# t-neumann/versalignLib

Hardware: AMD Instinct MI355X
Metric: GCUPS (giga DP cell updates/sec) SW affine-gap, 150x500 bp (higher is better)
Workload: dtype int16; 1 GPU; 1048576 pairs/GPU, 150 bp x 500 bp, SW affine-gap int16 score (open -5, extend -1), inputs resident in HBM; pairs_per_gpu=1048576, read_length=150, ref_length=500, kernel_geometry=16x10

## Files before the change

### versalignlib_amd/csrc/cell_constants.h

```cpp
#pragma once

namespace valign {

struct Scoring {
    int match = 2, mismatch = -1, gap_read = -3, gap_ref = -3;
    bool affine = false;
    int open_read = -3, ext_read = -3, open_ref = -3, ext_ref = -3;
};

constexpr int kAlgSW = 0;
constexpr int kAlgNW = 1;

constexpr int kGapLinear = 0, kGapSym = 1, kGapAffine = 2, kGapAffineSym = 3;
constexpr int kGapAffineSymF16 = 4, kGapAffineF16 = 5, kGapSymF16 = 6;
constexpr int kTiltMaxK = 12;

constexpr int kBandNwAbsent16 = -16384;
constexpr int kBandNwAbsent32 = -(1 << 29);

enum FillKernel {
    kFillLinear = 0,
    kFillLinearSym,
    kFillAffine,
    kFillSse,
    kFillTag,
    kFillTagKey,
    kFillAffineSym,
    kFillAffineTag,
    kFillAffineTagSym,
    kFillSseTag,
    kFillSseTagKey,
    kFillTagProfKey,
    kFillKernels
};

}
```

### versalignlib_amd/csrc/cell_rules.h

```cpp
#pragma once

#include <algorithm>
#include <cstdlib>
#include <stdexcept>
#include <string>

#include "cell_constants.h"

namespace valign {

struct RuleInputs {
    Scoring sc;
    int R = 0, F = 0;
    bool sse_policy = false;
    bool no_sym = false, no_tag = false, no_f16 = false, no_prof_key = false;
    bool no_max3 = false;
    bool no_tilt = false;
    bool no_row_tables = false;
};

inline long long nw_tilt_span(const Scoring &sc, int rows, int F) {
    const long long per_row = -(long long)(sc.affine ? sc.ext_ref : sc.gap_ref);
    const long long per_col = -(long long)(sc.affine ? sc.ext_read : sc.gap_read);
    return per_row * (rows + 1) + per_col * (F + 1);
}

inline bool half_float_exact(const Scoring &sc, int alg, int R, int F, int rows) {
    const long long top = (long long)std::min(R, F) * std::max({sc.match, sc.mismatch, 0});
    long long slack = std::max({std::abs(sc.match), std::abs(sc.mismatch), std::abs(sc.open_read),
                                std::abs(sc.ext_read), std::abs(sc.open_ref), std::abs(sc.ext_ref)});
    if (alg == kAlgSW) return top + 2 * slack <= 2048 && slack <= 1024;
    if (!sc.affine) slack = std::max<long long>(slack, std::max(std::abs(sc.gap_read), std::abs(sc.gap_ref)));
    const long long span = nw_tilt_span(sc, rows, F);
    const long long centre = (top + span) / 2;
    return span < 30000 && (top + span - centre) + 3 * slack <= 2048 && centre + 3 * slack <= 2048 && slack <= 512;
}

inline bool half_float_unit_exact(const Scoring &sc, int R, int F) {
    const long long top = (long long)std::min(R, F) * std::max({sc.match, sc.mismatch, 0});
    const long long slack = std::max({std::abs(sc.match), std::abs(sc.mismatch), std::abs(sc.gap_read), std::abs(sc.gap_ref)});
    return top + 2 * slack < 1024 && slack < 512;
}

inline bool int16_range_ok(const RuleInputs &in, int alg, bool score_path, bool long_mode, int tilt_rows) {
    const Scoring &sc = in.sc;
    long long hi = (long long)std::min(in.R, in.F) * std::max(sc.match, 0) + 1;
    if (score_path && alg == kAlgNW && !long_mode) hi += nw_tilt_span(sc, tilt_rows, in.F);
    const int worst_gap = std::min({sc.gap_read, sc.gap_ref, sc.open_read, sc.open_ref, sc.ext_read, sc.ext_ref, 0});
    long long lo = alg == kAlgSW ? (long long)std::min(sc.mismatch, 0) + worst_gap
                                 : (long long)(std::min(in.R, in.F) + 2) * std::min(worst_gap, std::min(sc.mismatch, 0));
    if ((!score_path || long_mode) && sc.affine && alg == kAlgNW)
        lo = (long long)std::min(sc.open_ref, 0) + (long long)in.R * std::min(sc.ext_ref, 0) + std::min({sc.open_read, sc.open_ref, 0}) +
             std::min(sc.mismatch, 0);
    return !(hi > 32000 || lo < -32000 || (sc.affine && alg == kAlgNW && lo < -15000));
}

inline bool border_bad(const RuleInputs &in, int alg) {
    return alg == kAlgNW && !in.sc.affine && (long long)(in.R + 1) * std::min(in.sc.gap_ref, 0) < -32000;
}

inline bool int32_refused(const RuleInputs &in) {
    const Scoring &sc = in.sc;
    const long long worst = std::max({std::abs((long long)sc.match), std::abs((long long)sc.mismatch),
                                      std::abs((long long)(sc.affine ? sc.open_read : sc.gap_read)), std::abs((long long)(sc.affine ? sc.open_ref : sc.gap_ref)),
                                      sc.affine ? std::abs((long long)sc.ext_read) : 0ll, sc.affine ? std::abs((long long)sc.ext_ref) : 0ll});
    return (long long)(in.R + in.F + 2) * worst >= (1ll << 28);
}

inline bool tagged_range_ok(const RuleInputs &in, int alg, int rows) {
    const Scoring &sc = in.sc;
    long long hi = (long long)std::min(in.R, in.F) * std::max(sc.match, 0) + 1;
    if (alg == kAlgNW && !in.sse_policy)
        hi += (long long)-sc.gap_ref * (rows + 1) + (long long)-sc.gap_read * (in.F + 1);
    const int worst = std::min({sc.gap_read, sc.gap_ref, sc.mismatch, 0});
    const long long lo = alg == kAlgSW ? worst : (long long)(in.R + in.F + 2) * worst;
    if (alg == kAlgSW && !in.sse_policy && sc.gap_ref >= 0) return false;
    return 4 * hi + 4 <= 32000 && 4 * lo - 4 >= -32000 && std::abs(sc.match) < 2000 && std::abs(sc.mismatch) < 2000;
}

inline bool affine_tagged_range_ok(const RuleInputs &in, int alg, int geo_rows, int K) {
    const Scoring &sc = in.sc;
    long long hi = (long long)std::min(in.R, in.F) * std::max(sc.match, 0) + 1;
    const int worst = std::min({sc.open_read, sc.open_ref, sc.ext_read, sc.ext_ref, sc.mismatch, 0});
    long long lo = alg == kAlgSW ? worst
                                 : 2ll * (std::min(sc.open_read, 0) + std::min(sc.open_ref, 0)) +
                                       (long long)(in.R + in.F + 2) * std::min({sc.ext_read, sc.ext_ref, 0}) + worst;
    if (alg == kAlgNW) {
        const long long rows = (long long)geo_rows + 1, cols = in.F + 1;
        hi += std::max(0, -sc.ext_ref) * rows + std::max(0, -sc.ext_read) * cols;
        lo += std::min(0, -sc.ext_ref) * rows + std::min(0, -sc.ext_read) * cols;
        if (std::abs((long long)sc.ext_ref) * rows > 3500 || std::abs((long long)sc.ext_read) * cols > 3500) return false;
    }
    if (alg == kAlgSW && (sc.open_read >= 0 || sc.open_ref >= 0)) return false;
    const int key_bits = K <= 16 ? 4 : 5;
    if (alg == kAlgSW && ((hi + 1) << key_bits) > 32000) return false;
    return 8 * hi + 8 <= 32000 && 8 * lo - 8 >= -28000 && std::abs(sc.match) < 1000 && std::abs(sc.mismatch) < 1000;
}

inline bool lane_key_ok(const RuleInputs &in, int K) {
    return (((long long)std::min(in.R, in.F) * std::max(in.sc.match, 0) + 1) << (K <= 16 ? 4 : 5)) <= 32000;
}
inline bool prof_key_ok(const RuleInputs &in, int K) {
    const Scoring &sc = in.sc;
    return !in.sse_policy && !in.no_prof_key && K <= 16 && (((long long)std::min(in.R, in.F) * std::max(sc.match, 0) + 2) << 6) <= 32000 &&
           64ll * std::max(std::abs(sc.gap_read), std::abs(sc.gap_ref)) < 32000 && 64ll * std::abs(sc.mismatch) < 16000;
}

inline int score_gap_form(const RuleInputs &in, int alg, int R, int F, int rows) {
    const Scoring &sc = in.sc;
    if (sc.affine) {
        const bool sym = sc.open_read == sc.open_ref && sc.ext_read == sc.ext_ref && !in.no_sym;
        if (!in.no_f16 && half_float_exact(sc, alg, R, F, rows)) return sym ? kGapAffineSymF16 : kGapAffineF16;
        return sym ? kGapAffineSym : kGapAffine;
    }
    const int gaps = (sc.gap_read == sc.gap_ref && !in.no_sym) ? kGapSym : kGapLinear;
    if ((gaps == kGapSym || alg == kAlgNW) && !in.no_f16 &&
        (alg == kAlgNW ? half_float_exact(sc, alg, R, F, rows) : half_float_unit_exact(sc, R, F)))
        return kGapSymF16;
    return gaps;
}
inline bool gap_form_f16(int gaps) { return gaps == kGapSymF16 || gaps == kGapAffineSymF16 || gaps == kGapAffineF16; }

constexpr int kMax3WindowLow = 0x0400, kMax3WindowHigh = 0x7BFF;
inline int sym_affine_bias(const Scoring &sc) {
    const int o = -sc.open_ref, x = -sc.ext_ref, m = std::max({0, -sc.mismatch, -sc.match});
    return kMax3WindowLow + o + x + m;
}
inline bool sym_affine_max3_ok(const RuleInputs &in, int R, int F) {
    const Scoring &sc = in.sc;
    if (in.no_max3 || !sc.affine || sc.open_read != sc.open_ref || sc.ext_read != sc.ext_ref) return false;
    if (sc.open_ref > 0 || sc.ext_ref > 0) return false;
    const long long B = sym_affine_bias(sc);
    const long long hi = (long long)std::min(R, F) * std::max({sc.match, sc.mismatch, 0}) + 1;
    return B - kMax3WindowLow <= 1024 && B + hi <= kMax3WindowHigh;
}
inline const char *ran_sym_affine_name(bool max3) { return max3 ? "max3" : "sources"; }

inline int sym_affine_tilt_bias(const Scoring &sc) {
    const int o = -sc.open_ref, x = -sc.ext_ref, m = std::max({0, -sc.mismatch, -sc.match});
    return kMax3WindowLow + std::max(o - x, m);
}
inline long long sym_affine_tilt_top_index(int R, int F, int rows, int K) {
    const int lead = rows > R ? (rows - R) / K : 0;
    return (long long)rows + F - lead;
}
inline bool sym_affine_tilt_ok(const RuleInputs &in, int R, int F, int rows, int K) {
    if (in.no_tilt || K > kTiltMaxK || !sym_affine_max3_ok(in, R, F)) return false;
    const Scoring &sc = in.sc;
    const long long B = sym_affine_tilt_bias(sc);
    const long long hi = (long long)std::min(R, F) * std::max({sc.match, sc.mismatch, 0}) + 1;
    return B + (long long)-sc.ext_ref * sym_affine_tilt_top_index(R, F, rows, K) + hi <= kMax3WindowHigh;
}
inline const char *ran_sym_affine_frame_name(bool tilted) { return tilted ? "tilted" : "plain"; }

inline int sym_affine_row_table_low(const Scoring &sc) { return std::min({sc.match, sc.mismatch, 0}) - 2 * sc.ext_ref; }
inline int sym_affine_row_table_high(const Scoring &sc) {
    return std::max({sc.match, sc.mismatch, 0}) - 2 * sc.ext_ref + (sc.ext_ref - sc.open_ref);
}
inline bool sym_affine_row_tables_ok(const RuleInputs &in, int R, int F, int rows, int K, int lds_profile, int lds_tables) {
    if (in.no_row_tables || !sym_affine_tilt_ok(in, R, F, rows, K)) return false;
    if (in.sc.ext_ref - in.sc.open_ref < 0 || F > 60000) return false;
    return sym_affine_row_table_low(in.sc) >= 0 && sym_affine_row_table_high(in.sc) <= 255 && lds_tables <= lds_profile;
}
inline const char *ran_sym_affine_scores_name(bool row_tables) { return row_tables ? "row_tables" : "lds_profile"; }

struct FillChoice {
    int kernel = 0;
    bool affine_tagged = false, tagged = false;
};
inline FillChoice fill_choice(const RuleInputs &in, int alg, int G, int K) {
    const Scoring &sc = in.sc;
    FillChoice c;
    const int rows = G * K;
    c.affine_tagged = sc.affine && !in.sse_policy && !in.no_tag && affine_tagged_range_ok(in, alg, rows, K);
    c.tagged = !sc.affine && !in.no_tag && tagged_range_ok(in, alg, rows);
    const bool lane_key = c.tagged && alg == kAlgSW && lane_key_ok(in, K);
    const bool prof_key = lane_key && prof_key_ok(in, K);
    const bool affine_sym = sc.affine && sc.open_read == sc.open_ref && sc.ext_read == sc.ext_ref && !in.no_sym;
    if (prof_key) c.kernel = kFillTagProfKey;
    else if (c.tagged) c.kernel = in.sse_policy ? (lane_key ? kFillSseTagKey : kFillSseTag) : (lane_key ? kFillTagKey : kFillTag);
    else if (in.sse_policy) c.kernel = kFillSse;
    else if (sc.affine) c.kernel = c.affine_tagged ? (affine_sym ? kFillAffineTagSym : kFillAffineTag) : (affine_sym ? kFillAffineSym : kFillAffine);
    else c.kernel = (sc.gap_read == sc.gap_ref && !in.no_sym) ? kFillLinearSym : kFillLinear;
    return c;
}

constexpr int placed_key_bits(int K) { return K <= 4 ? 2 : (K <= 8 ? 3 : 4); }
constexpr int kPlacedKeyMaxK = 16;
constexpr int kPlacedStripRows = 1024;

enum class PlacedRoute { Refused, Key, Rows, Strip, Chain, Wide };

constexpr int kBandPlacedKeyBits = 4;
inline bool band_placed_key_ok(const RuleInputs &in) {
    return (((long long)std::min(in.R, in.F) * std::max(in.sc.match, 0) + 1) << kBandPlacedKeyBits) <= 0x7FFFFFFFll;
}

struct PlacedFacts {
    int band_width = 0;
    int score_width = 0;
    bool forced = false;
    bool long_plan = false;
    bool band_placed = false;
    bool chain_usable = false;
    bool placed_wide = false;
    bool extend_wide = false;
};

struct PlacedChoice {
    PlacedRoute route = PlacedRoute::Refused;
    int key_bits = 0;
    const char *reason = "";
};

inline PlacedChoice placed_choice(const RuleInputs &in, int alg, const PlacedFacts &f, int G, int K) {
    PlacedChoice c;
    (void)G;
    if (alg != kAlgSW)
        c.reason = "placed scores exist for Smith-Waterman only (the NW variant's score and its alignment's end cell are different cells)";
    else if (f.band_width > 0 && !f.band_placed)
        c.reason = "placed scores are not built for band_width > 0";
    else if (in.sse_policy)
        c.reason = "placed scores are not built for traceback_policy = 1 (SSE/AVX tie-breaks)";
    else if (f.band_width > 0) {
        if (!f.chain_usable)
            c.reason = "band_placed: the block chain has no usable plan for this read_length, ref_length, band_width and scoring (band_chain_plan); "
                       "placed scores under a band run nowhere else";
        else if (int32_refused(in))
            c.reason = "band_placed: shape x scoring can leave the int32 range of the DP cells";
        else if (!band_placed_key_ok(in))
            c.reason = "band_placed: min(read_length, ref_length) x match leaves the range of the chain's end-cell key (value << 4 in int32)";
        else {
            c.route = PlacedRoute::Chain;
            c.key_bits = kBandPlacedKeyBits;
        }
        return c;
    } else if (f.score_width == 32)
        c.reason = "placed scores are not built for score_width = 32 (int32 cells)";
    else if (!int16_range_ok(in, kAlgSW, true, false, 0))
        c.reason = "placed scores run on int16 cells: shape x scoring can leave their range";
    if (c.reason[0] && alg == kAlgSW && f.band_width <= 0 && !in.sse_policy && f.placed_wide && f.score_width != 16) {
        c.reason = "";
        if (int32_refused(in))
            c.reason = "placed_wide: shape x scoring can leave the int32 range of the DP cells";
        else
            c.route = PlacedRoute::Wide;
        return c;
    }
    if (c.reason[0]) return c;
    if (f.long_plan || (!f.forced && in.R > kPlacedStripRows)) {
        c.route = PlacedRoute::Strip;
        return c;
    }
    const int bits = placed_key_bits(K);
    const long long top = (long long)std::min(in.R, in.F) * std::max(in.sc.match, 0);
    if (K <= kPlacedKeyMaxK && ((top + 1) << bits) <= 32000) {
        c.route = PlacedRoute::Key;
        c.key_bits = bits;
    } else {
        c.route = PlacedRoute::Rows;
    }
    return c;
}

inline const char *ran_placed_name(PlacedRoute r) {
    static const char *const names[] = {"none", "key", "rows", "strip", "chain", "wide"};
    return names[(int)r];
}

inline long long span_ref_length(const RuleInputs &in) {
    const Scoring &sc = in.sc;
    const long long R = in.R, F = in.F;
    const long long m = std::max({sc.match, sc.mismatch, 0});
    const long long c = sc.affine ? std::min(std::abs((long long)sc.open_read), std::abs((long long)sc.ext_read)) : std::abs((long long)sc.gap_read);
    if (c == 0) return F;
    const long long gap_cols = R * m >= 1 ? (R * m - 1) / c : 0;
    return std::min(F, R + gap_cols);
}

inline PlacedChoice span_choice(const RuleInputs &in, int alg, const PlacedFacts &f, int G = 0, int K = 0) {
    PlacedFacts unbanded = f;
    unbanded.band_width = 0;
    PlacedChoice c = placed_choice(in, alg, unbanded, G, K);
    if (c.route != PlacedRoute::Refused && f.band_width > 0) {
        c = PlacedChoice{};
        c.reason = "spanned scores are not built for band_width > 0";
    }
    return c;
}

inline PlacedChoice subopt_choice(const RuleInputs &in, int alg, const PlacedFacts &f, int G, int K, int mask = 0) {
    PlacedFacts plain = f;
    plain.band_width = 0;
    plain.placed_wide = false;
    PlacedChoice c = placed_choice(in, alg, plain, G, K);
    if (c.route == PlacedRoute::Refused) return c;
    const char *reason = "";
    if (mask < 0)
        reason = "suboptimal scores need mask >= 0";
    else if (f.band_width > 0)
        reason = "suboptimal scores are not built for band_width > 0";
    else if (c.route != PlacedRoute::Key && c.route != PlacedRoute::Rows)
        reason = "suboptimal scores run on the register sweep only: reads of more than 1024 rows and shapes without a register geometry are refused";
    if (reason[0]) {
        c = PlacedChoice{};
        c.reason = reason;
    }
    return c;
}

inline int subopt_block_waves(int wave_lds, int ring_bytes, int placed_waves, int block_limit) {
    for (int waves = placed_waves; waves >= 1; waves >>= 1)
        if ((long long)(wave_lds + ring_bytes) * waves <= block_limit) return waves;
    return 0;
}
constexpr const char *kSuboptNoRing = "suboptimal scores: one wave's reference tables leave no room for its column ring in the LDS (a shorter reference, or a geometry of more lanes per group, has it)";

inline long long extend_cell_top(const RuleInputs &in) {
    return (long long)std::min(in.R, in.F) * std::max({in.sc.match, in.sc.mismatch, 0});
}
inline long long extend_cell_bottom(const RuleInputs &in) {
    const Scoring &sc = in.sc;
    const long long per_row = sc.affine ? std::min({sc.open_ref, sc.ext_ref, 0}) : std::min(sc.gap_ref, 0);
    const long long per_col = sc.affine ? std::min({sc.open_read, sc.ext_read, 0}) : std::min(sc.gap_read, 0);
    const long long addend = sc.affine ? std::min({sc.match, sc.mismatch, sc.open_read, sc.ext_read, sc.open_ref, sc.ext_ref, 0})
                                       : std::min({sc.match, sc.mismatch, sc.gap_read, sc.gap_ref, 0});
    return per_row * in.R + per_col * in.F + addend;
}
inline bool extend_int16_ok(const RuleInputs &in) { return extend_cell_top(in) <= 32000 && extend_cell_bottom(in) >= -32000; }

constexpr long long kExtendWideCellBound = 1ll << 28;
constexpr int kExtendWideLoses = -(1 << 29);
inline bool extend_int32_ok(const RuleInputs &in) {
    const Scoring &sc = in.sc;
    const long long top_addend = std::max({sc.match, sc.mismatch, 0});
    const long long worst_ext = sc.affine ? std::min({sc.ext_read, sc.ext_ref, 0}) : std::min({sc.gap_read, sc.gap_ref, 0});
    const long long low_addend = sc.affine ? std::min({sc.match, sc.mismatch, sc.open_read, sc.ext_read, sc.open_ref, sc.ext_ref, 0})
                                           : std::min({sc.match, sc.mismatch, sc.gap_read, sc.gap_ref, 0});
    if (extend_cell_top(in) > kExtendWideCellBound || extend_cell_bottom(in) < -kExtendWideCellBound) return false;
    if (kExtendWideLoses + top_addend >= -kExtendWideCellBound) return false;
    return kExtendWideLoses + worst_ext * ((long long)in.R + in.F) + low_addend >= -(1ll << 31);
}

inline PlacedChoice extend_choice(const RuleInputs &in, int alg, const PlacedFacts &f, int G, int K) {
    PlacedChoice c;
    (void)G;
    (void)K;
    bool opens_wide = false;
    if (alg != kAlgSW)
        c.reason = "extension scores are defined for opt & 0xF == 0 only (the NW variant's free reference start is another matrix)";
    else if (in.sse_policy)
        c.reason = "extension scores are not built for traceback_policy = 1 (SSE/AVX tie-breaks)";
    else if (f.band_width > 0)
        c.reason = "extension scores are not built for band_width > 0";
    else if (f.score_width == 32) {
        c.reason = "extension scores are not built for score_width = 32 (int32 cells)";
        opens_wide = true;
    } else if (!extend_int16_ok(in)) {
        c.reason = "extension scores run on signed int16 cells: shape x scoring can leave their range";
        opens_wide = f.score_width == 0;
    } else if (f.long_plan || (!f.forced && in.R > kPlacedStripRows)) {
        c.reason = "extension scores run on the register sweep only: reads of more than 1024 rows and shapes without a register geometry are refused";
        opens_wide = true;
    } else
        c.route = PlacedRoute::Rows;
    if (opens_wide && f.extend_wide) {
        if (extend_int32_ok(in)) {
            c.reason = "";
            c.route = PlacedRoute::Wide;
        } else {
            c.reason = "extend_wide: shape x scoring can leave the range the int32 cells keep below their borders' sentinel";
        }
    }
    return c;
}

inline bool band_nw_connects(int R, int F, int band_width) {
    return R > 0 && 2ll * (band_width / 2) + 1 >= ((long long)F + R - 1) / R;
}
inline void band_nw_check(int R, int F, int band_width) {
    if (!band_nw_connects(R, F, band_width))
        throw std::runtime_error("band_nw: band_width " + std::to_string(band_width) + " is too narrow for read_length " + std::to_string(R) +
                                 ", ref_length " + std::to_string(F) + " (the windows of consecutive blocks do not connect: 2 * (band_width / 2) + 1 "
                                 "must be at least ceil(ref_length / read_length))");
}

inline bool band_nw_int16_ok(const RuleInputs &in) {
    const Scoring &sc = in.sc;
    const long long worst = sc.affine ? std::min({sc.open_read, sc.open_ref, sc.ext_read, sc.ext_ref, sc.mismatch, sc.match, 0})
                                      : std::min({sc.gap_read, sc.gap_ref, sc.mismatch, sc.match, 0});
    const long long top_add = std::max({sc.match, sc.mismatch, 0});
    const long long hi = (long long)std::min(in.R, in.F) * std::max(sc.match, 0) + 1;
    const long long lo = (long long)(in.R + in.F + 2) * worst + (sc.affine ? std::min({sc.open_read, sc.open_ref, 0}) : 0);
    return kBandNwAbsent16 + top_add < lo && kBandNwAbsent16 + worst >= -32768 && hi <= 16000;
}

enum class AlignRoute { Fused, Register, Strip, StripBand, StripWide, StripWideBand, StripCkpt };

struct RouteFacts {
    bool banded = false;
    bool wide_align = false;
    bool read_strips = false;
    bool fused_off = false;
    bool small_call = false;
    int fused_rows = 0;
    bool checkpoints = false;
    bool band_nw = false;
    int band_width = 0;
};

inline AlignRoute align_route(const RuleInputs &in, int alg, const RouteFacts &f) {
    if (f.banded && alg != kAlgSW && !f.band_nw) throw std::runtime_error("band_alignments applies to Smith-Waterman alignments only");
    if (f.banded && in.sse_policy)
        throw std::runtime_error("band_alignments needs traceback_policy = 0 (no banded SSE/AVX tie-breaks)");
    const bool nw_band = f.banded && alg == kAlgNW;
    if (nw_band) band_nw_check(in.R, in.F, f.band_width);
    if (border_bad(in, alg) || !int16_range_ok(in, alg, false, false, 0) || f.wide_align || (nw_band && !band_nw_int16_ok(in))) {
        if (int32_refused(in))
            throw std::runtime_error("shape x scoring can leave the int32 range of the DP cells (read_length " + std::to_string(in.R) +
                                     ", ref_length " + std::to_string(in.F) + ")");
        return f.banded ? AlignRoute::StripWideBand : AlignRoute::StripWide;
    }
    if (f.banded) return AlignRoute::StripBand;
    if (f.read_strips) return (f.checkpoints && !in.sse_policy) ? AlignRoute::StripCkpt : AlignRoute::Strip;
    if (in.sse_policy && in.sc.affine)
        throw std::runtime_error("traceback_policy = 1 (SSE/AVX tie-breaks) exists for the linear gap model only");
    if (f.small_call && !f.fused_off && !in.sc.affine && !in.sse_policy && !in.no_tag && tagged_range_ok(in, alg, f.fused_rows)) return AlignRoute::Fused;
    return AlignRoute::Register;
}

inline bool strip_chunks(AlignRoute r, const RouteFacts &f) {
    return r == AlignRoute::Strip || r == AlignRoute::StripCkpt || r == AlignRoute::StripBand || r == AlignRoute::StripWideBand || (r == AlignRoute::StripWide && f.read_strips);
}

inline const char *ran_fill_name(AlignRoute r, int fill_kernel = -1) {
    static const char *const names[kFillKernels] = {"linear", "linear_sym", "affine", "sse", "tag", "tag_key", "affine_sym",
                                                    "affine_tag", "affine_tag_sym", "sse_tag", "sse_tag_key", "tag_prof_key"};
    static const char *const routes[] = {"fused_tag", nullptr, "strip", "strip_band", "strip_wide", "strip_wide_band", "strip_ckpt"};
    if (r != AlignRoute::Register) return routes[(int)r];
    return fill_kernel >= 0 && fill_kernel < kFillKernels ? names[fill_kernel] : "none";
}

struct SpanCigarChoice {
    PlacedChoice forward;
    AlignRoute child = AlignRoute::Register;
    std::string reason;
    bool refused() const { return !reason.empty(); }
};
constexpr const char *kSpanCigarPrefix = "spanned CIGARs: ";
inline SpanCigarChoice span_cigar_choice(const RuleInputs &in, int alg, const PlacedFacts &f, const RuleInputs &child, const RouteFacts &child_facts,
                                         int G = 0, int K = 0) {
    SpanCigarChoice c;
    c.forward = span_choice(in, alg, f, G, K);
    if (c.forward.route == PlacedRoute::Refused) {
        c.reason = c.forward.reason;
        return c;
    }
    try {
        c.child = align_route(child, alg, child_facts);
    } catch (const std::runtime_error &e) {
        c.forward = PlacedChoice{};
        c.reason = std::string(kSpanCigarPrefix) + e.what();
    }
    return c;
}

}
```

### versalignlib_amd/csrc/dp_kernels.hip.h

```cpp
#pragma once

#include <hip/hip_runtime.h>
#include <stdint.h>

#include <type_traits>
#include <utility>

#include "base_classes.h"
#include "cell_constants.h"

namespace valign {

typedef short s16x2 __attribute__((ext_vector_type(2)));
typedef _Float16 f16x2 __attribute__((ext_vector_type(2)));
typedef unsigned short u16x2 __attribute__((ext_vector_type(2)));

constexpr int kWave = 64;
constexpr int kWaveLanes = 64;
constexpr int kCodePad = 72;
constexpr short kNegInf = -16384;

constexpr int kMaxScoreGroups = 16;
constexpr int kOneSweep = 0x7FFFFFFF;

struct ScoreArgs {
    const uint8_t *reads;
    const uint8_t *refs;
    int16_t *scores;
    long long n;
    int R, F;
    int prof_area;
    int refc_stride;
    int wave_lds;
    short match, mismatch;
    union {
        struct {
            short gap_read, gap_ref;
        };
        int sym_max3_bias;
    };
    short open_read, ext_read, open_ref, ext_ref;
    int n_groups;
    struct Group {
        unsigned block_end;
        int F;
        long long n;
        long long pair_ofs;
        long long read_ofs, ref_ofs;
    } groups[kMaxScoreGroups];
};

__device__ __forceinline__ s16x2 pk(short v) { return s16x2{v, v}; }
__device__ __forceinline__ s16x2 pk_max(s16x2 a, s16x2 b) { return __builtin_elementwise_max(a, b); }
__device__ __forceinline__ s16x2 pk_add_sat(s16x2 a, s16x2 b) { return __builtin_elementwise_add_sat(a, b); }
__device__ __forceinline__ s16x2 pk_sub_floor0(s16x2 a, s16x2 g) {
    return (s16x2)__builtin_elementwise_sub_sat((u16x2)a, (u16x2)g);
}
__device__ __forceinline__ unsigned as_u32(s16x2 v) { return __builtin_bit_cast(unsigned, v); }
__device__ __forceinline__ s16x2 as_pk(unsigned v) { return __builtin_bit_cast(s16x2, v); }

__device__ __forceinline__ unsigned from_prev_lane(unsigned v) {
    return (unsigned)__builtin_amdgcn_update_dpp(0, (int)v, 0x138 , 0xF, 0xF, false);
}

template <int G>
__device__ __forceinline__ unsigned group_prev_or_zero(unsigned v, unsigned lmask) {
    if (G == 16) return (unsigned)__builtin_amdgcn_update_dpp(0, (int)v, 0x111 , 0xF, 0xF, true);
    return from_prev_lane(v) & lmask;
}

template <int G>
__device__ __forceinline__ s16x2 group_prev_or(s16x2 v, s16x2 lead_border, unsigned lmask) {
    return as_pk(group_prev_or_zero<G>(as_u32(v), lmask) | as_u32(lead_border));
}
__device__ __forceinline__ s16x2 pk_max_h(s16x2 a, s16x2 b) {
    return __builtin_bit_cast(s16x2, __builtin_elementwise_maximum(__builtin_bit_cast(f16x2, a), __builtin_bit_cast(f16x2, b)));
}
__device__ __forceinline__ s16x2 pk_max3_h(s16x2 a, s16x2 b, s16x2 c) {
    return __builtin_bit_cast(s16x2, __builtin_elementwise_maximum(__builtin_elementwise_maximum(__builtin_bit_cast(f16x2, a), __builtin_bit_cast(f16x2, b)),
                                                                  __builtin_bit_cast(f16x2, c)));
}

template <int... Is, class Fn>
__device__ __forceinline__ void unrolled_steps(std::integer_sequence<int, Is...>, Fn &&fn) {
    (fn(std::integral_constant<int, Is>{}), ...);
}

constexpr int profile_conflicts(int G, int lane_dw, int width, int stride_dw) {
    const int banks = width == 1 ? 32 : 64;
    int extra = 0;
    const int ngroups = width == 4 ? 4 : 2;
    for (int grp = 0; grp < ngroups; ++grp) {
        int hits[64] = {};
        int worst = 0;
        for (int lane = 0; lane < kWaveLanes; ++lane) {
            int member = 0;
            if (width == 4) {
                const int m = lane & 31;
                const bool first = m < 4 || (m >= 12 && m < 16) || (m >= 20 && m < 28);
                member = (lane < 32 ? 0 : 2) + (first ? 0 : 1);
            } else {
                member = lane / 32;
            }
            if (member != grp) continue;
            const int l = lane % G, pair = 2 * (lane / G);
            const int dw = pair * stride_dw + l * lane_dw;
            for (int x = 0; x < width; ++x) {
                const int b = (dw + x) % banks;
                hits[b] += 1;
                worst = hits[b] > worst ? hits[b] : worst;
            }
        }
        extra += worst - 1;
    }
    return extra;
}

template <int G, int K>
struct Geo {
    static_assert(G == 4 || G == 8 || G == 16 || G == 32 || G == 64, "group size");
    static_assert(K % 2 == 0, "rows per lane must be even");
    static constexpr int kGroups = kWave / G;
    static constexpr int kPairs = 2 * kGroups;
    static constexpr int kRows = G * K;
    static constexpr int kLaneBytes = K * 2;
    static constexpr int kLoadDwords = (K * 2) % 16 == 0 ? 4 : ((K * 2) % 8 == 0 ? 2 : 1);
    static constexpr int slab_dwords() {
        const int rows_dw = kRows / 2;
        int best = rows_dw, best_cost = profile_conflicts(G, K / 2, kLoadDwords, rows_dw);
        for (int pad = kLoadDwords; pad < 64 && best_cost > 0; pad += kLoadDwords) {
            const int c = profile_conflicts(G, K / 2, kLoadDwords, rows_dw + pad);
            if (c < best_cost) {
                best_cost = c;
                best = rows_dw + pad;
            }
        }
        return best;
    }
    static constexpr int kPairStride = slab_dwords() * 4;
    static constexpr int kZeroSlab = 4 * kPairs;
    static constexpr int kProfBytes = (4 * kPairs + 1) * kPairStride;
    __host__ __device__ static constexpr int row_offset(int l, int q) { return l * kLaneBytes + q * 2; }
};

typedef __attribute__((address_space(3))) const unsigned lds_cu32;
typedef unsigned u32x2 __attribute__((ext_vector_type(2)));
typedef unsigned u32x4 __attribute__((ext_vector_type(4)));
typedef __attribute__((address_space(3))) const u32x2 lds_cu32x2;
typedef __attribute__((address_space(3))) const u32x4 lds_cu32x4;
typedef __attribute__((address_space(3))) const unsigned char lds_cu8;

__device__ __forceinline__ unsigned lds_offset(const void *p) {
    return (unsigned)(size_t)(__attribute__((address_space(3))) const void *)p;
}

__device__ __forceinline__ void stage_span(unsigned char *dst, const uint8_t *src, long long begin,
                                           long long end, int lane) {
    const unsigned long long a0 = (unsigned long long)(src + begin) & ~15ull;
    const unsigned long long lo = (unsigned long long)(src + begin);
    const unsigned long long hi = (unsigned long long)(src + end);
    for (unsigned long long a = a0 + 16ull * lane; a < hi; a += 16ull * kWave) {
        unsigned char *d = dst + (a - a0);
        if (a >= lo && a + 16 <= hi) {
            *reinterpret_cast<uint4 *>(d) = *reinterpret_cast<const uint4 *>(a);
        } else {
            for (int b = 0; b < 16; ++b)
                if (a + b >= lo && a + b < hi) d[b] = *reinterpret_cast<const uint8_t *>(a + b);
        }
    }
}

__device__ __forceinline__ unsigned lds_dword_at(const unsigned char *p) {
    const unsigned a = lds_offset(p), base = a & ~3u;
    const unsigned lo = *(lds_cu32 *)(base), hi = *(lds_cu32 *)(base + 4);
    return __builtin_amdgcn_alignbyte(hi, lo, a & 3u);
}

extern __shared__ __align__(16) unsigned char valign_smem[];

struct WaveTables {
    unsigned char *prof;
    unsigned char *refc;
    int *first_bad;
    long long pair0;
    int last;
    int cols_used;
};

template <int G, int K, bool FIND_BAD>
__device__ __forceinline__ bool wave_setup(const uint8_t *reads, const uint8_t *refs, long long n, int R, int F,
                                           int prof_area, int refc_stride, int wave_lds, short match,
                                           short mismatch, WaveTables &w, bool bad_is_non_acgt = false,
                                           unsigned block = blockIdx.x, short zero_score = 0,
                                           int strip_row0 = kOneSweep, short row_key_step = 0, short row0_score = 0) {
    using geo = Geo<G, K>;
    const int lane = threadIdx.x & (kWave - 1);
    const int wave = threadIdx.x / kWave;
    const int row0 = strip_row0 == kOneSweep ? R - geo::kRows : strip_row0;

    unsigned char *lds = valign_smem + (size_t)wave * wave_lds;
    unsigned char *prof = lds;
    unsigned char *refc = lds + prof_area;
    int *first_bad = reinterpret_cast<int *>(refc + geo::kGroups * refc_stride);

    const int waves = blockDim.x / kWave;
    const long long pair0 = ((long long)block * waves + wave) * geo::kPairs;
    const bool live = pair0 < n;
    long long pair_end = pair0 + geo::kPairs;
    if (pair_end > n) pair_end = n;
    const int last = (int)(pair_end - pair0) - 1;

    const bool whole = geo::kPairs * F + 32 <= prof_area;
    const int rd_off = ((geo::kPairs * F + 32 + 15) / 16) * 16;
    const bool rd_staged = whole && strip_row0 == kOneSweep && rd_off + geo::kPairs * R + 32 <= prof_area;

    unsigned char rd[2 * K];
    if (live && FIND_BAD && lane < geo::kPairs) {
        first_bad[2 * lane] = R;
        first_bad[2 * lane + 1] = F;
    }
    if (live && !rd_staged) {
#pragma unroll
        for (int i = 0; i < 2 * K; ++i) {
            const int idx = lane + kWave * i;
            const int p = idx / geo::kRows, rr = idx - p * geo::kRows;
            const int ps = p > last ? last : p;
            const int pos = row0 + rr;
            rd[i] = (pos >= 0 && pos < R) ? reads[(pair0 + ps) * R + pos] : (unsigned char)0;
        }
    }

    int cols_used = 0;
    if (live) {
        for (int idx = lane; idx < geo::kGroups * 2 * kCodePad; idx += kWave) {
            const int g = idx / (2 * kCodePad), x = idx - g * (2 * kCodePad);
            const int col = x < kCodePad ? x : F + x;
            unsigned char *dst = refc + g * refc_stride + 2 * col;
            dst[0] = dst[1] = (unsigned char)geo::kZeroSlab;
        }
    }
    if (whole) {
        if (live) stage_span(prof, refs, pair0 * F, pair_end * F, lane);
        if (live && rd_staged) stage_span(prof + rd_off, reads, pair0 * R, pair_end * R, lane);
        __syncthreads();
    }
    constexpr unsigned kZero4 = (unsigned)geo::kZeroSlab * 0x01010101u;
#pragma unroll
    for (int g = 0; g < geo::kGroups; ++g) {
        int pa = 2 * g, pb = 2 * g + 1;
        pa = pa > last ? last : pa;
        pb = pb > last ? last : pb;
        const long long ref_lo = whole ? pair0 * F : (pair0 + pa) * F;
        if (!whole) {
            if (live) stage_span(prof, refs, ref_lo, (pair0 + pb + 1) * F, lane);
            __syncthreads();
        }
        if (live) {
            const int ref_skew = (int)((unsigned long long)(refs + ref_lo) & 15ull);
            const unsigned char *raw_a = prof + ref_skew + (whole ? pa * F : 0), *raw_b = raw_a + (pb - pa) * F;
            unsigned char *codes_g = refc + g * refc_stride + 2 * kCodePad;
            const unsigned slab_a_lo = geo::kZeroSlab | (unsigned)(2 * g) << 8 | (unsigned)(geo::kPairs + 2 * g) << 16 |
                                       (unsigned)(2 * geo::kPairs + 2 * g) << 24;
            const unsigned slab_a_hi = (unsigned)(3 * geo::kPairs + 2 * g) | (kZero4 & 0xFFFFFF00u);
            const unsigned slab_b_lo = slab_a_lo + 0x01010100u, slab_b_hi = slab_a_hi + 1u;
            const int F4 = F & ~3;
            for (int j = 4 * lane; j < F4; j += 4 * kWave) {
                const unsigned ca = base_class4(lds_dword_at(raw_a + j)), cb = base_class4(lds_dword_at(raw_b + j));
                const unsigned sa = select_bytes8(slab_a_hi, slab_a_lo, ca), sb = select_bytes8(slab_b_hi, slab_b_lo, cb);
                uint2 codes;
                codes.x = __builtin_amdgcn_perm(sb, sa, 0x05010400u);
                codes.y = __builtin_amdgcn_perm(sb, sa, 0x07030602u);
                *reinterpret_cast<uint2 *>(codes_g + 2 * j) = codes;
                const unsigned used = (sa ^ kZero4) | (sb ^ kZero4);
                if (used) {
                    const int end = j + 4 - (__builtin_clz(used) >> 3);
                    cols_used = end > cols_used ? end : cols_used;
                }
                if (FIND_BAD) {
                    const unsigned bad_a = ~nonzero_bytes(bad_is_non_acgt ? sa ^ kZero4 : ca) & 0x80808080u;
                    const unsigned bad_b = ~nonzero_bytes(bad_is_non_acgt ? sb ^ kZero4 : cb) & 0x80808080u;
                    if (bad_a) atomicMin(&first_bad[2 * (2 * g) + 1], j + (__builtin_ctz(bad_a) >> 3));
                    if (bad_b) atomicMin(&first_bad[2 * (2 * g + 1) + 1], j + (__builtin_ctz(bad_b) >> 3));
                }
            }
            for (int j = F4 + lane; j < F; j += kWave) {
                const int ca = base_class(raw_a[j]);
                const int cb = base_class(raw_b[j]);
                const bool va = ca >= 1 && ca <= 4, vb = cb >= 1 && cb <= 4;
                const unsigned sa = va ? (ca - 1) * geo::kPairs + 2 * g : geo::kZeroSlab;
                const unsigned sb = vb ? (cb - 1) * geo::kPairs + 2 * g + 1 : geo::kZeroSlab;
                *reinterpret_cast<unsigned short *>(codes_g + 2 * j) = (unsigned short)(sa | (sb << 8));
                if (va || vb) cols_used = j + 1 > cols_used ? j + 1 : cols_used;
                if (FIND_BAD) {
                    if (ca == 0 || (bad_is_non_acgt && ca == 5)) atomicMin(&first_bad[2 * (2 * g) + 1], j);
                    if (cb == 0 || (bad_is_non_acgt && cb == 5)) atomicMin(&first_bad[2 * (2 * g + 1) + 1], j);
                }
            }
        }
        if (!whole) __syncthreads();
    }
    unsigned rd4[K / 2];
    constexpr int kItemPairs = 256 / geo::kRows, kItemRows = 256 % geo::kRows;
    const int item_p0 = (4 * lane) / geo::kRows, item_rr0 = (4 * lane) % geo::kRows, item_q0 = (4 * lane) % K;
    if (live && rd_staged) {
        const unsigned char *raw = prof + rd_off + (int)((unsigned long long)(reads + pair0 * R) & 15ull);
        int p = item_p0, rr = item_rr0;
#pragma unroll
        for (int it = 0; it < K / 2; ++it) {
            const int ps = p > last ? last : p;
            const int pos = row0 + rr;
            const int at = pos < -3 ? -3 : pos;
            unsigned w4 = lds_dword_at(raw + ps * R + at);
            if (pos < 0) w4 = pos < -3 ? 0u : w4 & (0xFFFFFFFFu << (8 * -pos));
            rd4[it] = base_class4(w4);
            p += kItemPairs; rr += kItemRows;
            if (rr >= geo::kRows) { rr -= geo::kRows; ++p; }
        }
    }
    if (whole) __syncthreads();

    if (live && rd_staged) {
        auto table = [&](int c, int shift, unsigned &lo, unsigned &hi) __attribute__((always_inline)) {
            unsigned b[8];
#pragma unroll
            for (int a = 0; a < 8; ++a)
                b[a] = ((unsigned)(unsigned short)(a >= 1 && a <= 4 ? (a == c + 1 ? match : mismatch) : zero_score) >> shift) & 0xFFu;
            lo = b[0] | b[1] << 8 | b[2] << 16 | b[3] << 24;
            hi = b[4] | b[5] << 8 | b[6] << 16 | b[7] << 24;
        };
        int p = item_p0, rr = item_rr0;
#pragma unroll
        for (int it = 0; it < K / 2; ++it) {
            const unsigned cls = rd4[it];
            const int pos = row0 + rr;
            if (FIND_BAD) {
                unsigned good = bad_is_non_acgt ? select_bytes8(0x00000001u, 0x01010100u, cls) : cls;
                if (pos < 0) good |= pos < -3 ? 0xFFFFFFFFu : ~(0xFFFFFFFFu << (8 * -pos));
                const unsigned bad = ~nonzero_bytes(good) & 0x80808080u;
                if (bad) atomicMin(&first_bad[2 * p], pos + (__builtin_ctz(bad) >> 3));
            }
            u16x2 key01 = u16x2{0, 0}, key23 = u16x2{0, 0};
            if (row_key_step != 0) {
                const int q0 = rr % K, q1 = (rr + 1) % K, q2 = (rr + 2) % K, q3 = (rr + 3) % K;
                key01 = u16x2{(unsigned short)(row_key_step * (15 - q0)), (unsigned short)(row_key_step * (15 - q1))};
                key23 = u16x2{(unsigned short)(row_key_step * (15 - q2)), (unsigned short)(row_key_step * (15 - q3))};
            }
            if (row0_score != 0) {
                int q0 = item_q0 + (256 * it) % K;
                q0 -= q0 >= K ? K : 0;
                auto row0 = [&](int i) __attribute__((always_inline)) {
                    const int q = q0 + i;
                    return (i == 0 ? q == 0 : q == K) || (K < 4 && q == 2 * K);
                };
                const unsigned short a = (unsigned short)row0_score, none = 0;
                key01 = key01 + u16x2{row0(0) ? a : none, row0(1) ? a : none};
                key23 = key23 + u16x2{row0(2) ? a : none, row0(3) ? a : none};
            }
            unsigned char *dst = prof + p * geo::kPairStride + 2 * rr;
#pragma unroll
            for (int c = 0; c < 4; ++c) {
                unsigned lo_lo, lo_hi, hi_lo, hi_hi;
                table(c, 0, lo_lo, lo_hi);
                table(c, 8, hi_lo, hi_hi);
                const unsigned lows = select_bytes8(lo_hi, lo_lo, cls), highs = select_bytes8(hi_hi, hi_lo, cls);
                const u16x2 s01 = __builtin_bit_cast(u16x2, __builtin_amdgcn_perm(highs, lows, 0x05010400u)) + key01;
                const u16x2 s23 = __builtin_bit_cast(u16x2, __builtin_amdgcn_perm(highs, lows, 0x07030602u)) + key23;
                unsigned *out = reinterpret_cast<unsigned *>(dst + c * geo::kPairs * geo::kPairStride);
                out[0] = __builtin_bit_cast(unsigned, s01);
                out[1] = __builtin_bit_cast(unsigned, s23);
            }
            p += kItemPairs; rr += kItemRows;
            if (rr >= geo::kRows) { rr -= geo::kRows; ++p; }
        }
    }
    if (live && !rd_staged) {
#pragma unroll
        for (int i = 0; i < 2 * K; ++i) {
            const int idx = lane + kWave * i;
            const int p = idx / geo::kRows, rr = idx - p * geo::kRows;
            const int pos = row0 + rr;
            const bool in_read = pos >= 0 && pos < R;
            const int a = in_read ? base_class(rd[i]) : 0;
            if (FIND_BAD && in_read && (a == 0 || (bad_is_non_acgt && a == 5)))
                atomicMin(&first_bad[2 * p], pos);
            const bool valid = a >= 1 && a <= 4;
            const int off = p * geo::kPairStride + geo::row_offset(rr / K, rr % K);
            const short row_key = (short)(row_key_step * (15 - rr % K) + (rr % K == 0 ? row0_score : 0));
#pragma unroll
            for (int c = 0; c < 4; ++c) {
                const short sc = (short)((valid ? (a == c + 1 ? match : mismatch) : zero_score) + row_key);
                *reinterpret_cast<short *>(prof + c * geo::kPairs * geo::kPairStride + off) = sc;
            }
        }
    }
    if (live) {
        for (int idx = lane; idx < geo::kPairStride / 4; idx += kWave) {
            const unsigned lo = (unsigned short)(zero_score + row_key_step * (15 - (2 * idx) % K) + ((2 * idx) % K == 0 ? row0_score : 0));
            const unsigned hi = (unsigned short)(zero_score + row_key_step * (15 - (2 * idx + 1) % K) + ((2 * idx + 1) % K == 0 ? row0_score : 0));
            reinterpret_cast<unsigned *>(prof + geo::kZeroSlab * geo::kPairStride)[idx] = lo | (hi << 16);
        }
    }
    __syncthreads();
#pragma unroll
    for (int d = kWave / 2; d >= 1; d >>= 1) {
        const int other = __shfl_xor(cols_used, d, kWave);
        cols_used = other > cols_used ? other : cols_used;
    }
    w.cols_used = __builtin_amdgcn_readfirstlane(cols_used);
    w.prof = prof;
    w.refc = refc + 2 * kCodePad;
    w.first_bad = first_bad;
    w.pair0 = pair0;
    w.last = last;
    return live;
}

constexpr int row_table_pad(int G) { return G + 4; }
constexpr unsigned kSelZero4 = 0x0c0c0c0cu;

template <int G, int K>
__device__ __forceinline__ bool wave_setup_tables(const uint8_t *reads, const uint8_t *refs, long long n, int R, int F,
                                                  int refs_area, int sel_stride, int wave_lds, short match, short mismatch,
                                                  short zero_score, short row0_score, unsigned block, WaveTables &w,
                                                  unsigned (&Ta)[K], unsigned (&Tb)[K], bool &repair) {
    using geo = Geo<G, K>;
    constexpr int kPad = row_table_pad(G);
    const int lane = threadIdx.x & (kWave - 1);
    const int wave = threadIdx.x / kWave;
    const int row0 = R - geo::kRows;

    unsigned char *raw = valign_smem + (size_t)wave * wave_lds;
    unsigned char *sel = raw + refs_area;

    const int waves = blockDim.x / kWave;
    const long long pair0 = ((long long)block * waves + wave) * geo::kPairs;
    const bool live = pair0 < n;
    long long pair_end = pair0 + geo::kPairs;
    if (pair_end > n) pair_end = n;
    const int last = (int)(pair_end - pair0) - 1;

    if (live) {
        stage_span(raw, refs, pair0 * F, pair_end * F, lane);
        stage_span(sel, reads, pair0 * R, pair_end * R, lane);
    }
    __syncthreads();

    if (live) {
        auto table = [&](int c, unsigned &lo, unsigned &hi) __attribute__((always_inline)) {
            unsigned b[8];
#pragma unroll
            for (int a = 0; a < 8; ++a) b[a] = (unsigned)(a >= 1 && a <= 4 ? (a == c + 1 ? match : mismatch) : zero_score) & 0xFFu;
            lo = b[0] | b[1] << 8 | b[2] << 16 | b[3] << 24;
            hi = b[4] | b[5] << 8 | b[6] << 16 | b[7] << 24;
        };
        unsigned t_lo[4], t_hi[4];
#pragma unroll
        for (int c = 0; c < 4; ++c) table(c, t_lo[c], t_hi[c]);
        const unsigned char *raw_rd = sel + (int)((unsigned long long)(reads + pair0 * R) & 15ull);
        const int grp = lane / G, l = lane % G;
#pragma unroll
        for (int half = 0; half < 2; ++half) {
            int p = 2 * grp + half;
            p = p > last ? last : p;
#pragma unroll
            for (int q0 = 0; q0 < K; q0 += 4) {
                const int pos = row0 + l * K + q0;
                const int at = pos < -3 ? -3 : pos;
                unsigned w4 = lds_dword_at(raw_rd + p * R + at);
                if (pos < 0) w4 = pos < -3 ? 0u : w4 & (0xFFFFFFFFu << (8 * -pos));
                const unsigned cls = base_class4(w4);
                unsigned col[4];
#pragma unroll
                for (int c = 0; c < 4; ++c) col[c] = select_bytes8(t_hi[c], t_lo[c], cls);
                const unsigned lo01 = __builtin_amdgcn_perm(col[1], col[0], 0x05010400u), hi01 = __builtin_amdgcn_perm(col[1], col[0], 0x07030602u);
                const unsigned lo23 = __builtin_amdgcn_perm(col[3], col[2], 0x05010400u), hi23 = __builtin_amdgcn_perm(col[3], col[2], 0x07030602u);
                unsigned (&T)[K] = half ? Tb : Ta;
                T[q0] = __builtin_amdgcn_perm(lo23, lo01, 0x05040100u);
                T[q0 + 1] = __builtin_amdgcn_perm(lo23, lo01, 0x07060302u);
                if (q0 + 2 < K) {
                    T[q0 + 2] = __builtin_amdgcn_perm(hi23, hi01, 0x05040100u);
                    T[q0 + 3] = __builtin_amdgcn_perm(hi23, hi01, 0x07060302u);
                }
            }
        }
        const unsigned r4 = ((unsigned)row0_score & 0xFFu) * 0x01010101u;
        Ta[0] += r4;
        Tb[0] += r4;
    }
    __syncthreads();

    int cols_used = 0;
    bool before_last = false;
    unsigned *stream = reinterpret_cast<unsigned *>(sel);
    const int stride_dw = sel_stride / 4;
    if (live) {
        for (int idx = lane; idx < geo::kGroups * 2 * kPad; idx += kWave) {
            const int g = idx / (2 * kPad), x = idx - g * (2 * kPad);
            stream[g * stride_dw + (x < kPad ? x : F + x)] = kSelZero4;
        }
        const int ref_skew = (int)((unsigned long long)(refs + pair0 * F) & 15ull);
        typedef unsigned short u16;
#pragma unroll
        for (int g = 0; g < geo::kGroups; ++g) {
            int pa = 2 * g, pb = 2 * g + 1;
            pa = pa > last ? last : pa;
            pb = pb > last ? last : pb;
            const unsigned char *raw_a = raw + ref_skew + pa * F, *raw_b = raw + ref_skew + pb * F;
            unsigned *out_g = stream + g * stride_dw + kPad;
            u16x2 ends_a = u16x2{0, 0}, ends_b = u16x2{0, 0};
            auto note = [](u16x2 &ends, unsigned acgt, int j) __attribute__((always_inline)) {
                const unsigned none = ~nonzero_bytes(acgt) & 0x80808080u;
                const u16 end = acgt ? (u16)(j + 4 - (__builtin_clz(acgt) >> 3)) : (u16)0;
                const u16 first_none = none ? (u16)(0xFFFF - (j + (__builtin_ctz(none) >> 3))) : (u16)0;
                ends = __builtin_elementwise_max(ends, u16x2{end, first_none});
            };
            const int F4 = F & ~3;
            for (int j = 4 * lane; j < F4; j += 4 * kWave) {
                const unsigned ca = base_class4(lds_dword_at(raw_a + j)), cb = base_class4(lds_dword_at(raw_b + j));
                const unsigned sa = select_bytes8(0x0c0c0c03u, 0x0201000cu, ca), sb = select_bytes8(0x0c0c0c07u, 0x0605040cu, cb);
                uint4 s;
                s.x = __builtin_amdgcn_perm(sb, sa, 0x0c040c00u) | 0x0c000c00u;
                s.y = __builtin_amdgcn_perm(sb, sa, 0x0c050c01u) | 0x0c000c00u;
                s.z = __builtin_amdgcn_perm(sb, sa, 0x0c060c02u) | 0x0c000c00u;
                s.w = __builtin_amdgcn_perm(sb, sa, 0x0c070c03u) | 0x0c000c00u;
                *reinterpret_cast<uint4 *>(out_g + j) = s;
                note(ends_a, sa ^ kSelZero4, j);
                note(ends_b, sb ^ kSelZero4, j);
            }
            for (int j = F4 + lane; j < F; j += kWave) {
                const int ca = base_class(raw_a[j]), cb = base_class(raw_b[j]);
                const bool va = ca >= 1 && ca <= 4, vb = cb >= 1 && cb <= 4;
                out_g[j] = (va ? (unsigned)(ca - 1) : 0x0cu) | (vb ? (unsigned)(cb + 3) : 0x0cu) << 16 | 0x0c000c00u;
                ends_a = __builtin_elementwise_max(ends_a, u16x2{va ? (u16)(j + 1) : (u16)0, va ? (u16)0 : (u16)(0xFFFF - j)});
                ends_b = __builtin_elementwise_max(ends_b, u16x2{vb ? (u16)(j + 1) : (u16)0, vb ? (u16)0 : (u16)(0xFFFF - j)});
            }
#pragma unroll
            for (int d = kWave / 2; d >= 1; d >>= 1) {
                ends_a = __builtin_elementwise_max(ends_a, __builtin_bit_cast(u16x2, __shfl_xor(__builtin_bit_cast(int, ends_a), d, kWave)));
                ends_b = __builtin_elementwise_max(ends_b, __builtin_bit_cast(u16x2, __shfl_xor(__builtin_bit_cast(int, ends_b), d, kWave)));
            }
            before_last |= 0xFFFF - (int)ends_a.y < (int)ends_a.x || 0xFFFF - (int)ends_b.y < (int)ends_b.x;
            cols_used = (int)ends_a.x > cols_used ? (int)ends_a.x : cols_used;
            cols_used = (int)ends_b.x > cols_used ? (int)ends_b.x : cols_used;
        }
    }
    __syncthreads();
    repair = __builtin_amdgcn_readfirstlane((int)before_last) != 0;
    w.cols_used = __builtin_amdgcn_readfirstlane(cols_used);
    w.prof = raw;
    w.refc = reinterpret_cast<unsigned char *>(stream + kPad);
    w.first_bad = nullptr;
    w.pair0 = pair0;
    w.last = last;
    return live;
}

template <int K>
__device__ __forceinline__ void lds_load_lane(unsigned addr, unsigned (&v)[K / 2]) {
    constexpr int N = K / 2;
    if constexpr ((K * 2) % 16 == 0) {
#pragma unroll
        for (int i = 0; i < N / 4; ++i) {
            const u32x4 x = *(lds_cu32x4 *)(addr + 16 * i);
            v[4 * i] = x.x; v[4 * i + 1] = x.y; v[4 * i + 2] = x.z; v[4 * i + 3] = x.w;
        }
    } else if constexpr ((K * 2) % 8 == 0) {
#pragma unroll
        for (int i = 0; i < N / 2; ++i) {
            const u32x2 x = *(lds_cu32x2 *)(addr + 8 * i);
            v[2 * i] = x.x; v[2 * i + 1] = x.y;
        }
    } else {
#pragma unroll
        for (int i = 0; i < N; ++i) v[i] = *(lds_cu32 *)(addr + 4 * i);
    }
}

template <int K>
__device__ __forceinline__ void merge_profile(const unsigned (&va)[K / 2], const unsigned (&vb)[K / 2], s16x2 (&S)[K]) {
#pragma unroll
    for (int c = 0; c < K / 2; ++c) {
        S[2 * c + 0] = as_pk(__builtin_amdgcn_perm(vb[c], va[c], 0x05040100u));
        S[2 * c + 1] = as_pk(__builtin_amdgcn_perm(vb[c], va[c], 0x07060302u));
    }
}

template <int G, int K>
__device__ __forceinline__ void fetch_profile(unsigned addr_a, unsigned addr_b, s16x2 (&S)[K]) {
    unsigned va[K / 2], vb[K / 2];
    lds_load_lane<K>(addr_a, va);
    lds_load_lane<K>(addr_b, vb);
    merge_profile<K>(va, vb, S);
}



constexpr int kTrackAll = 0, kTrackNone = 1, kTrackPair = 2;

__host__ __device__ inline int nw_frame_centre(int R, int F, int rows, int match, int mismatch, int tilt_row, int tilt_col) {
    const int best = match > mismatch ? match : mismatch;
    const int top = (R < F ? R : F) * (best > 0 ? best : 0);
    return (top + tilt_row * (rows + 1) + tilt_col * (F + 1)) / 2;
}

template <int G, int K, int ALG, int GAPS>
__global__ void __launch_bounds__(256)
score_kernel(const ScoreArgs args) {
    using geo = Geo<G, K>;
    constexpr bool F16 = GAPS == kGapAffineSymF16 || GAPS == kGapAffineF16;
    constexpr bool F16SYM = GAPS == kGapAffineSymF16;
    constexpr bool AFFINE = GAPS == kGapAffine || GAPS == kGapAffineSym || F16;
    constexpr bool SYM = GAPS == kGapSym;
    constexpr bool LINF16 = GAPS == kGapSymF16;
    constexpr bool AFFSYM = GAPS == kGapAffineSym;
    constexpr bool SOURCES = AFFSYM && ALG == kAlgSW;
    const int lane = threadIdx.x & (kWave - 1);
    const int grp = lane / G;
    const int l = lane % G;

    const uint8_t *reads = args.reads, *refs = args.refs;
    int16_t *scores = args.scores;
    long long n_pairs = args.n;
    int F_batch = args.F;
    unsigned block = blockIdx.x;
    if (args.n_groups > 0) {
        int g = 0;
        while (g + 1 < args.n_groups && block >= args.groups[g].block_end) ++g;
        block -= g ? args.groups[g - 1].block_end : 0u;
        reads += args.groups[g].read_ofs;
        refs += args.groups[g].ref_ofs;
        scores += args.groups[g].pair_ofs;
        n_pairs = args.groups[g].n;
        F_batch = args.groups[g].F;
    }

    WaveTables w;
    constexpr bool LINF16_SW = LINF16 && ALG == kAlgSW, LINF16_NW = LINF16 && ALG == kAlgNW;
    constexpr bool TILT = ALG == kAlgNW;
    constexpr bool HALF = F16 || LINF16;
    const int tilt_row = TILT ? -(int)(AFFINE ? args.ext_ref : args.gap_ref) : 0;
    const int tilt_col = TILT ? -(int)(AFFINE ? args.ext_read : args.gap_read) : 0;
    int fold = tilt_row + tilt_col;
    short s_row0 = 0;
    if constexpr (SOURCES && K <= kTiltMaxK) {
        if (args.sym_max3_bias > 0 && (args.sym_max3_bias >> 16) != 0) {
            fold = -2 * (int)args.ext_ref;
            s_row0 = (short)((int)args.ext_ref - (int)args.open_ref);
        }
    }
    const int centre = (HALF && TILT) ? nw_frame_centre(args.R, F_batch, G * K, args.match, args.mismatch, tilt_row, tilt_col) : 0;
    const int rcentre = (HALF && TILT) ? nw_frame_centre(args.R, F_batch, G * K, args.match, args.mismatch, 0, 0) : 0;
    const float unit = LINF16_SW ? 1.0f / 1024.0f : 1.0f;
    auto cell = [](int v) __attribute__((always_inline)) {
        return HALF ? pk(__builtin_bit_cast(short, (_Float16)v)) : pk((short)v);
    };
    auto cell_add = [](s16x2 a, s16x2 b) __attribute__((always_inline)) {
        return HALF ? __builtin_bit_cast(s16x2, __builtin_bit_cast(f16x2, a) + __builtin_bit_cast(f16x2, b)) : a + b;
    };
    auto cell_sub = [](s16x2 a, s16x2 b) __attribute__((always_inline)) {
        return HALF ? __builtin_bit_cast(s16x2, __builtin_bit_cast(f16x2, a) - __builtin_bit_cast(f16x2, b)) : a - b;
    };
    const short s_match = HALF ? __builtin_bit_cast(short, (_Float16)(((int)args.match + fold) * unit)) : (short)(args.match + fold);
    const short s_mismatch = HALF ? __builtin_bit_cast(short, (_Float16)(((int)args.mismatch + fold) * unit)) : (short)(args.mismatch + fold);
    const short s_zero = HALF ? __builtin_bit_cast(short, (_Float16)fold) : (short)fold;
    bool tables = false, repair = false;
    unsigned Ta[K], Tb[K];
    if constexpr (SOURCES && K <= kTiltMaxK) {
        tables = args.sym_max3_bias > 0 && (args.sym_max3_bias >> 16 & 3) == 3;
        bool live = false;
        if (tables)
            live = wave_setup_tables<G, K>(reads, refs, n_pairs, args.R, F_batch, args.prof_area, args.refc_stride, args.wave_lds,
                                           s_match, s_mismatch, s_zero, s_row0, block, w, Ta, Tb, repair);
        if (!tables)
            live = wave_setup<G, K, false>(reads, refs, n_pairs, args.R, F_batch, args.prof_area, args.refc_stride,
                                           args.wave_lds, s_match, s_mismatch, w, false, block, s_zero, kOneSweep, 0, s_row0);
        if (!live) return;
    } else if (!wave_setup<G, K, false>(reads, refs, n_pairs, args.R, F_batch, args.prof_area, args.refc_stride,
                                        args.wave_lds, s_match, s_mismatch, w, false, block, s_zero, kOneSweep, 0, s_row0))
        return;
    const long long pair0 = w.pair0;
    const int F = (ALG == kAlgSW) ? w.cols_used : F_batch;

    const unsigned lmask = l == 0 ? 0u : 0xFFFFFFFFu;
    const unsigned lane_base = lds_offset(w.prof) + l * geo::kLaneBytes;
    const int lead = (ALG == kAlgSW && G * K > args.R) ? (G * K - args.R) / K : 0;
    unsigned code_addr = lds_offset(w.refc) + grp * args.refc_stride - 2 * (l - lead);

    s16x2 g_read, g_ref, o_read, e_read, o_ref, e_ref;
    if (ALG == kAlgSW) {
        g_read = pk((short)-args.gap_read);   g_ref = pk((short)-args.gap_ref);
        o_read = pk((short)-args.open_read);  e_read = pk((short)-args.ext_read);
        o_ref = pk((short)-args.open_ref);    e_ref = pk((short)-args.ext_ref);
    } else {
        g_read = g_ref = e_read = e_ref = pk(0);
        o_read = pk((short)(args.open_read - args.ext_read));
        o_ref = pk((short)(args.open_ref - args.ext_ref));
    }
    const s16x2 border_f = pk(ALG == kAlgNW ? (F16 ? (short)0xFC00 : kNegInf) : (short)0);
    const _Float16 open_h = (_Float16)(int)(TILT ? args.open_ref - args.ext_ref : args.open_ref), ext_h = (_Float16)(int)args.ext_ref;
    const _Float16 open_rd = (_Float16)(int)(TILT ? args.open_read - args.ext_read : args.open_read), ext_rd = (_Float16)(int)args.ext_read;
    const f16x2 o_half = f16x2{open_h, open_h}, e_half = f16x2{ext_h, ext_h}, zero_half = f16x2{(_Float16)0, (_Float16)0};
    const f16x2 o_read_half = f16x2{open_rd, open_rd}, e_read_half = f16x2{ext_rd, ext_rd};

    s16x2 Hl[K], El[K], HOl[K];
#pragma unroll
    for (int q = 0; q < K; ++q) {
        Hl[q] = cell(tilt_row * (l * K + q) - centre);
        El[q] = border_f;
        HOl[q] = (ALG == kAlgSW) ? pk(0) : (F16 ? cell_add(Hl[q], pk(__builtin_bit_cast(short, open_h))) : Hl[q] + o_ref);
    }
    s16x2 up0 = pk(0), h_last = Hl[K - 1], f_last = border_f, best = pk(0);
    s16x2 fup_keep = border_f;
    s16x2 row_best = cell(-rcentre);
    int j = -l;
    s16x2 top_row = pk(0), top_step = pk(0), row_tilt = pk(0);
    const s16x2 col_step = cell(tilt_col);
    if (TILT) {
        if (l == 0) {
            top_row = cell(-tilt_row + tilt_col - centre);
            top_step = col_step;
            up0 = cell(-tilt_row - centre);
        }
        row_tilt = cell(tilt_row * (G * K - 1) + tilt_col * (1 - l) - centre + rcentre);
    }

    constexpr bool PIPE = true;
    unsigned pa[K / 2], pb[K / 2];
    s16x2 S0[K], S1[K];
    unsigned ca_next = 0, cb_next = 0;
    if (PIPE && !tables) {
        const unsigned ca = *(lds_cu8 *)(code_addr), cb = *(lds_cu8 *)(code_addr + 1);
        lds_load_lane<K>(lane_base + ca * geo::kPairStride, pa);
        lds_load_lane<K>(lane_base + cb * geo::kPairStride, pb);
        ca_next = *(lds_cu8 *)(code_addr + 2);
        cb_next = *(lds_cu8 *)(code_addr + 3);
    }

    lds_cu8 *code_ptr = (lds_cu8 *)code_addr;

    auto step = [&](auto masked_tag, auto track_tag, s16x2 (&S)[K], s16x2 (&Snext)[K]) __attribute__((always_inline)) {
        constexpr bool MASKED = decltype(masked_tag)::value;
        constexpr int TRACK = decltype(track_tag)::value;
        const s16x2 diag0 = up0;
        if (G == 16) {
            up0 = as_pk((unsigned)__builtin_amdgcn_update_dpp(0, (int)as_u32(h_last), 0x111, 0xF, 0xF, true));
        } else {
            up0 = as_pk(from_prev_lane(as_u32(h_last)) & lmask);
        }
        if (TILT) up0 = as_pk(as_u32(up0) | as_u32(top_row));
        s16x2 fup0 = border_f;
        if (AFFINE && !SOURCES) {
            if (G == 16 && ALG == kAlgSW) {
                fup0 = as_pk((unsigned)__builtin_amdgcn_update_dpp(0, (int)as_u32(f_last), 0x111, 0xF, 0xF, true));
            } else if (G != 16) {
                const unsigned fv = from_prev_lane(as_u32(f_last));
                fup0 = (ALG == kAlgNW) ? as_pk(l == 0 ? as_u32(border_f) : fv) : as_pk(fv & lmask);
            }
            if (G == 16 && ALG == kAlgNW) {
                fup_keep = as_pk((unsigned)__builtin_amdgcn_update_dpp((int)as_u32(fup_keep), (int)as_u32(f_last), 0x111, 0xF, 0xF, false));
                fup0 = fup_keep;
            }
        }
        s16x2 gup0 = pk(0);
        if (LINF16_SW) gup0 = as_pk(group_prev_or_zero<G>(as_u32(f_last), lmask));
        if (PIPE) {
            merge_profile<K>(pa, pb, S);
            lds_load_lane<K>(lane_base + ca_next * geo::kPairStride, pa);
            lds_load_lane<K>(lane_base + cb_next * geo::kPairStride, pb);
            if constexpr (SOURCES) {
                ca_next = code_ptr[4];
                cb_next = code_ptr[5];
            } else {
                ca_next = *(lds_cu8 *)(code_addr + 4);
                cb_next = *(lds_cu8 *)(code_addr + 5);
            }
        }
        if (!MASKED || (unsigned)j < (unsigned)F) {
            if (!PIPE) {
                const unsigned ca = *(lds_cu8 *)(code_addr), cb = *(lds_cu8 *)(code_addr + 1);
                fetch_profile<G, K>(lane_base + ca * geo::kPairStride, lane_base + cb * geo::kPairStride, S);
            }
            if (LINF16_SW) {
                auto hf = [](s16x2 v) __attribute__((always_inline)) { return __builtin_bit_cast(f16x2, v); };
                auto bits = [](f16x2 v) __attribute__((always_inline)) { return __builtin_bit_cast(s16x2, v); };
                const _Float16 gs = (_Float16)((int)args.gap_ref * (1.0f / 1024.0f));
                const f16x2 g_unit = f16x2{gs, gs}, zero2 = f16x2{(_Float16)0, (_Float16)0}, one2 = f16x2{(_Float16)1, (_Float16)1};
                f16x2 up_c = hf(gup0);
                f16x2 h = zero2;
                f16x2 d_cur = hf(diag0) + hf(S[0]), d_prev = zero2;
                f16x2 bestf = hf(best);
#pragma unroll
                for (int q = 0; q < K; ++q) {
                    f16x2 d_next = d_cur;
                    if (q + 1 < K) d_next = hf(Hl[q]) + hf(S[q + 1]);
                    h = __builtin_elementwise_maximum(__builtin_elementwise_maximum(d_cur, hf(El[q])), up_c);
                    Hl[q] = bits(h);
                    up_c = __builtin_elementwise_min(__builtin_elementwise_max(h + g_unit, zero2), one2);
                    El[q] = bits(up_c);
                    if (q & 1) bestf = __builtin_elementwise_maximum(__builtin_elementwise_maximum(bestf, d_prev), d_cur);
                    else if (q == K - 1) bestf = __builtin_elementwise_maximum(bestf, d_cur);
                    d_prev = d_cur;
                    d_cur = d_next;
                }
                best = bits(bestf);
                h_last = bits(h);
                f_last = bits(up_c);
            } else if (LINF16) {
                auto hf = [](s16x2 v) __attribute__((always_inline)) { return __builtin_bit_cast(f16x2, v); };
                f16x2 h = hf(up0);
                f16x2 d_cur = hf(diag0) + hf(S[0]);
#pragma unroll
                for (int q = 0; q < K; ++q) {
                    f16x2 d_next = d_cur;
                    if (q + 1 < K) d_next = hf(Hl[q]) + hf(S[q + 1]);
                    h = __builtin_elementwise_maximum(__builtin_elementwise_maximum(d_cur, hf(Hl[q])), h);
                    Hl[q] = __builtin_bit_cast(s16x2, h);
                    d_cur = d_next;
                }
                h_last = __builtin_bit_cast(s16x2, h);
            } else if (F16) {
                auto hf = [](s16x2 v) __attribute__((always_inline)) { return __builtin_bit_cast(f16x2, v); };
                auto bits = [](f16x2 v) __attribute__((always_inline)) { return __builtin_bit_cast(s16x2, v); };
                f16x2 d_cur, e_cur, d_prev = zero_half;
                auto pass1 = [&](int q, f16x2 &d, f16x2 &e) __attribute__((always_inline)) {
                    d = hf(q == 0 ? diag0 : Hl[q - 1]) + hf(S[q]);
                    const f16x2 e_open = F16SYM ? hf(HOl[q]) : hf(Hl[q]) + o_read_half;
                    e = __builtin_elementwise_maximum(TILT ? hf(El[q]) : hf(El[q]) + e_read_half, e_open);
                    if (ALG == kAlgSW) e = __builtin_elementwise_maximum(e, zero_half);
                    El[q] = bits(e);
                };
                f16x2 f = hf(fup0);
                f16x2 ho = hf(up0) + o_half;
                f16x2 h = zero_half;
                f16x2 bestf = hf(best);
                pass1(0, d_cur, e_cur);
#pragma unroll
                for (int q = 0; q < K; ++q) {
                    f = __builtin_elementwise_maximum(TILT ? f : f + e_half, ho);
                    f16x2 d_next = zero_half, e_next = zero_half;
                    if (q + 1 < K) pass1(q + 1, d_next, e_next);
                    h = __builtin_elementwise_maximum(__builtin_elementwise_maximum(d_cur, e_cur), f);
                    Hl[q] = bits(h);
                    ho = h + o_half;
                    if (F16SYM) HOl[q] = bits(ho);
                    if (ALG == kAlgSW) {
                        if (q & 1) bestf = __builtin_elementwise_maximum(__builtin_elementwise_maximum(bestf, d_prev), d_cur);
                        else if (q == K - 1) bestf = __builtin_elementwise_maximum(bestf, d_cur);
                    }
                    d_prev = d_cur;
                    d_cur = d_next;
                    e_cur = e_next;
                }
                best = bits(bestf);
                h_last = bits(h);
                f_last = bits(f);
            } else if (SOURCES) {
                s16x2 d_cur = diag0 + S[0];
                s16x2 xf = as_pk(group_prev_or_zero<G>(as_u32(f_last), lmask)), h = pk(0);
#pragma unroll
                for (int q = 0; q < K; ++q) {
                    const s16x2 g = pk_max(El[q], xf);
                    s16x2 d_next = pk(0);
                    if (q + 1 < K) d_next = Hl[q] + S[q + 1];
                    const s16x2 y = pk_sub_floor0(g, o_ref);
                    const s16x2 a = pk_sub_floor0(El[q], e_ref);
                    if (TRACK == kTrackAll) best = pk_max(best, d_cur);
                    if (TRACK == kTrackPair) best = pk_max(best, g);
                    h = pk_max(d_cur, y);
                    const s16x2 b = pk_sub_floor0(xf, e_ref);
                    Hl[q] = h;
                    El[q] = pk_max(a, h);
                    xf = pk_max(b, h);
                    d_cur = d_next;
                }
                if (TRACK == kTrackPair) best = pk_max(best, h);
                h_last = h;
                f_last = xf;
            } else if (SYM) {
                s16x2 h = up0;
                s16x2 d_cur = diag0 + S[0];
#pragma unroll
                for (int q = 0; q < K; ++q) {
                    const s16x2 x = pk_max(Hl[q], h);
                    s16x2 d_next = pk(0);
                    if (q + 1 < K) d_next = Hl[q] + S[q + 1];
                    const s16x2 y = (ALG == kAlgSW) ? pk_sub_floor0(x, g_ref) : x;
                    if (ALG == kAlgSW && TRACK == kTrackAll) best = pk_max(best, d_cur);
                    if (ALG == kAlgSW && TRACK == kTrackPair) best = pk_max(best, x);
                    h = pk_max(d_cur, y);
                    Hl[q] = h;
                    d_cur = d_next;
                }
                if (ALG == kAlgSW && TRACK == kTrackPair) best = pk_max(best, h);
                h_last = h;
            } else {
                auto pass1 = [&](int q) __attribute__((always_inline)) -> s16x2 {
                    const s16x2 d = (q == 0 ? diag0 : Hl[q - 1]) + S[q];
                    s16x2 e;
                    if (AFFSYM) {
                        e = pk_max((ALG == kAlgSW) ? pk_sub_floor0(El[q], e_read) : El[q], HOl[q]);
                        El[q] = e;
                    } else if (AFFINE) {
                        e = (ALG == kAlgSW)
                                ? pk_max(pk_sub_floor0(El[q], e_read), pk_sub_floor0(Hl[q], o_read))
                                : pk_max(El[q], pk_add_sat(Hl[q], o_read));
                        El[q] = e;
                    } else {
                        e = (ALG == kAlgSW) ? pk_sub_floor0(Hl[q], g_read) : Hl[q];
                    }
                    if (ALG == kAlgSW) best = pk_max(best, d);
                    return pk_max(d, e);
                };
                s16x2 h = up0, f = fup0;
                s16x2 ho = pk(0);
                if (AFFSYM) ho = (ALG == kAlgSW) ? pk_sub_floor0(up0, o_ref) : pk_add_sat(up0, o_ref);
                s16x2 m_cur = pass1(0);
#pragma unroll
                for (int q = 0; q < K; ++q) {
                    if (AFFSYM) {
                        f = pk_max((ALG == kAlgSW) ? pk_sub_floor0(f, e_ref) : f, ho);
                    } else if (AFFINE) {
                        f = (ALG == kAlgSW) ? pk_max(pk_sub_floor0(f, e_ref), pk_sub_floor0(h, o_ref))
                                            : pk_max(f, pk_add_sat(h, o_ref));
                    } else {
                        f = (ALG == kAlgSW) ? pk_sub_floor0(h, g_ref) : h;
                    }
                    s16x2 m_next = pk(0);
                    if (q + 1 < K) m_next = pass1(q + 1);
                    h = pk_max(m_cur, f);
                    Hl[q] = h;
                    if (AFFSYM) {
                        ho = (ALG == kAlgSW) ? pk_sub_floor0(h, o_ref) : pk_add_sat(h, o_ref);
                        HOl[q] = ho;
                    }
                    m_cur = m_next;
                }
                h_last = h;
                f_last = f;
            }
            if (ALG == kAlgNW) {
                const s16x2 last = cell_sub(h_last, row_tilt);
                if (HALF) row_best = __builtin_bit_cast(s16x2, __builtin_elementwise_maximum(__builtin_bit_cast(f16x2, row_best),
                                                                                      __builtin_bit_cast(f16x2, last)));
                else row_best = pk_max(row_best, last);
            }
        }
        if (TILT) {
            top_row = cell_add(top_row, top_step);
            row_tilt = cell_add(row_tilt, col_step);
        }
        ++j;
        if constexpr (SOURCES) code_ptr += 2;
        else code_addr += 2;
    };

    using all_t = std::integral_constant<int, kTrackAll>;
    using first_t = std::integral_constant<int, ((SYM && ALG == kAlgSW) || SOURCES) ? kTrackNone : kTrackAll>;
    using second_t = std::integral_constant<int, ((SYM && ALG == kAlgSW) || SOURCES) ? kTrackPair : kTrackAll>;
    if constexpr (ALG == kAlgSW) {
        static_assert(G - 1 + 1 + 2 <= kCodePad, "the unmasked sweep and its prefetch stay inside the code pad");
        const int steps = F + G - 1 - lead;
        int t = 0;
        bool biased = false;
        if constexpr (SOURCES) {
            biased = args.sym_max3_bias > 0;
            const bool tilted = K <= kTiltMaxK && biased && (args.sym_max3_bias >> 16) != 0;
            if constexpr (K <= kTiltMaxK) if (tilted) {
                const int B = args.sym_max3_bias & 0xFFFF, xi = -(int)args.ext_ref;
                const int oxi = -(int)args.open_ref - xi;
                const s16x2 ox_c = pk((short)oxi), kx_c = pk((short)(K * xi));
                const int u0 = l * (K - 1);
                s16x2 lead_border = as_pk(as_u32(pk((short)(B + xi - oxi))) & ~lmask);
                const s16x2 lead_step = as_pk(as_u32(pk((short)xi)) & ~lmask);
                const int s0 = K - steps % K;
                s16x2 fl[K], acc[K], dprev[K];
#pragma unroll
                for (int q = 0; q < K; ++q) {
                    Hl[q] = El[q] = pk((short)(B + xi * (u0 + q + 1)));
                    HOl[q] = Hl[q] - ox_c;
                    int c = q - s0;
                    c += c < 0 ? K : 0;
                    fl[q] = acc[q] = pk((short)(B + xi * (u0 + c + 2)));
                    dprev[q] = Hl[q];
                }
                up0 = pk((short)(B + xi * u0 - oxi));
                f_last = HOl[K - 1];
                constexpr int kLdsProfile = 0, kRowTables = 1, kRowTablesRepair = 2;
                lds_cu32 *sel_ptr = (lds_cu32 *)(lds_offset(w.refc) + grp * args.refc_stride - 4 * (l - lead));
                unsigned sel_cur = 0, sel_next = 0;
                if (tables) {
                    sel_cur = sel_ptr[0];
                    sel_next = sel_ptr[1];
                }
                const unsigned zero_q = as_u32(pk(s_zero)), zero_0 = as_u32(pk((short)(s_zero + s_row0)));
                auto tilted_step = [&](auto slot_tag, auto form_tag) __attribute__((always_inline)) {
                    constexpr int SLOT0 = decltype(slot_tag)::value;
                    constexpr int FORM = decltype(form_tag)::value;
                    s16x2 S[K], d[K];
                    const s16x2 diag0 = up0;
                    up0 = group_prev_or<G>(HOl[K - 1], lead_border, lmask);
                    lead_border = lead_border + lead_step;
                    if constexpr (FORM == kLdsProfile) {
                        merge_profile<K>(pa, pb, S);
                        lds_load_lane<K>(lane_base + ca_next * geo::kPairStride, pa);
                        lds_load_lane<K>(lane_base + cb_next * geo::kPairStride, pb);
                        ca_next = ((volatile lds_cu8 *)code_ptr)[4];
                        cb_next = ((volatile lds_cu8 *)code_ptr)[5];
                    } else {
#pragma unroll
                        for (int q = 0; q < K; ++q) S[q] = as_pk(__builtin_amdgcn_perm(Tb[q], Ta[q], sel_cur));
                        if constexpr (FORM == kRowTablesRepair) {
                            const unsigned none = ((sel_cur >> 3) & 0x00010001u) * 0xFFFFu;
                            const unsigned fix_0 = zero_0 & none, fix_q = zero_q & none;
#pragma unroll
                            for (int q = 0; q < K; ++q) S[q] = as_pk(as_u32(S[q]) | (q == 0 ? fix_0 : fix_q));
                        }
                        sel_cur = sel_next;
                        sel_next = ((volatile lds_cu32 *)sel_ptr)[2];
                        sel_ptr += 1;
                    }
                    s16x2 e_cur;
                    auto pass1 = [&](int q, s16x2 &e) __attribute__((always_inline)) {
                        d[q] = (q == 0 ? diag0 : Hl[q - 1]) + S[q];
                        e = pk_max3_h(El[q], HOl[q], fl[(q + SLOT0) % K]);
                        El[q] = e;
                    };
                    s16x2 ho = up0;
                    pass1(0, e_cur);
                    s16x2 f = as_pk(group_prev_or_zero<G>(as_u32(f_last), lmask)), h = pk(0);
#pragma unroll
                    for (int q = 0; q < K; ++q) {
                        f = pk_max_h(f, ho);
                        s16x2 e_next = pk(0);
                        if (q + 1 < K) pass1(q + 1, e_next);
                        h = pk_max3_h(d[q], e_cur, f);
                        Hl[q] = h;
                        ho = h - ox_c;
                        HOl[q] = ho;
                        if (!(q & 1)) {
                            s16x2 &a = acc[(q + SLOT0) % K];
                            a = pk_max3_h(a, d[q], dprev[q + 1]);
                        }
                        e_cur = e_next;
                    }
#pragma unroll
                    for (int q = 1; q < K; q += 2) dprev[q] = d[q];
                    f_last = f;
                    acc[SLOT0 % K] = acc[SLOT0 % K] + kx_c;
                    fl[SLOT0 % K] = fl[SLOT0 % K] + kx_c;
                    if constexpr (FORM == kLdsProfile) code_ptr += 2;
                };
                auto tilted_sweep = [&](auto form_tag) __attribute__((always_inline)) {
                    unrolled_steps(std::make_integer_sequence<int, K>{}, [&](auto slot_tag) __attribute__((always_inline)) {
                        if constexpr (decltype(slot_tag)::value > 0) {
                            if (decltype(slot_tag)::value >= s0) tilted_step(slot_tag, form_tag);
                        }
                    });
                    for (int trips = steps / K; trips > 0; --trips)
                        unrolled_steps(std::make_integer_sequence<int, K>{}, [&](auto slot_tag) __attribute__((always_inline)) { tilted_step(slot_tag, form_tag); });
                };
                int form = __builtin_amdgcn_readfirstlane(tables ? (repair ? kRowTablesRepair : kRowTables) : kLdsProfile);
                if (form == kLdsProfile) tilted_sweep(std::integral_constant<int, kLdsProfile>{});
                asm volatile("" : "+s"(form));
                if (form == kRowTables) tilted_sweep(std::integral_constant<int, kRowTables>{});
                asm volatile("" : "+s"(form));
                if (form == kRowTablesRepair) tilted_sweep(std::integral_constant<int, kRowTablesRepair>{});
                best = pk(0);
#pragma unroll
                for (int q = 0; q < K; q += 2) acc[q] = pk_max_h(acc[q], dprev[q + 1]);
#pragma unroll
                for (int q = 0; q < K; ++q) best = pk_max(best, acc[q] - fl[q]);
            }
            if (biased && !tilted) {
                const s16x2 bias_c = pk((short)args.sym_max3_bias);
                const s16x2 lead_bias = as_pk(as_u32(bias_c) & ~lmask);
                auto biased_step = [&](s16x2 (&S)[K]) __attribute__((always_inline)) {
                    const s16x2 diag0 = up0;
                    up0 = group_prev_or<G>(h_last, lead_bias, lmask);
                    merge_profile<K>(pa, pb, S);
                    lds_load_lane<K>(lane_base + ca_next * geo::kPairStride, pa);
                    lds_load_lane<K>(lane_base + cb_next * geo::kPairStride, pb);
                    ca_next = code_ptr[4];
                    cb_next = code_ptr[5];
                    s16x2 d_cur, e_cur, d_prev = bias_c;
                    auto pass1 = [&](int q, s16x2 &d, s16x2 &e) __attribute__((always_inline)) {
                        d = (q == 0 ? diag0 : Hl[q - 1]) + S[q];
                        e = pk_max3_h(El[q] - e_read, HOl[q], bias_c);
                        El[q] = e;
                    };
                    s16x2 ho = up0 - o_ref;
                    pass1(0, d_cur, e_cur);
                    s16x2 f = group_prev_or<G>(f_last, lead_bias, lmask), h = bias_c;
#pragma unroll
                    for (int q = 0; q < K; ++q) {
                        f = pk_max_h(f - e_ref, ho);
                        s16x2 d_next = bias_c, e_next = bias_c;
                        if (q + 1 < K) pass1(q + 1, d_next, e_next);
                        h = pk_max3_h(d_cur, e_cur, f);
                        Hl[q] = h;
                        ho = h - o_ref;
                        HOl[q] = ho;
                        if (q & 1) best = pk_max3_h(best, d_prev, d_cur);
                        else if (q == K - 1) best = pk_max_h(best, d_cur);
                        d_prev = d_cur;
                        d_cur = d_next;
                        e_cur = e_next;
                    }
                    h_last = h;
                    f_last = f;
                    code_ptr += 2;
                };
#pragma unroll
                for (int q = 0; q < K; ++q) {
                    Hl[q] = El[q] = bias_c;
                    HOl[q] = bias_c - o_ref;
                }
                up0 = h_last = f_last = best = bias_c;
                for (; t + 1 < steps; t += 2) {
                    biased_step(S0);
                    biased_step(S1);
                }
                if (t < steps) biased_step(S0);
                best = best - bias_c;
            }
        }
        if (!biased) {
            for (; t + 1 < steps; t += 2) {
                step(std::false_type{}, first_t{}, S0, S1);
                step(std::false_type{}, second_t{}, S1, S0);
            }
            if (t < steps) step(std::false_type{}, all_t{}, S0, S1);
        }
    } else {
        const int steps = F + G - 1;
        const int fill_end = G - 1 < steps ? G - 1 : steps;
        const int steady_end = F > fill_end ? F : fill_end;
        int t = 0;
        auto single = [&](auto masked_tag) __attribute__((always_inline)) { step(masked_tag, all_t{}, S0, S1); };
        for (; t < fill_end; ++t) single(std::true_type{});
        {
            for (; t + 1 < steady_end; t += 2) {
                step(std::false_type{}, first_t{}, S0, S1);
                step(std::false_type{}, second_t{}, S1, S0);
            }
        }
        for (; t < steady_end; ++t) single(std::false_type{});
        for (; t < steps; ++t) single(std::true_type{});
    }

    s16x2 res;
    if (LINF16_SW) {
        const f16x2 b = __builtin_bit_cast(f16x2, best);
        res = s16x2{(short)(int)((float)b.x * 1024.0f), (short)(int)((float)b.y * 1024.0f)};
    } else if (HALF) {
        f16x2 b = __builtin_bit_cast(f16x2, best);
        if (ALG == kAlgNW) {
            b = __builtin_bit_cast(f16x2, l == G - 1 ? row_best : cell(-rcentre));
#pragma unroll
            for (int q = 0; q < K; ++q)
                b = __builtin_elementwise_maximum(b, __builtin_bit_cast(f16x2, cell_sub(Hl[q], cell(tilt_row * (l * K + q) + tilt_col * F - centre + rcentre))));
            res = s16x2{(short)((int)b.x + rcentre), (short)((int)b.y + rcentre)};
        } else {
            res = s16x2{(short)(int)b.x, (short)(int)b.y};
        }
    } else if (ALG == kAlgSW) {
        res = best;
    } else {
        s16x2 col = l == G - 1 ? row_best : pk(0);
#pragma unroll
        for (int q = 0; q < K; ++q) col = pk_max(col, Hl[q] - cell(tilt_row * (l * K + q) + tilt_col * F));
        res = pk_max(col, pk(0));
    }
#pragma unroll
    for (int d = G / 2; d >= 1; d >>= 1)
        res = pk_max(res, as_pk((unsigned)__shfl_xor((int)as_u32(res), d, kWave)));
    if (l == 0) {
        const long long pa = pair0 + 2 * grp;
        if (pa + 1 < n_pairs && ((unsigned long long)scores & 3ull) == 0) {
            *reinterpret_cast<unsigned *>(scores + pa) = as_u32(res);
        } else {
            if (pa < n_pairs) scores[pa] = res.x;
            if (pa + 1 < n_pairs) scores[pa + 1] = res.y;
        }
    }
}

struct WaveLds {
    int prof_area, refc_stride, total;
};

template <int G, int K>
inline WaveLds wave_lds(int R, int F) {
    using geo = Geo<G, K>;
    WaveLds w;
    const int raw_refs = ((2 * F + 16 + 15) / 16) * 16;
    w.prof_area = geo::kProfBytes > raw_refs ? geo::kProfBytes : raw_refs;
    w.prof_area = ((w.prof_area + 15) / 16) * 16;
    w.refc_stride = ((2 * (F + 2 * kCodePad) + 15) / 16) * 16;
    w.total = w.prof_area + geo::kGroups * w.refc_stride + ((geo::kPairs * 8 + 15) / 16) * 16;
    return w;
}

inline WaveLds row_table_lds(int G, int R, int F) {
    const int groups = kWave / G, pairs = 2 * groups;
    WaveLds w;
    w.prof_area = ((pairs * F + 32 + 15) / 16) * 16;
    int stride_dw = F + 2 * row_table_pad(G);
    stride_dw += ((G - stride_dw) % 64 + 64) % 64;
    w.refc_stride = 4 * stride_dw;
    const int streams = groups * w.refc_stride, raw_reads = ((pairs * R + 32 + 15) / 16) * 16;
    w.total = w.prof_area + (streams > raw_reads ? streams : raw_reads);
    return w;
}

}
```

### versalignlib_amd/csrc/engine.hip.h

```cpp
#pragma once

#include <hip/hip_runtime.h>
#include <stdint.h>
#include <stdio.h>
#include <stdlib.h>
#include <string.h>

#include <algorithm>
#include <atomic>
#include <chrono>
#include <condition_variable>
#include <functional>
#include <map>
#include <memory>
#include <mutex>
#include <stdexcept>
#include <string>
#include <thread>
#include <utility>
#include <vector>

#include "align_parts.h"
#include "cell_rules.h"
#include "hip_handles.h"
#include "host_pipeline.h"
#include "kernel_instances.hip.h"
#include "band_kernels.hip.h"
#include "cigar_kernels.hip.h"
#include "long_kernels.hip.h"
#include "long_plan.h"
#include "pack_kernels.hip.h"
#include "ragged_kernels.hip.h"
#include "span_kernels.hip.h"
#include "span_cigar_kernels.hip.h"
#include "subopt_kernels.hip.h"
#include "strip_kernels.hip.h"
#include "strip_plan.h"

namespace valign {

#define VALIGN_DECLARE_FULL(G, K) VALIGN_FAST_KERNELS(extern template, G, K) VALIGN_FALLBACK_KERNELS(extern template, G, K)
#define VALIGN_DECLARE_FAST(G, K) VALIGN_FAST_KERNELS(extern template, G, K)
VALIGN_ALL_PARTS(VALIGN_DECLARE_FULL, VALIGN_DECLARE_FAST)
#undef VALIGN_DECLARE_FULL
#undef VALIGN_DECLARE_FAST

struct Geometry {
    int G, K;
    bool full;
    WaveLds (*lds)(int R, int F);
    const void *kernel[2][7];
    const void *fill[2][kFillKernels];
    const void *(*placed)(int track, int gaps);
    const void *(*subopt)(int track, int gaps);
    const void *(*extend)(int gaps);
};

template <int G, int K>
constexpr void set_fast_kernels(Geometry &g) {
    g.kernel[0][0] = (const void *)&score_kernel<G, K, kAlgSW, kGapLinear>;
    g.kernel[0][1] = (const void *)&score_kernel<G, K, kAlgSW, kGapSym>;
    g.kernel[0][2] = (const void *)&score_kernel<G, K, kAlgSW, kGapAffine>;
    g.kernel[0][3] = (const void *)&score_kernel<G, K, kAlgSW, kGapAffineSym>;
    g.kernel[0][4] = (const void *)&score_kernel<G, K, kAlgSW, kGapAffineSymF16>;
    g.kernel[0][5] = (const void *)&score_kernel<G, K, kAlgSW, kGapAffineF16>;
    g.kernel[0][6] = (const void *)&score_kernel<G, K, kAlgSW, kGapSymF16>;
    g.kernel[1][0] = (const void *)&score_kernel<G, K, kAlgNW, kGapLinear>;
    g.kernel[1][1] = (const void *)&score_kernel<G, K, kAlgNW, kGapSym>;
    g.kernel[1][2] = (const void *)&score_kernel<G, K, kAlgNW, kGapAffine>;
    g.kernel[1][3] = (const void *)&score_kernel<G, K, kAlgNW, kGapAffineSym>;
    g.kernel[1][4] = (const void *)&score_kernel<G, K, kAlgNW, kGapAffineSymF16>;
    g.kernel[1][5] = (const void *)&score_kernel<G, K, kAlgNW, kGapAffineF16>;
    g.kernel[1][6] = (const void *)&score_kernel<G, K, kAlgNW, kGapSymF16>;
    g.fill[0][kFillTagKey] = (const void *)&align_fill_tag_kernel<G, K, kAlgSW, true, false>;
    g.fill[0][kFillTagProfKey] = (const void *)&align_fill_tag_kernel<G, K, kAlgSW, true, false, false, true>;
    g.fill[0][kFillAffineTagSym] = (const void *)&align_fill_affine_tag_kernel<G, K, kAlgSW, true>;
    g.fill[1][kFillTag] = (const void *)&align_fill_tag_kernel<G, K, kAlgNW, false, false>;
    g.fill[1][kFillAffineTagSym] = (const void *)&align_fill_affine_tag_kernel<G, K, kAlgNW, true>;
}

template <int G, int K>
constexpr Geometry fast_geometry() {
    Geometry g{G, K, false, &wave_lds<G, K>, {}, {}, &placed_kernel<G, K, false>, &subopt_kernel<G, K, false>, &extend_kernel<G, K, false>};
    set_fast_kernels<G, K>(g);
    return g;
}

template <int G, int K>
constexpr Geometry full_geometry() {
    Geometry g{G, K, true, &wave_lds<G, K>, {}, {}, &placed_kernel<G, K, true>, &subopt_kernel<G, K, true>, &extend_kernel<G, K, true>};
    set_fast_kernels<G, K>(g);
    g.fill[0][kFillLinear] = (const void *)&align_fill_kernel<G, K, kAlgSW, false>;
    g.fill[0][kFillLinearSym] = (const void *)&align_fill_kernel<G, K, kAlgSW, true>;
    g.fill[0][kFillAffine] = (const void *)&align_fill_affine_kernel<G, K, kAlgSW, false>;
    g.fill[0][kFillAffineSym] = (const void *)&align_fill_affine_kernel<G, K, kAlgSW, true>;
    g.fill[0][kFillSse] = (const void *)&align_fill_sse_kernel<G, K, kAlgSW>;
    g.fill[0][kFillTag] = (const void *)&align_fill_tag_kernel<G, K, kAlgSW, false, false>;
    g.fill[0][kFillSseTag] = (const void *)&align_fill_tag_kernel<G, K, kAlgSW, false, true>;
    g.fill[1][kFillLinear] = (const void *)&align_fill_kernel<G, K, kAlgNW, false>;
    g.fill[1][kFillLinearSym] = (const void *)&align_fill_kernel<G, K, kAlgNW, true>;
    g.fill[1][kFillAffine] = (const void *)&align_fill_affine_kernel<G, K, kAlgNW, false>;
    g.fill[1][kFillAffineSym] = (const void *)&align_fill_affine_kernel<G, K, kAlgNW, true>;
    g.fill[1][kFillSse] = (const void *)&align_fill_sse_kernel<G, K, kAlgNW>;
    g.fill[0][kFillSseTagKey] = (const void *)&align_fill_tag_kernel<G, K, kAlgSW, true, true>;
    g.fill[0][kFillAffineTag] = (const void *)&align_fill_affine_tag_kernel<G, K, kAlgSW, false>;
    g.fill[1][kFillSseTag] = (const void *)&align_fill_tag_kernel<G, K, kAlgNW, false, true>;
    g.fill[1][kFillAffineTag] = (const void *)&align_fill_affine_tag_kernel<G, K, kAlgNW, false>;
    return g;
}

static const Geometry kGeometries[] = {
    fast_geometry<8, 4>(),   fast_geometry<8, 6>(),   full_geometry<8, 8>(),   fast_geometry<16, 4>(),
    fast_geometry<8, 10>(),  fast_geometry<8, 12>(),  fast_geometry<16, 8>(),  full_geometry<16, 10>(),
    fast_geometry<16, 12>(), fast_geometry<32, 8>(),  full_geometry<32, 10>(), fast_geometry<32, 12>(),
    full_geometry<64, 8>(),  fast_geometry<64, 12>(), full_geometry<64, 16>(), fast_geometry<64, 24>(),
    full_geometry<64, 32>(),
};
constexpr int kNumGeometries = sizeof(kGeometries) / sizeof(kGeometries[0]);
#define VALIGN_COUNT(G, K) +1
static_assert(kNumGeometries == 0 VALIGN_ALL_PARTS(VALIGN_COUNT, VALIGN_COUNT), "kernel_instances.hip.h lists other geometries than this table");
#undef VALIGN_COUNT

constexpr int kMaxBlockLds = 160 * 1024;
constexpr int kSlots = 4;
constexpr int kDefaultBlockLds = 64 * 1024;

struct LaunchPlan {
    bool long_mode = false;
    const Geometry *geo = nullptr;
    WaveLds lds{};
    int waves_per_block = 4;
    int pairs_per_wave = 0;
};

class DebugSwitches {
public:
    DebugSwitches() {
        const char *env = getenv("VALIGN_HIP_DEBUG");
        if (!env) return;
        static const char *const known[] = {"no_sym", "no_tag", "no_f16", "no_max3", "no_tilt", "no_row_tables", "no_fused", "no_prof_key", "no_overlap", "no_band_chain",
                                            "force_long", "wide_align", "strip_k", "no_single_strip", "no_direct_out", "ragged_min", "chunk_bytes",
                                            "align_chunk_bytes", "direct_bytes", "scratch_cap_mb", "whole_rows", "short_strips", "cigar_rows_mb", "cigar_lanes",
                                            "span_scratch_bytes", "subopt_scratch_bytes", "span_cigar_mb"};
        std::string s(env);
        for (size_t at = 0; at <= s.size();) {
            const size_t end = std::min(s.find(',', at), s.size());
            const std::string item = s.substr(at, end - at);
            at = end + 1;
            if (item.empty()) continue;
            const size_t eq = item.find('=');
            const std::string name = item.substr(0, eq);
            bool ok = false;
            for (const char *k : known) ok = ok || name == k;
            if (!ok) throw std::runtime_error("VALIGN_HIP_DEBUG: unknown switch '" + name + "'");
            kv_[name] = eq == std::string::npos ? 1 : atoll(item.c_str() + eq + 1);
        }
    }
    bool on(const char *name) const { return kv_.count(name) != 0; }
    long long value(const char *name, long long fallback) const {
        auto it = kv_.find(name);
        return it == kv_.end() ? fallback : it->second;
    }

private:
    std::map<std::string, long long> kv_;
};

}

#include "host_runtime.hip.h"

namespace valign {

class Engine {
public:
    struct LengthGroup {
        int R = 0, F = 0;
        long long pairs = 0, pair_ofs = 0;
        size_t read_ofs = 0, ref_ofs = 0;
    };
    struct HostStats {
        int launches = 0;
        double cells_swept = 0, cells_padded = 0;
        double gather_ms = 0, wait_ms = 0, drain_ms = 0;
        double classify_ms = 0;
        double launch_ms = 0;
        int packed = 0;
        int direct_out = 0;
        int direct = 0;
        double d2h_row_bytes = 0, full_row_bytes = 0;
    };

    Engine(int device, int R, int F, const Scoring &sc, int force_g, int force_k);

    ~Engine();

    void set_band_width(int diagonals) {
        if (diagonals < 0) throw std::runtime_error("band_width must be >= 0");
        band_width_ = diagonals;
        plan_ = (diagonals > 0 && !base_plan_.long_mode) ? long_plan() : base_plan_;
        band_plan_ = band_chain_plan(R_, F_, band_width_, sc_.affine);
    }
    int band_width() const { return band_width_; }
    void set_band_alignments(int on) {
        if (on != 0 && on != 1) throw std::runtime_error("band_alignments must be 0 or 1");
        band_alignments_ = on == 1;
    }
    int band_alignments() const { return band_alignments_ ? 1 : 0; }
    void set_band_nw(int on) {
        if (on != 0 && on != 1) throw std::runtime_error("band_nw must be 0 or 1");
        band_nw_ = on == 1;
    }
    int band_nw() const { return band_nw_ ? 1 : 0; }
    void set_band_placed(int on) {
        if (on != 0 && on != 1) throw std::runtime_error("band_placed must be 0 or 1");
        band_placed_ = on == 1;
    }
    int band_placed() const { return band_placed_ ? 1 : 0; }
    void set_placed_wide(int on) {
        if (on != 0 && on != 1) throw std::runtime_error("placed_wide must be 0 or 1");
        placed_wide_ = on == 1;
    }
    int placed_wide() const { return placed_wide_ ? 1 : 0; }
    void set_extend_wide(int on) {
        if (on != 0 && on != 1) throw std::runtime_error("extend_wide must be 0 or 1");
        extend_wide_ = on == 1;
    }
    int extend_wide() const { return extend_wide_ ? 1 : 0; }
    void set_trace_checkpoints(int on) {
        if (on != 0 && on != 1) throw std::runtime_error("trace_checkpoints must be 0 or 1");
        trace_checkpoints_ = on == 1;
    }
    int trace_checkpoints() const { return trace_checkpoints_ ? 1 : 0; }
    void band_block_shape(int &block_rows, int &col_align) const;
    void set_score_width(int bits) {
        if (bits != 0 && bits != 16 && bits != 32) throw std::runtime_error("score_width must be 0, 16 or 32");
        score_width_ = bits;
    }
    void set_traceback_policy(int policy) {
        if (policy != 0 && policy != 1) throw std::runtime_error("traceback_policy must be 0 (default) or 1 (sse)");
        sse_policy_ = policy == 1;
    }
    void set_ragged_batching(int mode) {
        if (mode < 0 || mode > 2) throw std::runtime_error("ragged_batching must be 0, 1 or 2");
        ragged_ = mode;
    }
    void set_host_packing(int mode) {
        if (mode != 0 && mode != 1) throw std::runtime_error("host_packing must be 0 or 1");
        pack_ = mode == 1;
    }
    void set_half_float_cells(int mode) {
        if (mode != 0 && mode != 1) throw std::runtime_error("half_float_cells must be 0 or 1");
        no_f16_ = mode == 0 || dbg_.on("no_f16");
    }
    void set_pointer_scratch_cap_mb(long long mb) {
        if (mb < 0) throw std::runtime_error("pointer_scratch_cap_mb must be >= 0");
        if (mb > 0) scratch_cap_mb_ = mb;
    }
    int device() const { return device_; }
    int read_length() const { return R_; }
    int ref_length() const { return F_; }
    const LaunchPlan &plan() const { return plan_; }
    hipStream_t own_stream() const { return streams_[0].get(); }

    void score_device(int opt, long long n, const uint8_t *d_reads, const uint8_t *d_refs,
                      int16_t *d_scores, hipStream_t stream, bool length_sorted = true);

    void launch_score(const LaunchPlan &plan, int alg, int R, int F, long long n, const uint8_t *d_reads,
                      const uint8_t *d_refs, int16_t *d_scores, hipStream_t stream,
                      const LengthGroup *groups = nullptr, int n_groups = 0);


    void launch_unpack(const uint8_t *d_packed, uint8_t *d_out, long long n, int len, hipStream_t stream);

    LongFacts long_facts(int alg) const {
        return LongFacts{band_width_, band_nw_, score_wide_cells(alg), dbg_.on("short_strips"), dbg_.on("no_single_strip"), no_band_chain_, band_plan_.usable};
    }
    LongScoreMode long_mode(int alg, bool refuse) const { return long_score_mode(rule_inputs(), alg, long_facts(alg), refuse); }

    void score_long_device(int alg, long long n, const uint8_t *d_reads, const uint8_t *d_refs, int16_t *d_scores, hipStream_t stream);
    void sync_band_tables(hipStream_t stream);
    void score_band_device(const LongScoreMode &mode, long long n, const uint8_t *d_reads, const uint8_t *d_refs, int16_t *d_scores, PlacedRec *d_placed,
                           hipStream_t stream);

    const char *score_cell_format(int alg, long long n = 0) const;
    std::string ran_score_cells() const;
    const char *ran_align_fill() const { return ran_align_fill_; }
    static std::string ran_geometry(const Geometry *g) { return g ? std::to_string(g->G) + "x" + std::to_string(g->K) : "none"; }
    std::string ran_kernels() const;

    RuleInputs rule_inputs() const {
        RuleInputs in = RuleInputs{sc_, R_, F_, sse_policy_, no_sym_, no_tag_, no_f16_, no_prof_key_, no_max3_, no_tilt_};
        in.no_row_tables = no_row_tables_;
        return in;
    }
    bool score_int16_ok(int alg) const;
    bool score_wide_cells(int alg) const { return score_width_ == 32 || (score_width_ == 0 && !score_int16_ok(alg)); }

    void score_host(int opt, int n, const char *const *reads, const char *const *refs, short *scores,
                    int threads, int16_t *d_dest = nullptr);



    struct WalkChain {
        int region;
        long long chunk_pairs;
        int *min_start;
        uint8_t *packed;
    };
    hipEvent_t trace_done(int region) const { return trace_done_[region].get(); }
    const LaunchPlan &align_plan_for(int alg, FillChoice &choice);
    const LaunchPlan &align_base_plan() const {
        if (plan_.long_mode && align_resident_.geo && !align_resident_.long_mode && R_ <= 1024 && align_resident_.lds.total <= 140 * 1024) {
            const int wpb = align_resident_.waves_per_block;
            const int waves_per_cu = (kMaxBlockLds / std::max(1, align_resident_.lds.total * wpb)) * wpb;
            if (waves_per_cu >= 2 || !sc_.affine) return align_resident_;
        }
        return plan_;
    }

    bool align_device(int opt, long long n, const uint8_t *d_reads, const uint8_t *d_refs, uint8_t *d_rows,
                      short *d_idx, hipStream_t stream, const WalkChain *chain = nullptr);

    void ensure_trace_stream();

    RouteFacts route_facts(bool small_call) const;

    bool align_fused(int alg, long long n, const uint8_t *d_reads, const uint8_t *d_refs, uint8_t *d_rows, short *d_idx,
                     hipStream_t stream);

    void align_strips_device(const StripMode &mode, long long n, const uint8_t *d_reads, const uint8_t *d_refs, uint8_t *d_rows, short *d_idx,
                             hipStream_t stream);
    bool align_banded() const { return band_alignments_ && band_width_ > 0; }

    using FlatSink = valign::FlatSink;

    template <typename Sink>
    void align_host(int opt, int n, const char *const *reads, const char *const *refs, Sink alignments,
                    int threads);

    void align_cigar_device(int opt, long long n, const uint8_t *d_reads, const uint8_t *d_refs, int extended, CigarRec *d_recs,
                            unsigned *d_ops, int ops_stride, hipStream_t stream);
    bool align_cigar_host(int opt, int n, const char *const *reads, const char *const *refs, int extended, CigarRec *recs,
                          unsigned *ops, long long ops_cap, long long *offsets, long long *ops_needed, int threads);

    void score_placed_device(int opt, long long n, const uint8_t *d_reads, const uint8_t *d_refs, PlacedRec *d_placed, hipStream_t stream);
    void score_placed_host(int opt, int n, const char *const *reads, const char *const *refs, PlacedRec *placed, int threads);
    PlacedFacts placed_facts() const;
    const LaunchPlan &placed_plan_for(int alg, PlacedChoice &choice, int &gaps);
    const char *ran_placed() const { return ran_placed_; }

    void score_span_device(int opt, long long n, const uint8_t *d_reads, const uint8_t *d_refs, SpanRec *d_spans, hipStream_t stream);
    void score_span_host(int opt, int n, const char *const *reads, const char *const *refs, SpanRec *spans, int threads);
    const char *ran_span() const { return ran_span_.c_str(); }

    void align_span_device(int opt, long long n, const uint8_t *d_reads, const uint8_t *d_refs, int extended, CigarRec *d_recs, unsigned *d_ops,
                           int ops_stride, hipStream_t stream);
    bool align_span_host(int opt, int n, const char *const *reads, const char *const *refs, int extended, CigarRec *recs, unsigned *ops,
                         long long ops_cap, long long *offsets, long long *ops_needed, int threads);
    const char *ran_span_cigar() const { return ran_span_cigar_.c_str(); }

    void score_subopt_device(int opt, long long n, const uint8_t *d_reads, const uint8_t *d_refs, int mask, SuboptRec *d_subopt, hipStream_t stream);
    void score_subopt_host(int opt, int n, const char *const *reads, const char *const *refs, int mask, SuboptRec *subopt, int threads);
    const char *ran_subopt() const { return ran_subopt_; }

    void score_extend_device(int opt, long long n, const uint8_t *d_reads, const uint8_t *d_refs, ExtendRec *d_extend, hipStream_t stream);
    void score_extend_host(int opt, int n, const char *const *reads, const char *const *refs, ExtendRec *extend, int threads);
    const char *ran_extend() const { return ran_extend_; }

    std::string host_phases() const;

    std::string describe(int opt, long long n) const;

private:
    void validate_scoring();

    template <class A>
    void put_scoring(A &a) const {
        a.match = (short)sc_.match;
        a.mismatch = (short)sc_.mismatch;
        a.gap_read = (short)sc_.gap_read;
        a.gap_ref = (short)sc_.gap_ref;
        a.open_read = (short)sc_.open_read;
        a.ext_read = (short)sc_.ext_read;
        a.open_ref = (short)sc_.open_ref;
        a.ext_ref = (short)sc_.ext_ref;
    }

    template <class A>
    void put_sweep(A &a, const uint8_t *d_reads, const uint8_t *d_refs, long long n, int blocks8) const {
        a.reads = d_reads;
        a.refs = d_refs;
        a.n = n;
        a.R = R_;
        a.F = F_;
        a.blocks8 = blocks8;
        put_scoring(a);
    }
    template <class A>
    void put_lds(A &a, const WaveLds &lds) const {
        a.prof_area = lds.prof_area;
        a.refc_stride = lds.refc_stride;
        a.wave_lds = lds.total;
    }
    template <class A>
    void put_sweep(A &a, const uint8_t *d_reads, const uint8_t *d_refs, long long n, int blocks8, const WaveLds &lds) const {
        put_sweep(a, d_reads, d_refs, n, blocks8);
        put_lds(a, lds);
    }
    StripArgs strip_args(const uint8_t *d_reads, const uint8_t *d_refs, long long n, const StripPlan &plan, const WaveLds &lds, int s, unsigned *scratch,
                         size_t top, size_t bottom, size_t f_rows, EndCell *ends, const int *first_bad) const {
        StripArgs a{};
        put_sweep(a, d_reads, d_refs, n, plan.blocks8, lds);
        a.ends = ends;
        a.first_bad = first_bad;
        a.top = scratch + top;
        a.bottom = scratch + bottom;
        a.top_f = a.top + f_rows;
        a.bottom_f = a.bottom + f_rows;
        a.strip = s;
        a.strips = plan.strips;
        a.row_dwords = plan.row_dwords;
        a.band = plan.band;
        return a;
    }
    struct PlacedSweep {
        using ChunkStep = std::function<void(const StripArgs &a, long long begin, hipStream_t stream)>;
        const void *fn;
        WaveLds lds;
        StripPlan plan;
        bool first_bad;
        const char *rows_label, *what;
        ChunkStep close;
        size_t pair_bytes = sizeof(EndCell);
        std::function<void(StripArgs &a, long long pairs)> bind;
        ChunkStep open;
    };
    PlacedSweep placed_strip_sweep(PlacedRec *d_placed) const;
    PlacedSweep placed_wide_sweep(PlacedRec *d_placed) const;
    PlacedSweep::ChunkStep placed_records_step(PlacedRec *d_placed, bool wide) const;
    PlacedSweep extend_wide_sweep(ExtendRec *d_extend) const;
    void score_placed_strips(const PlacedSweep &sweep, long long n, const uint8_t *d_reads, const uint8_t *d_refs, hipStream_t stream);
    static void raise_block_lds(const void *fn, int bytes) {
        if (bytes > kDefaultBlockLds)
            hip_check(hipFuncSetAttribute(fn, hipFuncAttributeMaxDynamicSharedMemorySize, bytes), "hipFuncSetAttribute(MaxDynamicSharedMemorySize)");
    }
    TraceArgs trace_args(int alg, const uint8_t *d_reads, const uint8_t *d_refs, long long n, const unsigned *ptr, const EndCell *ends, uint8_t *rows,
                         short *idx, int G, int K, int pad_rows, int blocks8) const;

    LaunchPlan choose_plan(int R, int F, int force_g, int force_k, bool latency = false, bool full_only = false) const;

    static LaunchPlan long_plan();


    long long whole_rounds(long long pairs) const;

    bool direct_call(long long n, size_t per_pair) const;

    void prime_copy_engines(hipStream_t copy_in, hipStream_t copy_out, long long staged_pairs);

    void flat_destination(FlatSink sink, long long n, uint8_t *&rows, short *&idx) const {
        if (HostRegistry::instance().covers(sink.rows, (size_t)n * 2 * sink.AL) &&
            HostRegistry::instance().covers(sink.idx, sizeof(short) * 4 * (size_t)n)) {
            rows = sink.rows;
            idx = sink.idx;
        }
    }
    template <typename AlignmentT>
    void flat_destination(AlignmentT *, long long, uint8_t *&, short *&) const {}

    static uint8_t *dev_view(void *pinned) {
        void *d = nullptr;
        hip_check(hipHostGetDevicePointer(&d, pinned, 0), "hipHostGetDevicePointer");
        return (uint8_t *)d;
    }

    void reset_pipeline();

    void ensure_trace_scratch(long long pairs, size_t bytes_per_pp, long long ppw, hipStream_t stream);

    void ensure_align_staging(long long pairs);

    struct CigarSink {
        CigarRec *recs;
        unsigned *ops;
        int ops_stride, extended;
        const PlacedRec *fwd = nullptr;
        int fwd_ref_length = 0;
    };
    void launch_cigar(hipStream_t stream, const uint8_t *rows, const short *idx, const EndCell *ends, long long begin, long long cnt);
    void launch_cigar_args(hipStream_t stream, CigarArgs &a);
    void ensure_cigar_scratch(int slots, long long pairs, hipStream_t stream);
    void launch_cigar_scan(const CigarRec *recs, long long *offsets, long long n, hipStream_t stream);

    template <typename Sink>
    void scatter(Sink sink, long long cnt, const uint8_t *rows, const short *idx, int threads, size_t first_col = 0) {
        packer_.scatter(sink, cnt, rows, idx, threads, first_col);
    }

    void ensure_staging(long long pairs);

    long long host_chunk_pairs(bool shared_scratch, long long n) const;
    void stage_chunk(int slot, hipStream_t stream, const char *const *reads, const char *const *refs, long long cnt, int threads);
    void wait_slot(int slot, const std::function<void(int)> &drain);
    struct RecordKind {
        size_t bytes;
        const char *label, *d2h;
    };
    using ChunkLaunch = std::function<void(int slot, long long cnt, const uint8_t *d_reads, const uint8_t *d_refs, uint8_t *d_records, hipStream_t stream)>;
    void record_pipeline(long long n, const char *const *reads, const char *const *refs, void *out, const RecordKind &kind, long long chunk, bool one_stream,
                         int threads, const ChunkLaunch &launch);
    void ensure_record_staging(long long pairs, const RecordKind &kind);

    struct SpanCtx {
        long long cap = 0;
        DeviceBuffer<uint8_t> rev_reads, rev_refs;
        DeviceBuffer<PlacedRec> fwd, rev;
        size_t bytes() const { return rev_reads.bytes() + rev_refs.bytes() + fwd.bytes() + rev.bytes(); }
    };
    Engine &span_prepare(int alg, bool &strips);
    long long span_chunk_pairs(long long n) const;
    void ensure_span_scratch(int c, long long pairs, hipStream_t stream);
    void span_chunk(int c, int opt, long long n, const uint8_t *d_reads, const uint8_t *d_refs, SpanRec *d_spans, hipStream_t stream);
    void launch_span_reverse(long long n, const uint8_t *d_reads, const uint8_t *d_refs, const PlacedRec *fwd, uint8_t *rev_reads, uint8_t *rev_refs,
                             int Fr, hipStream_t stream);

    struct SpanCigarCtx {
        long long cap = 0;
        DeviceBuffer<uint8_t> rev_reads, rev_refs, rows;
        DeviceBuffer<PlacedRec> fwd;
        DeviceBuffer<short> idx;
        DeviceBuffer<CigarRec> recs;
        DeviceBuffer<long long> offsets;
        DeviceBuffer<uint8_t> out;
        PinnedBuffer<uint8_t> h_out;
        PinnedBuffer<long long> h_total;
        size_t bytes() const { return rev_reads.bytes() + rev_refs.bytes() + rows.bytes() + fwd.bytes() + idx.bytes(); }
    };
    Engine &span_cigar_prepare(int alg);
    long long span_cigar_chunk_pairs(long long n) const;
    void ensure_span_cigar_scratch(int c, long long pairs, bool host, hipStream_t stream);
    void span_cigar_chunk(int c, int opt, long long n, const uint8_t *d_reads, const uint8_t *d_refs, const CigarSink &sink, hipStream_t stream);
    void launch_span_cigar(hipStream_t stream, const uint8_t *rows, const short *idx, long long begin, long long cnt);
    void launch_span_cigar_args(hipStream_t stream, SpanCigarArgs &a);

    struct SuboptCtx {
        DeviceBuffer<unsigned> colmax;
        DeviceBuffer<PlacedRec> placed;
        size_t bytes() const { return colmax.bytes() + placed.bytes(); }
    };
    LaunchPlan subopt_plan_for(int alg, int mask, PlacedChoice &choice, int &gaps);
    long long subopt_chunk_pairs(const LaunchPlan &plan, long long n) const;
    void ensure_subopt_scratch(int c, const LaunchPlan &plan, long long pairs, hipStream_t stream);
    void subopt_chunk(int c, const LaunchPlan &plan, int track, int gaps, long long n, const uint8_t *d_reads, const uint8_t *d_refs, int mask,
                      SuboptRec *d_subopt, hipStream_t stream);

    const LaunchPlan &extend_plan_for(int alg, int &gaps, PlacedRoute &route);


    static double ms_between(std::chrono::steady_clock::time_point a, std::chrono::steady_clock::time_point b) {
        return std::chrono::duration<double, std::milli>(b - a).count();
    }

    bool ragged_applies(int alg) const;

    double sampled_cell_fraction(const char *const *reads, const char *const *refs, long long n) const;

    void build_length_classes();

    const LaunchPlan &class_plan(int R, int F);

    static int trimmed_length(const unsigned char *s, int len);

    template <typename Fn>
    void for_ranges(int threads, long long cnt, long long serial_below, Fn fn) {
        packer_.for_ranges(threads, cnt, serial_below, fn);
    }

    struct RaggedCtx {
        long long cap = 0;
        EventHandle counted;
        DeviceBuffer<uint8_t> reads, refs;
        DeviceBuffer<int16_t> scores;
        DeviceBuffer<uint16_t> bin;
        DeviceBuffer<int> pos;
        DeviceBuffer<RaggedPlace> place;
        DeviceBuffer<unsigned> counters;
        DeviceBuffer<uint8_t> tables;
        PinnedBuffer<unsigned> h_counts;
        PinnedBuffer<uint8_t> h_tables;
        const uint8_t *src_reads = nullptr, *src_refs = nullptr;
    };
    static constexpr size_t kRaggedTableBytes = sizeof(uint16_t) * kRaggedMaxBins + sizeof(RaggedGroupDev) * kRaggedMaxGroups;

    int ragged_bins() const { return (int)(read_caps_.size() * ref_caps_.size()); }
    bool ragged_fits(long long n) const {
        return ragged_bins() <= kRaggedMaxBins && read_caps_.size() * (size_t)kMaxScoreGroups <= (size_t)kRaggedMaxGroups &&
               n < 0x7FFFFFFFll;
    }

    void ensure_ragged(int c, long long n);

    void ragged_begin(int c, long long n, const uint8_t *d_reads, const uint8_t *d_refs, hipStream_t stream);

    std::vector<LengthGroup> fold_groups(std::vector<long long> &total, std::vector<int> &group_of_bin) const;

    bool ragged_finish(int c, int alg, long long n, int16_t *d_scores, hipStream_t stream, bool always);

    void gather(const char *const *reads, const char *const *refs, long long cnt, uint8_t *dst_reads,
                uint8_t *dst_refs, int threads) {
        packer_.gather(reads, refs, cnt, dst_reads, dst_refs, threads);
    }

    int device_, R_, F_;
    Scoring sc_;
    bool sse_policy_ = false;
    int band_width_ = 0;
    bool band_alignments_ = false;
    bool band_nw_ = false;
    bool band_placed_ = false;
    bool placed_wide_ = false;
    bool extend_wide_ = false;
    bool trace_checkpoints_ = false;
    int score_width_ = 0;
    int ragged_ = 0, force_g_ = 0, force_k_ = 0;
    size_t score_chunk_bytes_ = 48u << 20;
    size_t align_chunk_bytes_ = 128u << 20;
    size_t direct_bytes_ = 768u << 10;
    long long ragged_min_ = 2048;
    std::vector<int> read_caps_, ref_caps_;
    std::vector<unsigned char> read_class_;
    std::vector<unsigned short> ref_class_;
    std::map<std::pair<int, int>, LaunchPlan> class_plans_;
    hipStream_t ragged_dev_stream_ = nullptr;
    HostPacker packer_{R_, F_};
    HostStats host_stats_;
    DebugSwitches dbg_;
    bool no_sym_ = dbg_.on("no_sym");
    bool no_tag_ = dbg_.on("no_tag");
    bool no_f16_ = dbg_.on("no_f16");
    bool no_max3_ = dbg_.on("no_max3");
    bool no_tilt_ = dbg_.on("no_tilt");
    bool no_row_tables_ = dbg_.on("no_row_tables");
    bool no_fused_ = dbg_.on("no_fused");
    bool no_prof_key_ = dbg_.on("no_prof_key");
    bool copy_engines_primed_ = false;
    std::unique_ptr<CopyIssuer> copy_issuer_;
    bool wide_align_ = dbg_.on("wide_align");
    bool whole_rows_ = dbg_.on("whole_rows");
    bool no_direct_out_ = dbg_.on("no_direct_out");
    bool no_overlap_ = dbg_.on("no_overlap");
    int strip_k_ = (int)dbg_.value("strip_k", 0);
    long long scratch_cap_mb_ = dbg_.value("scratch_cap_mb", 0);
    bool chain_regions_busy_[2] = {false, false};
    std::string arch_;
    LaunchPlan plan_, latency_plan_;
    LaunchPlan base_plan_;
    LaunchPlan align_resident_;
    LaunchPlan fallback_plan_;
    long long slot_begin_[kSlots] = {}, slot_pending_[kSlots] = {};
    long long staged_pairs_ = 0, align_staged_pairs_ = 0;
    size_t record_staged_bytes_ = 0;
    bool pack_ = true;
    BandPlan band_plan_;
    int band_tables_width_ = -1;
    int band_blocks_per_cu_ = 0, band_lds_ = 0;
    int long_strip_rows_ = 0;
    static constexpr unsigned kRanF16 = 1, kRanInt16 = 2, kRanInt32 = 4;
    unsigned ran_score_cells_ = 0;
    const char *ran_align_fill_ = "none";
    const Geometry *ran_score_geo_ = nullptr, *ran_align_geo_ = nullptr;
    const Geometry *ran_placed_geo_ = nullptr, *ran_subopt_geo_ = nullptr, *ran_extend_geo_ = nullptr;
    const char *ran_score_sym_affine_ = nullptr;
    const char *ran_score_sym_affine_frame_ = "plain";
    const char *ran_score_sym_affine_scores_ = "lds_profile";
    const char *ran_placed_ = "none";
    std::string ran_span_ = "none";
    size_t span_scratch_bytes_ = (size_t)dbg_.value("span_scratch_bytes", 256ll << 20);
    std::string ran_span_cigar_ = "none";
    size_t span_cigar_bytes_ = (size_t)std::max(0ll, dbg_.value("span_cigar_mb", 768)) << 20;
    const char *ran_subopt_ = "none";
    int subopt_ring_cols_ = 0;
    size_t subopt_scratch_bytes_ = (size_t)dbg_.value("subopt_scratch_bytes", 256ll << 20);
    const char *ran_extend_ = "none";
    const char *ran_result_format_ = "rows";
    long long cigar_d2h_bytes_ = 0;
    const CigarSink *cigar_ = nullptr;
    long long cigar_pairs_[2] = {0, 0};
    long long align_ptr_bytes_per_pair_ = 0;
    long long align_ckpt_bytes_per_pair_ = 0;
    int cu_count_ = 0;
    bool no_band_chain_ = dbg_.on("no_band_chain");
    int start_col_[kSlots] = {};

    StreamHandle streams_[kSlots];
    EventHandle slot_done_[kSlots];
    EventHandle in_done_[kSlots], kernels_done_[kSlots];
    StreamHandle trace_stream_;
    EventHandle fill_done_[2], trace_done_[2], entry_ev_;
    EventHandle ragged_dev_done_;
    PinnedBuffer<uint8_t> h_reads_[kSlots], h_refs_[kSlots];
    PinnedBuffer<short> h_scores_[kSlots];
    DeviceBuffer<uint8_t> d_reads_[kSlots], d_refs_[kSlots];
    DeviceBuffer<int16_t> d_scores_[kSlots];
    DeviceBuffer<uint8_t> d_pack_reads_[kSlots], d_pack_refs_[kSlots];
    DeviceBuffer<unsigned> d_ptr_;
    DeviceBuffer<EndCell> d_ends_;
    DeviceBuffer<int> d_first_bad_;
    PinnedBuffer<uint8_t> h_rows_[kSlots];
    PinnedBuffer<short> h_idx_[kSlots];
    DeviceBuffer<uint8_t> d_rows_[kSlots];
    DeviceBuffer<short> d_idx_[kSlots];
    DeviceBuffer<uint8_t> d_packed_rows_[kSlots];
    DeviceBuffer<uint8_t> d_cig_rows_[2];
    DeviceBuffer<short> d_cig_idx_[2];
    DeviceBuffer<CigarRec> d_cig_recs_[2];
    DeviceBuffer<long long> d_cig_offsets_[2];
    DeviceBuffer<uint8_t> d_cig_out_[2];
    PinnedBuffer<uint8_t> h_cig_out_[2];
    PinnedBuffer<long long> h_cig_total_;
    DeviceBuffer<int> d_min_start_;
    PinnedBuffer<int> h_min_start_;
    PinnedBuffer<uint8_t> h_records_[kSlots];
    DeviceBuffer<uint8_t> d_records_[kSlots];
    DeviceBuffer<unsigned> d_placed_rows_;
    DeviceBuffer<EndCell> d_placed_ends_;
    DeviceBuffer<int> d_placed_bad_;
    SpanCtx span_[kSlots + 1];
    std::unique_ptr<Engine> span_child_;
    SpanCigarCtx span_cigar_[2];
    SuboptCtx subopt_[kSlots + 1];
    DeviceBuffer<unsigned> d_brow_;
    DeviceBuffer<BandBlock> d_band_blocks_;
    DeviceBuffer<int> d_band_fill_;
    RaggedCtx rag_[kSlots + 1];
    DeviceBuffer<uint8_t> d_read_class_;
    DeviceBuffer<uint16_t> d_ref_class_;
};

}
```

### versalignlib_amd/csrc/engine_core.hip

```cpp
#include "engine.hip.h"

namespace valign {

Engine::Engine(int device, int R, int F, const Scoring &sc, int force_g, int force_k)
    : device_(device), R_(R), F_(F), sc_(sc) {
    if (R < 0 || F < 0) throw std::runtime_error("negative sequence length");
    if ((long long)R + F > 32767)
        throw std::runtime_error("read_length + ref_length exceeds the ABI's 16-bit coordinates");
    validate_scoring();
    int count = 0;
    hip_check(hipGetDeviceCount(&count), "hipGetDeviceCount");
    if (device < 0 || device >= count)
        throw std::runtime_error("HIP device " + std::to_string(device) + " not present (" +
                                 std::to_string(count) + " visible): libHIPKernel.so has no CPU path");
    hip_check(hipSetDevice(device_), "hipSetDevice");
    hipDeviceProp_t prop;
    hip_check(hipGetDeviceProperties(&prop, device_), "hipGetDeviceProperties");
    arch_ = prop.gcnArchName;
    cu_count_ = prop.multiProcessorCount;
    if (arch_.find("gfx950") == std::string::npos)
        throw std::runtime_error("device is " + arch_ + "; this library carries gfx950 code only");
    force_g_ = force_g;
    force_k_ = force_k;
    plan_ = choose_plan(R_, F_, force_g, force_k);
    align_resident_ = plan_;
    if (!force_g && !force_k && !plan_.long_mode && plan_.geo && plan_.geo->G * plan_.geo->K > 1536) plan_ = long_plan();
    if (!force_g && !force_k && !plan_.long_mode && plan_.geo) {
        const int waves_per_cu = std::min(32, (kMaxBlockLds / std::max(1, plan_.lds.total * plan_.waves_per_block)) * plan_.waves_per_block);
        const int strip_rows = kLongG * kLongK;
        const bool pads_alike = R_ <= 1024 && ((R_ + strip_rows - 1) / strip_rows) * strip_rows * 100 <= plan_.geo->G * plan_.geo->K * 115;
        if (waves_per_cu <= 1 || (waves_per_cu <= 2 && (!sc_.affine || pads_alike)) || (waves_per_cu <= 4 && pads_alike)) plan_ = long_plan();
    }
    base_plan_ = plan_;
    latency_plan_ = (force_g || force_k || plan_.long_mode) ? plan_ : choose_plan(R_, F_, 0, 0, true);
    build_length_classes();
    for (int s = 0; s < kSlots; ++s) streams_[s] = make_stream();
    for (int s = 0; s < kSlots; ++s) {
        slot_done_[s] = make_event(hipEventDisableTiming);
        in_done_[s] = make_event(hipEventDisableTiming);
        kernels_done_[s] = make_event(hipEventDisableTiming | hipEventBlockingSync);
    }
}

Engine::~Engine() {
    copy_issuer_.reset();
    (void)hipSetDevice(device_);
    if (trace_stream_) (void)hipStreamSynchronize(trace_stream_.get());
}

const char *Engine::score_cell_format(int alg, long long n) const {
    if (alg > 1) return "none";
    if (plan_.long_mode || band_width_ > 0 || score_wide_cells(alg)) return long_cells_name(long_mode(alg, false).cells);
    const LaunchPlan &plan = (n > 0 && n <= (long long)latency_plan_.pairs_per_wave * 1024 && band_width_ == 0) ? latency_plan_ : plan_;
    return gap_form_f16(score_gap_form(rule_inputs(), alg, R_, F_, plan.geo->G * plan.geo->K)) ? "f16" : "int16";
}

std::string Engine::ran_score_cells() const {
    if (!ran_score_cells_) return "none";
    std::string s;
    for (const auto &f : {std::make_pair(kRanF16, "f16"), std::make_pair(kRanInt16, "int16"), std::make_pair(kRanInt32, "int32")})
        if (ran_score_cells_ & f.first) s += (s.empty() ? "" : "+") + std::string(f.second);
    return s;
}

std::string Engine::ran_kernels() const {
    return "{\"ran_score_cells\": \"" + ran_score_cells() + "\", \"ran_align_fill\": \"" + ran_align_fill_ + "\"}";
}

bool Engine::score_int16_ok(int alg) const {
    int rows = 0;
    if (!plan_.long_mode && plan_.geo) rows = plan_.geo->G * plan_.geo->K;
    if (latency_plan_.geo && !latency_plan_.long_mode) rows = std::max(rows, latency_plan_.geo->G * latency_plan_.geo->K);
    return int16_range_ok(rule_inputs(), alg, true, plan_.long_mode, rows);
}

std::string Engine::host_phases() const {
    char buf[320];
    snprintf(buf, sizeof buf, "{\"host_gather_ms\": %.3f, \"host_wait_ms\": %.3f, \"host_drain_ms\": %.3f, \"host_classify_ms\": %.3f, \"host_launch_ms\": %.3f, \"d2h_row_mb\": %.1f, \"full_row_mb\": %.1f}",
             host_stats_.gather_ms, host_stats_.wait_ms, host_stats_.drain_ms, host_stats_.classify_ms, host_stats_.launch_ms,
             host_stats_.d2h_row_bytes / 1e6, host_stats_.full_row_bytes / 1e6);
    return buf;
}

std::string Engine::describe(int opt, long long n) const {
    const long long ppb = (long long)plan_.pairs_per_wave * plan_.waves_per_block;
    int band_rows = 0, band_align = 0;
    band_block_shape(band_rows, band_align);
    char buf[4096];
    snprintf(buf, sizeof buf,
             "{\"arch\": \"%s\", \"device\": %d, \"alg\": %d, \"affine\": %d, \"group_lanes\": %d, "
             "\"rows_per_lane\": %d, \"padded_rows\": %d, \"pairs_per_wave\": %d, \"waves_per_block\": %d, "
             "\"lds_per_wave\": %d, \"lds_per_block\": %d, \"steps\": %d, \"blocks\": %lld, \"long_mode\": %d, "
             "\"band_width\": %d, \"ragged_batching\": %d, \"ragged_launches\": %d, \"ragged_cell_fraction\": %.4f, "
             "\"score_cells\": \"%s\", \"direct_call\": %d, \"packed_classes\": %d, \"direct_out\": %d, \"band_block_rows\": %d, \"band_col_align\": %d, \"band_waves_per_cu\": %d, \"band_lds_per_wave\": %d, \"band_cells_per_pair\": %lld, \"long_strip_rows\": %d, \"d2h_row_mb\": %.1f, \"full_row_mb\": %.1f, \"host_gather_ms\": %.3f, \"host_classify_ms\": %.3f, \"host_wait_ms\": %.3f, \"host_drain_ms\": %.3f, \"ran_score_cells\": \"%s\", \"ran_align_fill\": \"%s\", "
             "\"band_alignments\": %d, \"band_nw\": %d, \"band_placed\": %d, \"align_ptr_bytes_per_pair\": %lld, \"trace_checkpoints\": %d, "
             "\"align_ckpt_bytes_per_pair\": %lld, \"align_scratch_bytes\": %lld, \"ran_result_format\": \"%s\", "
             "\"cigar_d2h_bytes\": %lld, \"cigar_rows_scratch_bytes\": %lld, \"ran_placed\": \"%s\", \"placed_wide\": %d, \"placed_scratch_bytes\": %lld, "
             "\"ran_span\": \"%s\", \"span_ref_length\": %lld, \"span_scratch_bytes\": %lld, "
             "\"ran_span_cigar\": \"%s\", \"span_cigar_scratch_bytes\": %lld, "
             "\"ran_subopt\": \"%s\", \"subopt_scratch_bytes\": %lld, \"subopt_ring_cols\": %d, \"ran_extend\": \"%s\", \"extend_wide\": %d, "
             "\"ran_score_geometry\": \"%s\", \"ran_align_geometry\": \"%s\", "
             "\"ran_placed_geometry\": \"%s\", \"ran_subopt_geometry\": \"%s\", \"ran_extend_geometry\": \"%s\"}",
             arch_.c_str(), device_, opt & 0xF, sc_.affine ? 1 : 0, plan_.geo->G, plan_.geo->K,
             plan_.geo->G * plan_.geo->K, plan_.pairs_per_wave, plan_.waves_per_block, plan_.lds.total,
             plan_.lds.total * plan_.waves_per_block, F_ + plan_.geo->G - 1, n > 0 ? (n + ppb - 1) / ppb : 0,
             plan_.long_mode ? 1 : 0, band_width_, ragged_, host_stats_.launches,
             host_stats_.cells_padded > 0 ? host_stats_.cells_swept / host_stats_.cells_padded : 1.0,
             score_cell_format(opt & 0xF, n), host_stats_.direct, host_stats_.packed, host_stats_.direct_out,
             ((opt & 0xF) == kAlgSW || band_nw_) ? band_rows : VALIGN_HIP_BAND_BLOCK_ROWS, ((opt & 0xF) == kAlgSW || band_nw_) ? band_align : VALIGN_HIP_BAND_COL_ALIGN,
             band_blocks_per_cu_, band_lds_, (band_tables_width_ == band_width_ && band_plan_.usable) ? band_plan_.cells : 0ll, long_strip_rows_, host_stats_.d2h_row_bytes / 1e6, host_stats_.full_row_bytes / 1e6, host_stats_.gather_ms, host_stats_.classify_ms, host_stats_.wait_ms,
             host_stats_.drain_ms, ran_score_cells().c_str(), ran_align_fill_, band_alignments(), band_nw(), band_placed(), align_ptr_bytes_per_pair_, trace_checkpoints(),
             align_ckpt_bytes_per_pair_, (long long)d_ptr_.bytes(), ran_result_format_, cigar_d2h_bytes_,
             (long long)(d_cig_rows_[0].bytes() + d_cig_rows_[1].bytes()), ran_placed_, placed_wide(), (long long)(d_placed_rows_.bytes() + d_placed_ends_.bytes()),
             ran_span_.c_str(), span_ref_length(rule_inputs()), (long long)span_[kSlots].bytes(),
             ran_span_cigar_.c_str(), (long long)(span_cigar_[0].bytes() + span_cigar_[1].bytes()),
             ran_subopt_, (long long)subopt_[kSlots].bytes(), subopt_ring_cols_, ran_extend_, extend_wide(),
             ran_geometry(ran_score_geo_).c_str(), ran_geometry(ran_align_geo_).c_str(),
             ran_geometry(ran_placed_geo_).c_str(), ran_geometry(ran_subopt_geo_).c_str(), ran_geometry(ran_extend_geo_).c_str());
    std::string out(buf);
    if (ran_score_sym_affine_)
        out.insert(out.size() - 1, std::string(", \"ran_score_sym_affine\": \"") + ran_score_sym_affine_ + "\", \"ran_score_sym_affine_frame\": \"" +
                                       ran_score_sym_affine_frame_ + "\", \"ran_score_sym_affine_scores\": \"" + ran_score_sym_affine_scores_ + "\"");
    return out;
}

void Engine::band_block_shape(int &block_rows, int &col_align) const {
    const bool chain = long_mode(kAlgSW, false).chain;
    block_rows = chain ? kBandK : VALIGN_HIP_BAND_BLOCK_ROWS;
    col_align = chain ? VALIGN_HIP_BAND_CHAIN_COL_ALIGN : VALIGN_HIP_BAND_COL_ALIGN;
}

void Engine::validate_scoring() {
    auto fits = [](int v) { return v >= -32768 && v <= 32767; };
    if (!fits(sc_.match) || !fits(sc_.mismatch) || !fits(sc_.gap_read) || !fits(sc_.gap_ref) ||
        !fits(sc_.open_read) || !fits(sc_.ext_read) || !fits(sc_.open_ref) || !fits(sc_.ext_ref))
        throw std::runtime_error("scoring parameter outside int16");
    const bool gaps_ok = sc_.affine ? (sc_.open_read <= 0 && sc_.ext_read <= 0 && sc_.open_ref <= 0 && sc_.ext_ref <= 0)
                                    : (sc_.gap_read <= 0 && sc_.gap_ref <= 0);
    if (!gaps_ok) throw std::runtime_error("positive gap scores are not supported by the HIP kernels");
    if (sc_.affine && (sc_.ext_read < sc_.open_read || sc_.ext_ref < sc_.open_ref))
        throw std::runtime_error("affine gap scores need extend >= open in each direction (an extension dearer "
                                 "than the opening is not an affine model)");
}

LaunchPlan Engine::choose_plan(int R, int F, int force_g, int force_k, bool latency, bool full_only) const {
    LaunchPlan best;
    double best_cost = 0;
    for (int i = 0; i < kNumGeometries; ++i) {
        const Geometry &g = kGeometries[i];
        if (g.G * g.K < R) continue;
        if (full_only && !g.full) continue;
        if (force_g && (g.G != force_g || (force_k && g.K != force_k))) continue;
        if (!force_g && force_k && g.K != force_k) continue;
        LaunchPlan p;
        p.geo = &g;
        p.lds = g.lds(R, F);
        p.pairs_per_wave = 2 * (kWave / g.G);
        int best_waves = 0;
        if (p.lds.total * 8 <= kMaxBlockLds) {
            p.waves_per_block = 4;
            best_waves = std::min(32, (kMaxBlockLds / (p.lds.total * 4)) * 4);
        } else {
            for (int wpb = 4; wpb >= 1; wpb >>= 1) {
                if (p.lds.total * wpb > kMaxBlockLds) continue;
                const int resident = std::min(32, (kMaxBlockLds / (p.lds.total * wpb)) * wpb);
                if (resident > best_waves && (best_waves == 0 || 2 * resident >= 3 * best_waves)) {
                    best_waves = resident;
                    p.waves_per_block = wpb;
                }
            }
        }
        if (best_waves == 0) continue;
        double per_step = g.K * (sc_.affine ? 9.3 : 5.6) + 7.0;
        if (g.K > 10) per_step *= 1.0 + 0.06 * (g.K - 10);
        double cost = (double)(F + g.G - 1) * per_step * g.G / 2.0;
        if (best_waves < 8) cost *= 1.0 + 0.08 * (8 - best_waves);
        if (latency) cost = (double)(F + g.G - 1) * (g.K * (sc_.affine ? 9.3 : 5.6) + 7.0);
        if (!best.geo || cost < best_cost) {
            best = p;
            best_cost = cost;
        }
    }
    if (!best.geo || (dbg_.on("force_long") && !force_g)) {
        if (force_g || force_k)
            throw std::runtime_error("the forced kernel geometry does not fit read_length=" + std::to_string(R) +
                                     ", ref_length=" + std::to_string(F));
        return long_plan();
    }
    return best;
}

LaunchPlan Engine::long_plan() {
    LaunchPlan p;
    p.long_mode = true;
    p.pairs_per_wave = 2 * (kWave / kLongG);
    p.waves_per_block = 1;
    p.lds.total = LongLds<kLongG, kLongK>::kTotal;
    for (int i = 0; i < kNumGeometries; ++i)
        if (kGeometries[i].G == kLongG && kGeometries[i].K == kLongK) p.geo = &kGeometries[i];
    return p;
}

long long Engine::whole_rounds(long long pairs) const {
    if (plan_.long_mode || !plan_.geo || cu_count_ <= 0) return pairs;
    const long long waves_per_cu = std::min<long long>(32, (kMaxBlockLds / std::max(1, plan_.lds.total * plan_.waves_per_block)) * plan_.waves_per_block);
    const long long round_pairs = std::max<long long>(1, waves_per_cu) * cu_count_ * plan_.pairs_per_wave;
    return pairs >= round_pairs ? pairs / round_pairs * round_pairs : pairs;
}

bool Engine::direct_call(long long n, size_t per_pair) const {
    return direct_bytes_ > 0 && (size_t)n * per_pair <= direct_bytes_ && n <= staged_pairs_;
}

void Engine::reset_pipeline() {
    bool stale = false;
    for (int s = 0; s < kSlots; ++s) stale = stale || slot_pending_[s] != 0;
    if (!stale) return;
    if (copy_issuer_) {
        try {
            copy_issuer_->wait_idle();
        } catch (...) {
        }
    }
    if (trace_stream_) (void)hipStreamSynchronize(trace_stream_.get());
    for (int s = 0; s < kSlots; ++s) {
        (void)hipStreamSynchronize(streams_[s].get());
        slot_pending_[s] = 0;
        slot_begin_[s] = 0;
    }
}

void Engine::ensure_staging(long long pairs) {
    if (pairs <= staged_pairs_) return;
    staged_pairs_ = 0;
    for (int s = 0; s < kSlots; ++s) {
        h_reads_[s].reset();
        h_refs_[s].reset();
        h_scores_[s].reset();
        d_reads_[s].reset();
        d_refs_[s].reset();
        d_scores_[s].reset();
        d_pack_reads_[s].reset();
        d_pack_refs_[s].reset();
    }
    for (int s = 0; s < kSlots; ++s) {
        h_reads_[s].reserve(std::max<size_t>((size_t)pairs * R_, 16));
        h_refs_[s].reserve(std::max<size_t>((size_t)pairs * F_, 16));
        h_scores_[s].reserve(sizeof(short) * (size_t)pairs);
        d_reads_[s].reserve(std::max<size_t>((size_t)pairs * R_, 16));
        d_refs_[s].reserve(std::max<size_t>((size_t)pairs * F_, 16));
        d_scores_[s].reserve(sizeof(short) * (size_t)pairs);
        d_pack_reads_[s].reserve(std::max<size_t>((size_t)pairs * packed_length(R_), 16));
        d_pack_refs_[s].reserve(std::max<size_t>((size_t)pairs * packed_length(F_), 16));
    }
    staged_pairs_ = pairs;
}

void Engine::build_length_classes() {
    std::vector<int> caps;
    for (int i = 0; i < kNumGeometries; ++i) {
        const int rows = kGeometries[i].G * kGeometries[i].K;
        if (rows < R_) caps.push_back(rows);
    }
    caps.push_back(R_);
    std::sort(caps.begin(), caps.end());
    caps.erase(std::unique(caps.begin(), caps.end()), caps.end());
    read_caps_ = caps;
    ref_caps_.clear();
    const int width = 64 * std::max(1, (F_ + 64 * kMaxScoreGroups - 1) / (64 * kMaxScoreGroups));
    for (int c = width; c < F_; c += width) ref_caps_.push_back(c);
    ref_caps_.push_back(F_);
    read_class_.assign((size_t)R_ + 1, 0);
    for (int len = 0, c = 0; len <= R_; ++len) {
        while (read_caps_[c] < len) ++c;
        read_class_[len] = (unsigned char)c;
    }
    ref_class_.assign((size_t)F_ + 1, 0);
    for (int len = 0, c = 0; len <= F_; ++len) {
        while (ref_caps_[c] < len) ++c;
        ref_class_[len] = (unsigned short)c;
    }
    ragged_min_ = std::max(1ll, dbg_.value("ragged_min", ragged_min_));
    score_chunk_bytes_ = (size_t)std::max(4096ll, dbg_.value("chunk_bytes", (long long)score_chunk_bytes_));
    align_chunk_bytes_ = (size_t)std::max(4096ll, dbg_.value("align_chunk_bytes", (long long)align_chunk_bytes_));
    direct_bytes_ = (size_t)std::max(0ll, dbg_.value("direct_bytes", (long long)direct_bytes_));
}

const LaunchPlan &Engine::class_plan(int R, int F) {
    const std::pair<int, int> key(R, F);
    auto it = class_plans_.find(key);
    if (it == class_plans_.end()) it = class_plans_.emplace(key, choose_plan(R, F, 0, 0)).first;
    return it->second;
}

int Engine::trimmed_length(const unsigned char *s, int len) {
    static const struct Table {
        bool acgt[256] = {};
        Table() { for (const char *p = "ACGTacgt"; *p; ++p) acgt[(unsigned char)*p] = true; }
    } table;
    while (len >= 8) {
        uint64_t tail;
        memcpy(&tail, s + len - 8, 8);
        if (tail != 0) break;
        len -= 8;
    }
    while (len > 0 && !table.acgt[s[len - 1]]) --len;
    return len;
}

}
```

### versalignlib_amd/csrc/engine_score.hip

```cpp
#define VALIGN_TU_SCORE 1
#include "engine.hip.h"

namespace valign {

void Engine::score_device(int opt, long long n, const uint8_t *d_reads, const uint8_t *d_refs,
                  int16_t *d_scores, hipStream_t stream, bool length_sorted) {
    const int alg = opt & 0xF;
    if (alg > 1 || n <= 0) return;
    hip_check(hipSetDevice(device_), "hipSetDevice");
    if (length_sorted) {
        host_stats_ = HostStats{};
        ran_score_cells_ = 0;
        ran_score_geo_ = nullptr;
        ran_score_sym_affine_ = nullptr;
    }
    if (score_width_ == 16 && !score_int16_ok(alg))
        throw std::runtime_error("shape x scoring can leave the int16 range of the DP cells (read_length " +
                                 std::to_string(R_) + ", ref_length " + std::to_string(F_) + ")");
    const bool wide = score_wide_cells(alg);
    if (plan_.long_mode || wide) {
        score_long_device(alg, n, d_reads, d_refs, d_scores, stream);
        return;
    }
    if (length_sorted && ragged_applies(alg) && ragged_fits(n) && n >= 2 * ragged_min_) {
        if (ragged_dev_done_ && ragged_dev_stream_ != stream)
            hip_check(hipEventSynchronize(ragged_dev_done_.get()), "hipEventSynchronize(previous length-sorted call)");
        if (!ragged_dev_done_) ragged_dev_done_ = make_event(hipEventDisableTiming);
        ragged_dev_stream_ = stream;
        ragged_begin(kSlots, n, d_reads, d_refs, stream);
        const bool swept = ragged_finish(kSlots, alg, n, d_scores, stream, ragged_ == 2);
        hip_check(hipEventRecord(ragged_dev_done_.get(), stream), "hipEventRecord");
        if (swept) return;
    }
    const bool few = n <= (long long)latency_plan_.pairs_per_wave * 1024 && band_width_ == 0;
    launch_score(few ? latency_plan_ : plan_, alg, R_, F_, n, d_reads, d_refs, d_scores, stream);
}

void Engine::launch_score(const LaunchPlan &plan, int alg, int R, int F, long long n, const uint8_t *d_reads,
                  const uint8_t *d_refs, int16_t *d_scores, hipStream_t stream,
                  const LengthGroup *groups, int n_groups) {
    ScoreArgs a;
    a.reads = d_reads;
    a.refs = d_refs;
    a.scores = d_scores;
    a.n = n;
    a.R = R;
    a.F = F;
    a.n_groups = n_groups;
    const long long pairs_per_block = (long long)plan.pairs_per_wave * plan.waves_per_block;
    long long blocks = (n + pairs_per_block - 1) / pairs_per_block;
    if (n_groups > 0) {
        if (n_groups > kMaxScoreGroups) throw std::runtime_error("too many length groups for one launch");
        blocks = 0;
        for (int g = 0; g < n_groups; ++g) {
            blocks += (groups[g].pairs + pairs_per_block - 1) / pairs_per_block;
            if (blocks > 0x7FFFFFFFll) throw std::runtime_error("batch too large for one launch");
            a.groups[g].block_end = (unsigned)blocks;
            a.groups[g].F = groups[g].F;
            a.groups[g].n = groups[g].pairs;
            a.groups[g].pair_ofs = groups[g].pair_ofs;
            a.groups[g].read_ofs = (long long)groups[g].read_ofs;
            a.groups[g].ref_ofs = (long long)groups[g].ref_ofs;
        }
    }
    a.prof_area = plan.lds.prof_area;
    a.refc_stride = plan.lds.refc_stride;
    a.wave_lds = plan.lds.total;
    put_scoring(a);
    const int gaps = score_gap_form(rule_inputs(), alg, R, F, plan.geo->G * plan.geo->K);
    const void *fn = plan.geo->kernel[alg][gaps];
    ran_score_cells_ |= gap_form_f16(gaps) ? kRanF16 : kRanInt16;
    ran_score_geo_ = plan.geo;
    if (alg == kAlgSW && gaps == kGapAffineSym) {
        const bool max3 = sym_affine_max3_ok(rule_inputs(), R_, F_);
        a.sym_max3_bias = max3 ? sym_affine_bias(sc_) : 0;
        const bool tilted = sym_affine_tilt_ok(rule_inputs(), R_, F_, plan.geo->G * plan.geo->K, plan.geo->K);
        if (tilted) a.sym_max3_bias = sym_affine_tilt_bias(sc_) | 1 << 16;
        const WaveLds tables_lds = row_table_lds(plan.geo->G, R, F);
        const bool row_tables = tilted && sym_affine_row_tables_ok(rule_inputs(), R_, F_, plan.geo->G * plan.geo->K, plan.geo->K, plan.lds.total, tables_lds.total);
        if (row_tables) {
            a.sym_max3_bias |= 1 << 17;
            a.prof_area = tables_lds.prof_area;
            a.refc_stride = tables_lds.refc_stride;
            a.wave_lds = tables_lds.total;
        }
        ran_score_sym_affine_ = ran_sym_affine_name(max3);
        ran_score_sym_affine_frame_ = ran_sym_affine_frame_name(tilted);
        ran_score_sym_affine_scores_ = ran_sym_affine_scores_name(row_tables);
    }
    const int block_lds = a.wave_lds * plan.waves_per_block;
    if (block_lds > kDefaultBlockLds)
        hip_check(hipFuncSetAttribute(fn, hipFuncAttributeMaxDynamicSharedMemorySize, block_lds),
                  "hipFuncSetAttribute(MaxDynamicSharedMemorySize)");
    if (blocks > 0x7FFFFFFFll) throw std::runtime_error("batch too large for one launch");
    if (blocks == 0) return;
    void *kargs[] = {&a};
    hip_check(hipLaunchKernel(fn, dim3((unsigned)blocks), dim3(plan.waves_per_block * kWave), kargs,
                              (size_t)block_lds, stream),
              "hipLaunchKernel(score_kernel)");
}

void Engine::launch_unpack(const uint8_t *d_packed, uint8_t *d_out, long long n, int len, hipStream_t stream) {
    if (n <= 0 || len <= 0) return;
    UnpackArgs a{d_packed, d_out, n, len};
    void *kargs[] = {&a};
    const bool even = (len & 1) == 0;
    const long long items = even ? (n * (long long)(len / 2) + 7) / 8 : n * (long long)((len + 1) / 2);
    const long long blocks = (items + 255) / 256;
    if (blocks > 0x7FFFFFFFll) throw std::runtime_error("batch too large for one launch");
    hip_check(hipLaunchKernel(even ? (const void *)&unpack_even_kernel : (const void *)&unpack_odd_kernel, dim3((unsigned)blocks),
                              dim3(256), kargs, 0, stream),
              "hipLaunchKernel(unpack_kernel)");
}

long long Engine::host_chunk_pairs(bool shared_scratch, long long n) const {
    const size_t per_pair = (size_t)R_ + F_;
    const size_t chunk_bytes = shared_scratch && !dbg_.on("chunk_bytes") ? std::max<size_t>(score_chunk_bytes_, 192u << 20) : score_chunk_bytes_;
    long long chunk = per_pair ? (long long)(chunk_bytes / per_pair) : n;
    chunk = whole_rounds(chunk);
    chunk = std::max<long long>(chunk, 1024);
    return std::min<long long>(chunk, n);
}

void Engine::stage_chunk(int slot, hipStream_t st, const char *const *reads, const char *const *refs, long long cnt, int threads) {
    const auto t0 = std::chrono::steady_clock::now();
    uint8_t *h_reads = h_reads_[slot].get(), *h_refs = h_refs_[slot].get(), *d_reads = d_reads_[slot].get(), *d_refs = d_refs_[slot].get();
    if (pack_) {
        const size_t PR = packed_length(R_), PF = packed_length(F_);
        packer_.gather_packed(reads, refs, cnt, h_reads, h_refs, threads);
        host_stats_.gather_ms += ms_between(t0, std::chrono::steady_clock::now());
        hip_check(hipMemcpyAsync(d_pack_reads_[slot].get(), h_reads, (size_t)cnt * PR, hipMemcpyHostToDevice, st), "H2D reads (classes)");
        hip_check(hipMemcpyAsync(d_pack_refs_[slot].get(), h_refs, (size_t)cnt * PF, hipMemcpyHostToDevice, st), "H2D refs (classes)");
        launch_unpack(d_pack_reads_[slot].get(), d_reads, cnt, R_, st);
        launch_unpack(d_pack_refs_[slot].get(), d_refs, cnt, F_, st);
        host_stats_.packed = 1;
    } else {
        gather(reads, refs, cnt, h_reads, h_refs, threads);
        host_stats_.gather_ms += ms_between(t0, std::chrono::steady_clock::now());
        hip_check(hipMemcpyAsync(d_reads, h_reads, (size_t)cnt * R_, hipMemcpyHostToDevice, st), "H2D reads");
        hip_check(hipMemcpyAsync(d_refs, h_refs, (size_t)cnt * F_, hipMemcpyHostToDevice, st), "H2D refs");
    }
}

void Engine::wait_slot(int slot, const std::function<void(int)> &drain) {
    const auto t0 = std::chrono::steady_clock::now();
    hip_check(hipEventSynchronize(slot_done_[slot].get()), "hipEventSynchronize");
    const auto t1 = std::chrono::steady_clock::now();
    drain(slot);
    host_stats_.wait_ms += ms_between(t0, t1);
    host_stats_.drain_ms += ms_between(t1, std::chrono::steady_clock::now());
}

void Engine::ensure_record_staging(long long pairs, const RecordKind &kind) {
    const size_t bytes = kind.bytes * (size_t)pairs;
    if (bytes <= record_staged_bytes_) return;
    record_staged_bytes_ = 0;
    for (int s = 0; s < kSlots; ++s) {
        h_records_[s].reset();
        d_records_[s].reset();
    }
    for (int s = 0; s < kSlots; ++s) {
        h_records_[s].reserve(bytes);
        d_records_[s].reserve(bytes, kind.label);
    }
    record_staged_bytes_ = bytes;
}

void Engine::record_pipeline(long long n, const char *const *reads, const char *const *refs, void *out, const RecordKind &kind, long long chunk,
                             bool one_stream, int threads, const ChunkLaunch &launch) {
    const size_t per_pair = (size_t)R_ + F_;
    reset_pipeline();
    ensure_staging(chunk);
    ensure_record_staging(chunk, kind);
    threads = std::min(std::max(threads, 1), 64);
    host_stats_ = HostStats{};
    if (direct_call(n, per_pair)) {
        auto t0 = std::chrono::steady_clock::now();
        gather(reads, refs, n, h_reads_[0].get(), h_refs_[0].get(), threads);
        auto t1 = std::chrono::steady_clock::now();
        launch(0, n, dev_view(h_reads_[0].get()), dev_view(h_refs_[0].get()), dev_view(h_records_[0].get()), streams_[0].get());
        hip_check(hipStreamSynchronize(streams_[0].get()), "hipStreamSynchronize");
        auto t2 = std::chrono::steady_clock::now();
        memcpy(out, h_records_[0].get(), kind.bytes * (size_t)n);
        host_stats_.gather_ms = ms_between(t0, t1);
        host_stats_.wait_ms = ms_between(t1, t2);
        host_stats_.drain_ms = ms_between(t2, std::chrono::steady_clock::now());
        host_stats_.direct = 1;
        return;
    }
    const std::function<void(int)> drain = [&](int s) {
        if (slot_pending_[s] <= 0) return;
        memcpy((uint8_t *)out + kind.bytes * (size_t)slot_begin_[s], h_records_[s].get(), kind.bytes * (size_t)slot_pending_[s]);
        slot_pending_[s] = 0;
    };
    int slot = 0;
    for (long long begin = 0; begin < n; begin += chunk, slot = (slot + 1) % kSlots) {
        const long long cnt = std::min<long long>(chunk, n - begin);
        wait_slot(slot, drain);
        hipStream_t st = streams_[one_stream ? 0 : slot].get();
        stage_chunk(slot, st, reads + begin, refs + begin, cnt, threads);
        launch(slot, cnt, d_reads_[slot].get(), d_refs_[slot].get(), d_records_[slot].get(), st);
        hip_check(hipMemcpyAsync(h_records_[slot].get(), d_records_[slot].get(), kind.bytes * (size_t)cnt, hipMemcpyDeviceToHost, st), kind.d2h);
        hip_check(hipEventRecord(slot_done_[slot].get(), st), "hipEventRecord");
        slot_begin_[slot] = begin;
        slot_pending_[slot] = cnt;
    }
    for (int k = 0; k < kSlots; ++k) wait_slot((slot + k) % kSlots, drain);
}

void Engine::score_host(int opt, int n, const char *const *reads, const char *const *refs, short *scores,
                int threads, int16_t *d_dest) {
    const int alg = opt & 0xF;
    if (alg > 1 || n <= 0) return;
    hip_check(hipSetDevice(device_), "hipSetDevice");
    ran_score_cells_ = 0;
    ran_score_geo_ = nullptr;
    ran_score_sym_affine_ = nullptr;
    const size_t per_pair = (size_t)R_ + F_;
    const bool shared_scratch = (plan_.long_mode || score_wide_cells(alg)) && long_mode(alg, false).brow;
    const bool strips_in_turn = plan_.long_mode && shared_scratch;
    const long long chunk = host_chunk_pairs(strips_in_turn, n);
    reset_pipeline();
    ensure_staging(chunk);
    if (threads < 1) threads = 1;
    threads = std::min(threads, 64);
    if (direct_call(n, per_pair) && (!ragged_applies(alg) || d_dest)) {
        host_stats_ = HostStats{};
        auto t0 = std::chrono::steady_clock::now();
        gather(reads, refs, n, h_reads_[0].get(), h_refs_[0].get(), threads);
        auto t1 = std::chrono::steady_clock::now();
        score_device(opt, n, dev_view(h_reads_[0].get()), dev_view(h_refs_[0].get()), d_dest ? d_dest : (int16_t *)dev_view(h_scores_[0].get()),
                     streams_[0].get());
        hip_check(hipStreamSynchronize(streams_[0].get()), "hipStreamSynchronize");
        auto t2 = std::chrono::steady_clock::now();
        if (!d_dest) memcpy(scores, h_scores_[0].get(), sizeof(short) * (size_t)n);
        host_stats_.gather_ms = ms_between(t0, t1);
        host_stats_.wait_ms = ms_between(t1, t2);
        host_stats_.drain_ms = ms_between(t2, std::chrono::steady_clock::now());
        host_stats_.direct = 1;
        return;
    }
    const bool ragged = !d_dest && ragged_applies(alg) && ragged_fits(chunk) &&
                        (ragged_ == 2 || sampled_cell_fraction(reads, refs, n) < 0.67);
    host_stats_ = HostStats{};
    const std::function<void(int)> drain = [&](int s) {
        if (slot_pending_[s] <= 0) return;
        if (d_dest) {
            slot_pending_[s] = 0;
            return;
        }
        memcpy(scores + slot_begin_[s], h_scores_[s].get(), sizeof(short) * (size_t)slot_pending_[s]);
        slot_pending_[s] = 0;
    };
    auto finish_chunk = [&](int s, long long pairs) {
        hipStream_t cs = streams_[shared_scratch ? 0 : s].get();
        if (ragged) (void)ragged_finish(s, alg, pairs, d_scores_[s].get(), cs, true);
        if (!d_dest)
            hip_check(hipMemcpyAsync(h_scores_[s].get(), d_scores_[s].get(), sizeof(short) * (size_t)pairs, hipMemcpyDeviceToHost, cs), "D2H scores");
        hip_check(hipEventRecord(slot_done_[s].get(), cs), "hipEventRecord");
    };
    struct OpenChunk {
        int slot;
        long long pairs;
    };
    std::vector<OpenChunk> open;
    constexpr size_t kOpenChunks = 2;
    int slot = 0;
    long long chunk_no = 0, cnt = 0;
    for (long long begin = 0; begin < n; begin += cnt, slot = (slot + 1) % kSlots, ++chunk_no) {
        const long long ramp = (n > 2 * chunk) ? (chunk_no == 0 ? whole_rounds(chunk / 4) : (chunk_no == 1 ? whole_rounds(chunk / 2) : chunk)) : chunk;
        cnt = std::min<long long>(std::max<long long>(ramp, 1024), n - begin);
        wait_slot(slot, drain);
        hipStream_t st = streams_[shared_scratch ? 0 : slot].get();
        stage_chunk(slot, st, reads + begin, refs + begin, cnt, threads);
        const uint8_t *d_reads = d_reads_[slot].get(), *d_refs = d_refs_[slot].get();
        if (!ragged) {
            score_device(opt, cnt, d_reads, d_refs, d_dest ? d_dest + begin : d_scores_[slot].get(), st, false);
            finish_chunk(slot, cnt);
        } else {
            ragged_begin(slot, cnt, d_reads, d_refs, st);
            open.push_back(OpenChunk{slot, cnt});
            if (open.size() > kOpenChunks) {
                finish_chunk(open.front().slot, open.front().pairs);
                open.erase(open.begin());
            }
        }
        slot_begin_[slot] = begin;
        slot_pending_[slot] = cnt;
    }
    for (const OpenChunk &c : open) finish_chunk(c.slot, c.pairs);
    for (int k = 0; k < kSlots; ++k) wait_slot((slot + k) % kSlots, drain);
}

bool Engine::ragged_applies(int alg) const {
    return ragged_ && alg <= kAlgNW && !plan_.long_mode && !force_g_ && !force_k_ && score_width_ != 32 &&
           R_ > 0 && F_ > 0 && score_int16_ok(alg);
}

double Engine::sampled_cell_fraction(const char *const *reads, const char *const *refs, long long n) const {
    const long long samples = std::min<long long>(n, 256);
    double swept = 0;
    for (long long k = 0; k < samples; ++k) {
        const long long i = k * n / samples;
        const int r = read_caps_[read_class_[trimmed_length((const unsigned char *)reads[i], R_)]];
        const int f = ref_caps_[ref_class_[trimmed_length((const unsigned char *)refs[i], F_)]];
        swept += (double)r * f;
    }
    return swept / ((double)samples * R_ * F_);
}

void Engine::ensure_ragged(int c, long long n) {
    RaggedCtx &x = rag_[c];
    if (!d_ref_class_.get()) {
        d_read_class_.reserve(read_class_.size(), "read classes");
        d_ref_class_.reserve(sizeof(uint16_t) * ref_class_.size(), "ref classes");
        hip_check(hipMemcpy(d_read_class_.get(), read_class_.data(), read_class_.size(), hipMemcpyHostToDevice), "hipMemcpy");
        hip_check(hipMemcpy(d_ref_class_.get(), ref_class_.data(), sizeof(uint16_t) * ref_class_.size(), hipMemcpyHostToDevice), "hipMemcpy");
    }
    if (!x.counted) x.counted = make_event(hipEventDisableTiming);
    x.counters.reserve(sizeof(unsigned) * (kRaggedMaxBins + kRaggedMaxGroups), "ragged counters");
    x.tables.reserve(kRaggedTableBytes, "ragged tables");
    x.h_counts.reserve(sizeof(unsigned) * kRaggedMaxBins);
    x.h_tables.reserve(kRaggedTableBytes);
    if (x.cap >= n) return;
    x.cap = 0;
    x.reads.reset();
    x.refs.reset();
    x.scores.reset();
    x.bin.reset();
    x.pos.reset();
    x.place.reset();
    x.reads.reserve(std::max<size_t>((size_t)n * R_, 16), "ragged reads");
    x.refs.reserve(std::max<size_t>((size_t)n * F_, 16), "ragged refs");
    x.scores.reserve(sizeof(int16_t) * (size_t)n, "ragged scores");
    x.bin.reserve(sizeof(uint16_t) * (size_t)n, "ragged bins");
    x.pos.reserve(sizeof(int) * (size_t)n, "ragged places");
    x.place.reserve(sizeof(RaggedPlace) * (size_t)n, "ragged place records");
    x.cap = n;
}

void Engine::ragged_begin(int c, long long n, const uint8_t *d_reads, const uint8_t *d_refs, hipStream_t stream) {
    ensure_ragged(c, n);
    RaggedCtx &x = rag_[c];
    x.src_reads = d_reads;
    x.src_refs = d_refs;
    const int NG = ragged_bins();
    hip_check(hipMemsetAsync(x.counters.get(), 0, sizeof(unsigned) * (kRaggedMaxBins + kRaggedMaxGroups), stream), "hipMemsetAsync");
    RaggedClassifyArgs a{d_reads, d_refs, n, R_, F_, d_read_class_.get(), d_ref_class_.get(), (int)ref_caps_.size(), NG, x.bin.get(), x.counters.get()};
    void *kargs[] = {&a};
    const long long blocks = (n + kRaggedClassifyPairs - 1) / kRaggedClassifyPairs;
    hip_check(hipLaunchKernel((const void *)&ragged_classify_kernel, dim3((unsigned)blocks), dim3(256), kargs, 0, stream),
              "hipLaunchKernel(ragged_classify_kernel)");
    hip_check(hipMemcpyAsync(x.h_counts.get(), x.counters.get(), sizeof(unsigned) * (size_t)NG, hipMemcpyDeviceToHost, stream), "D2H histogram");
    hip_check(hipEventRecord(x.counted.get(), stream), "hipEventRecord");
}

std::vector<Engine::LengthGroup> Engine::fold_groups(std::vector<long long> &total, std::vector<int> &group_of_bin) const {
    const int NR = (int)read_caps_.size(), NF = (int)ref_caps_.size(), NG = NR * NF;
    std::vector<int> target((size_t)NG);
    for (int g = 0; g < NG; ++g) target[g] = g;
    const long long bin_min = std::min<long long>(ragged_min_, 256);
    for (int rc = 0; rc < NR; ++rc) {
        long long in_class = 0;
        for (int fc = 0; fc < NF; ++fc) in_class += total[rc * NF + fc];
        if (in_class == 0) continue;
        if (in_class < ragged_min_ && rc < NR - 1) {
            for (int fc = 0; fc < NF; ++fc) {
                const int g = rc * NF + fc;
                total[g + NF] += total[g];
                total[g] = 0;
                target[g] = g + NF;
            }
            continue;
        }
        for (int fc = 0; fc < NF - 1; ++fc) {
            const int g = rc * NF + fc;
            if (total[g] == 0 || total[g] >= bin_min) continue;
            total[g + 1] += total[g];
            total[g] = 0;
            target[g] = g + 1;
        }
    }
    for (int g = NG - 1; g >= 0; --g) target[g] = target[target[g]];
    std::vector<LengthGroup> groups;
    std::vector<int> group_at((size_t)NG, -1);
    long long pair_ofs = 0;
    size_t read_ofs = 0, ref_ofs = 0;
    for (int g = 0; g < NG; ++g) {
        if (total[g] == 0) continue;
        LengthGroup lg;
        lg.R = read_caps_[g / NF];
        lg.F = ref_caps_[g % NF];
        lg.pairs = total[g];
        lg.pair_ofs = pair_ofs;
        lg.read_ofs = read_ofs;
        lg.ref_ofs = ref_ofs;
        pair_ofs += lg.pairs;
        read_ofs += (size_t)lg.pairs * lg.R;
        ref_ofs += (size_t)lg.pairs * lg.F;
        group_at[g] = (int)groups.size();
        groups.push_back(lg);
    }
    group_of_bin.assign((size_t)NG, 0);
    for (int g = 0; g < NG; ++g) group_of_bin[g] = std::max(group_at[target[g]], 0);
    return groups;
}

bool Engine::ragged_finish(int c, int alg, long long n, int16_t *d_scores, hipStream_t stream, bool always) {
    RaggedCtx &x = rag_[c];
    const int NG = ragged_bins();
    const auto t0 = std::chrono::steady_clock::now();
    hip_check(hipEventSynchronize(x.counted.get()), "hipEventSynchronize");
    const auto t_counted = std::chrono::steady_clock::now();
    host_stats_.classify_ms += ms_between(t0, t_counted);
    std::vector<long long> total((size_t)NG);
    long long seen = 0;
    for (int g = 0; g < NG; ++g) seen += (total[g] = (long long)x.h_counts.get()[g]);
    if (seen != n) throw std::runtime_error("length classification lost pairs");
    std::vector<int> group_of_bin;
    const std::vector<LengthGroup> groups = fold_groups(total, group_of_bin);
    double swept = 0;
    for (const LengthGroup &g : groups) swept += (double)g.pairs * g.R * g.F;
    const double padded = (double)n * R_ * F_;
    if (!always && swept >= 0.67 * padded) return false;
    const int NL = (int)groups.size();
    if (NL > kRaggedMaxGroups) throw std::runtime_error("too many length groups");
    uint16_t *h_map = reinterpret_cast<uint16_t *>(x.h_tables.get());
    RaggedGroupDev *h_groups = reinterpret_cast<RaggedGroupDev *>(x.h_tables.get() + sizeof(uint16_t) * kRaggedMaxBins);
    for (int g = 0; g < NG; ++g) h_map[g] = (uint16_t)group_of_bin[g];
    for (int l = 0; l < NL; ++l)
        h_groups[l] = RaggedGroupDev{groups[l].R, groups[l].F, groups[l].pair_ofs, (long long)groups[l].read_ofs, (long long)groups[l].ref_ofs};
    hip_check(hipMemcpyAsync(x.tables.get(), x.h_tables.get(), kRaggedTableBytes, hipMemcpyHostToDevice, stream), "H2D length groups");
    RaggedPermuteArgs pa{x.src_reads, x.src_refs, n, R_, F_, x.bin.get(), reinterpret_cast<const uint16_t *>(x.tables.get()),
                         reinterpret_cast<const RaggedGroupDev *>(x.tables.get() + sizeof(uint16_t) * kRaggedMaxBins), NL,
                         x.counters.get() + kRaggedMaxBins, x.reads.get(), x.refs.get(), x.pos.get(), x.place.get()};
    void *pargs[] = {&pa};
    hip_check(hipLaunchKernel((const void *)&ragged_place_kernel, dim3((unsigned)((n + 255) / 256)), dim3(256), pargs, 0, stream),
              "hipLaunchKernel(ragged_place_kernel)");
    hip_check(hipLaunchKernel((const void *)&ragged_copy_kernel, dim3((unsigned)((n + 3) / 4)), dim3(256), pargs, 0, stream),
              "hipLaunchKernel(ragged_copy_kernel)");
    for (size_t first = 0; first < groups.size();) {
        size_t end = first;
        int widest = 0;
        while (end < groups.size() && groups[end].R == groups[first].R) widest = std::max(widest, groups[end++].F);
        launch_score(class_plan(groups[first].R, widest), alg, groups[first].R, widest, 0, x.reads.get(), x.refs.get(), x.scores.get(), stream,
                     groups.data() + first, (int)(end - first));
        host_stats_.launches += 1;
        first = end;
    }
    RaggedUnpermuteArgs ua{x.scores.get(), x.pos.get(), d_scores, n};
    void *uargs[] = {&ua};
    hip_check(hipLaunchKernel((const void *)&ragged_unpermute_kernel, dim3((unsigned)((n + 255) / 256)), dim3(256), uargs, 0, stream),
              "hipLaunchKernel(ragged_unpermute_kernel)");
    host_stats_.cells_swept += swept;
    host_stats_.cells_padded += padded;
    host_stats_.launch_ms += ms_between(t_counted, std::chrono::steady_clock::now());
    return true;
}

}
```

### versalignlib_amd/csrc/kernel_instances.hip.h

```cpp
#pragma once

#include "dp_kernels.hip.h"
#include "trace_kernels.hip.h"
#include "placed_kernels.hip.h"
#include "extend_kernels.hip.h"

#define VALIGN_PART0(X, Y) X(64, 32) Y(8, 4)
#define VALIGN_PART1(X, Y) Y(64, 24) Y(8, 6) Y(16, 4)
#define VALIGN_PART2(X, Y) X(64, 16) Y(8, 10)
#define VALIGN_PART3(X, Y) X(16, 10) Y(8, 12) Y(16, 8)
#define VALIGN_PART4(X, Y) X(32, 10) Y(16, 12) Y(64, 12)
#define VALIGN_PART5(X, Y) X(64, 8) X(8, 8) Y(32, 8) Y(32, 12)
#define VALIGN_KERNEL_PARTS 6

#define VALIGN_ALL_PARTS(X, Y) VALIGN_PART0(X, Y) VALIGN_PART1(X, Y) VALIGN_PART2(X, Y) VALIGN_PART3(X, Y) VALIGN_PART4(X, Y) VALIGN_PART5(X, Y)

#define VALIGN_FAST_KERNELS(PREFIX, G, K)                                                            \
    PREFIX __global__ void score_kernel<G, K, kAlgSW, kGapLinear>(const ScoreArgs);                  \
    PREFIX __global__ void score_kernel<G, K, kAlgSW, kGapSym>(const ScoreArgs);                     \
    PREFIX __global__ void score_kernel<G, K, kAlgSW, kGapAffine>(const ScoreArgs);                  \
    PREFIX __global__ void score_kernel<G, K, kAlgSW, kGapAffineSym>(const ScoreArgs);               \
    PREFIX __global__ void score_kernel<G, K, kAlgSW, kGapAffineSymF16>(const ScoreArgs);            \
    PREFIX __global__ void score_kernel<G, K, kAlgSW, kGapAffineF16>(const ScoreArgs);               \
    PREFIX __global__ void score_kernel<G, K, kAlgNW, kGapLinear>(const ScoreArgs);                  \
    PREFIX __global__ void score_kernel<G, K, kAlgNW, kGapSym>(const ScoreArgs);                     \
    PREFIX __global__ void score_kernel<G, K, kAlgNW, kGapAffine>(const ScoreArgs);                  \
    PREFIX __global__ void score_kernel<G, K, kAlgNW, kGapAffineSym>(const ScoreArgs);               \
    PREFIX __global__ void score_kernel<G, K, kAlgNW, kGapAffineSymF16>(const ScoreArgs);            \
    PREFIX __global__ void score_kernel<G, K, kAlgNW, kGapAffineF16>(const ScoreArgs);               \
    PREFIX __global__ void score_kernel<G, K, kAlgNW, kGapSymF16>(const ScoreArgs);                  \
    PREFIX __global__ void score_kernel<G, K, kAlgSW, kGapSymF16>(const ScoreArgs);                  \
    PREFIX __global__ void align_fill_affine_tag_kernel<G, K, kAlgSW, true>(const FillArgs);         \
    PREFIX __global__ void align_fill_affine_tag_kernel<G, K, kAlgNW, true>(const FillArgs);         \
    PREFIX __global__ void align_fill_tag_kernel<G, K, kAlgSW, true, false>(const FillArgs);         \
    PREFIX __global__ void align_fill_tag_kernel<G, K, kAlgSW, true, false, false, true>(const FillArgs); \
    PREFIX __global__ void align_fill_tag_kernel<G, K, kAlgNW, false, false>(const FillArgs);

#define VALIGN_FALLBACK_KERNELS(PREFIX, G, K)                                                        \
    PREFIX __global__ void align_fill_kernel<G, K, kAlgSW, false>(const FillArgs);                   \
    PREFIX __global__ void align_fill_kernel<G, K, kAlgSW, true>(const FillArgs);                    \
    PREFIX __global__ void align_fill_kernel<G, K, kAlgNW, false>(const FillArgs);                   \
    PREFIX __global__ void align_fill_kernel<G, K, kAlgNW, true>(const FillArgs);                    \
    PREFIX __global__ void align_fill_affine_kernel<G, K, kAlgSW, false>(const FillArgs);            \
    PREFIX __global__ void align_fill_affine_kernel<G, K, kAlgNW, false>(const FillArgs);            \
    PREFIX __global__ void align_fill_affine_kernel<G, K, kAlgSW, true>(const FillArgs);             \
    PREFIX __global__ void align_fill_affine_kernel<G, K, kAlgNW, true>(const FillArgs);             \
    PREFIX __global__ void align_fill_sse_kernel<G, K, kAlgSW>(const FillArgs);                      \
    PREFIX __global__ void align_fill_sse_kernel<G, K, kAlgNW>(const FillArgs);                      \
    PREFIX __global__ void align_fill_tag_kernel<G, K, kAlgSW, false, false>(const FillArgs);        \
    PREFIX __global__ void align_fill_tag_kernel<G, K, kAlgSW, false, true>(const FillArgs);         \
    PREFIX __global__ void align_fill_tag_kernel<G, K, kAlgSW, true, true>(const FillArgs);          \
    PREFIX __global__ void align_fill_tag_kernel<G, K, kAlgNW, false, true>(const FillArgs);         \
    PREFIX __global__ void align_fill_affine_tag_kernel<G, K, kAlgSW, false>(const FillArgs);        \
    PREFIX __global__ void align_fill_affine_tag_kernel<G, K, kAlgNW, false>(const FillArgs);

#define VALIGN_PLACED_KERNELS(PREFIX, G, K, FULL) PREFIX const void *placed_kernel<G, K, FULL>(int, int);

#define VALIGN_SUBOPT_KERNELS(PREFIX, G, K, FULL) PREFIX const void *subopt_kernel<G, K, FULL>(int, int);

#define VALIGN_EXTEND_KERNELS(PREFIX, G, K, FULL) PREFIX const void *extend_kernel<G, K, FULL>(int);
```

### versalignlib_amd/csrc/kernel_part.hip

```cpp
#include <hip/hip_runtime.h>
#include <stdint.h>

#include <type_traits>

#define VALIGN_KERNEL_PART_TU 1
#include "kernel_instances.hip.h"

#ifndef VALIGN_PART
#error "compile with -DVALIGN_PART=<0..VALIGN_KERNEL_PARTS-1>"
#endif

namespace valign {

#define VALIGN_DEFINE_FULL(G, K) VALIGN_FAST_KERNELS(template, G, K) VALIGN_FALLBACK_KERNELS(template, G, K) VALIGN_PLACED_KERNELS(template, G, K, true) VALIGN_SUBOPT_KERNELS(template, G, K, true) VALIGN_EXTEND_KERNELS(template, G, K, true)
#define VALIGN_DEFINE_FAST(G, K) VALIGN_FAST_KERNELS(template, G, K) VALIGN_PLACED_KERNELS(template, G, K, false) VALIGN_SUBOPT_KERNELS(template, G, K, false) VALIGN_EXTEND_KERNELS(template, G, K, false)
#if VALIGN_PART == 0
VALIGN_PART0(VALIGN_DEFINE_FULL, VALIGN_DEFINE_FAST)
#elif VALIGN_PART == 1
VALIGN_PART1(VALIGN_DEFINE_FULL, VALIGN_DEFINE_FAST)
#elif VALIGN_PART == 2
VALIGN_PART2(VALIGN_DEFINE_FULL, VALIGN_DEFINE_FAST)
#elif VALIGN_PART == 3
VALIGN_PART3(VALIGN_DEFINE_FULL, VALIGN_DEFINE_FAST)
#elif VALIGN_PART == 4
VALIGN_PART4(VALIGN_DEFINE_FULL, VALIGN_DEFINE_FAST)
#elif VALIGN_PART == 5
VALIGN_PART5(VALIGN_DEFINE_FULL, VALIGN_DEFINE_FAST)
#else
#error "VALIGN_PART out of range"
#endif

}
```

Baseline: 9618 GCUPS.

## Add 8x19 side-tile score kernel for SW symmetric-affine reads up to 152 bases

Adds a dedicated score kernel geometry (8 lanes per group, 19 rows per lane) that covers a 150-base read in one tile. It runs only the tilted frame with row tables, uses 16-bit selector streams in LDS instead of 32-bit ones, and drops the LDS profile. The host plan switches to it for SW symmetric-affine int16 calls with reads of 129 to 152 bases, and chunk rounding is adjusted to fit both plans. The aim is to waste fewer padded rows than the 16x10 tile (160 rows) and cut LDS traffic for selectors. The cost is an odd K that needs extra guards, plus higher register pressure from 19 rows per lane.

```diff
diff --git a/versalignlib_amd/csrc/cell_constants.h b/versalignlib_amd/csrc/cell_constants.h
--- a/versalignlib_amd/csrc/cell_constants.h
+++ b/versalignlib_amd/csrc/cell_constants.h
@@ -14,6 +14,19 @@
 constexpr int kGapLinear = 0, kGapSym = 1, kGapAffine = 2, kGapAffineSym = 3;
 constexpr int kGapAffineSymF16 = 4, kGapAffineF16 = 5, kGapSymF16 = 6;
 constexpr int kTiltMaxK = 12;
+constexpr int kSideTileG = 8, kSideTileK = 19;
+constexpr bool tilt_tables_only(int G, int K) { return G == kSideTileG && K == kSideTileK; }
+constexpr bool tilt_frame_built(int G, int K) { return K <= kTiltMaxK || tilt_tables_only(G, K); }
+constexpr int kSideTilePad = kSideTileG + 4, kSideTilePairs = 2 * (64 / kSideTileG);
+constexpr int side_tile_refs_area(int F) { return ((kSideTilePairs * F + 32 + 15) / 16) * 16; }
+constexpr int side_tile_stream_stride(int F) {
+    const int dw = (F + 2 * kSideTilePad + 1) / 2;
+    return 4 * (dw + ((kSideTileG - dw) % 64 + 64) % 64);
+}
+constexpr int side_tile_wave_lds(int R, int F) {
+    const int streams = (64 / kSideTileG) * side_tile_stream_stride(F), raw_reads = ((kSideTilePairs * R + 32 + 15) / 16) * 16;
+    return side_tile_refs_area(F) + (streams > raw_reads ? streams : raw_reads);
+}
 
 constexpr int kBandNwAbsent16 = -16384;
 constexpr int kBandNwAbsent32 = -(1 << 29);
diff --git a/versalignlib_amd/csrc/cell_rules.h b/versalignlib_amd/csrc/cell_rules.h
--- a/versalignlib_amd/csrc/cell_rules.h
+++ b/versalignlib_amd/csrc/cell_rules.h
@@ -17,6 +17,7 @@
     bool no_max3 = false;
     bool no_tilt = false;
     bool no_row_tables = false;
+    bool no_side_tile = false;
 };
 
 inline long long nw_tilt_span(const Scoring &sc, int rows, int F) {
@@ -145,7 +146,7 @@
     return (long long)rows + F - lead;
 }
 inline bool sym_affine_tilt_ok(const RuleInputs &in, int R, int F, int rows, int K) {
-    if (in.no_tilt || K > kTiltMaxK || !sym_affine_max3_ok(in, R, F)) return false;
+    if (in.no_tilt || K <= 0 || !tilt_frame_built(rows / K, K) || !sym_affine_max3_ok(in, R, F)) return false;
     const Scoring &sc = in.sc;
     const long long B = sym_affine_tilt_bias(sc);
     const long long hi = (long long)std::min(R, F) * std::max({sc.match, sc.mismatch, 0}) + 1;
@@ -163,6 +164,30 @@
     return sym_affine_row_table_low(in.sc) >= 0 && sym_affine_row_table_high(in.sc) <= 255 && lds_tables <= lds_profile;
 }
 inline const char *ran_sym_affine_scores_name(bool row_tables) { return row_tables ? "row_tables" : "lds_profile"; }
+
+constexpr int kSideTileRows = kSideTileG * kSideTileK, kSideTileMinRead = 129;
+constexpr int kSideTileBlockWaves = 4, kSideTileLdsGranule = 2048, kSideTileLdsBudget = 152 * 1024;
+inline bool side_tile_lds_ok(int lds_wave) {
+    const long long block = ((long long)lds_wave * kSideTileBlockWaves + kSideTileLdsGranule - 1) / kSideTileLdsGranule * kSideTileLdsGranule;
+    return lds_wave > 0 && 2 * block <= kSideTileLdsBudget;
+}
+inline const char *sym_affine_side_tile_refusal(const RuleInputs &in, int alg, int gaps, int R, int F, bool latency, bool forced) {
+    const int lds_wave = side_tile_wave_lds(R, F);
+    if (in.no_side_tile) return "the side tile is switched off (VALIGN_HIP_DEBUG=no_side_tile)";
+    if (alg != kAlgSW) return "the 8 x 19 tile exists for Smith-Waterman scores only";
+    if (gaps != kGapAffineSym)
+        return "the 8 x 19 tile exists for int16 cells with symmetric affine gaps only (half_float_cells = 0, open_read = open_ref, ext_read = ext_ref)";
+    if (R > kSideTileRows) return "the 8 x 19 tile holds reads of at most 152 bases";
+    if (in.no_tilt) return "the 8 x 19 tile runs the tilted frame only (VALIGN_HIP_DEBUG=no_tilt)";
+    if (in.no_row_tables) return "the 8 x 19 tile runs the row tables only (VALIGN_HIP_DEBUG=no_row_tables)";
+    if (!sym_affine_row_tables_ok(in, in.R, in.F, kSideTileRows, kSideTileK, lds_wave, lds_wave))
+        return "the 8 x 19 tile runs the tilted frame with row tables only: shape x scoring leave its window, or a substitution score of the frame is no byte (sym_affine_row_tables_ok)";
+    if (!side_tile_lds_ok(lds_wave)) return "the 8 x 19 tile needs two 4-wave blocks per CU: the reference is too long for its LDS budget";
+    if (forced) return "";
+    if (R < kSideTileMinRead) return "reads of at most 128 bases fit a smaller tile";
+    if (latency) return "small calls take the latency plan";
+    return "";
+}
 
 struct FillChoice {
     int kernel = 0;
diff --git a/versalignlib_amd/csrc/dp_kernels.hip.h b/versalignlib_amd/csrc/dp_kernels.hip.h
--- a/versalignlib_amd/csrc/dp_kernels.hip.h
+++ b/versalignlib_amd/csrc/dp_kernels.hip.h
@@ -48,6 +48,7 @@
         long long pair_ofs;
         long long read_ofs, ref_ofs;
     } groups[kMaxScoreGroups];
+    unsigned *form_seen;
 };
 
 __device__ __forceinline__ s16x2 pk(short v) { return s16x2{v, v}; }
@@ -119,7 +120,8 @@
 template <int G, int K>
 struct Geo {
     static_assert(G == 4 || G == 8 || G == 16 || G == 32 || G == 64, "group size");
-    static_assert(K % 2 == 0, "rows per lane must be even");
+    static constexpr bool kNoProfile = tilt_tables_only(G, K);
+    static_assert(K % 2 == 0 || kNoProfile, "rows per lane must be even");
     static constexpr int kGroups = kWave / G;
     static constexpr int kPairs = 2 * kGroups;
     static constexpr int kRows = G * K;
@@ -137,7 +139,7 @@
         }
         return best;
     }
-    static constexpr int kPairStride = slab_dwords() * 4;
+    static constexpr int kPairStride = kNoProfile ? 0 : slab_dwords() * 4;
     static constexpr int kZeroSlab = 4 * kPairs;
     static constexpr int kProfBytes = (4 * kPairs + 1) * kPairStride;
     __host__ __device__ static constexpr int row_offset(int l, int q) { return l * kLaneBytes + q * 2; }
@@ -417,6 +419,7 @@
 
 constexpr int row_table_pad(int G) { return G + 4; }
 constexpr unsigned kSelZero4 = 0x0c0c0c0cu;
+constexpr unsigned kSelWiden = 0x04010400u;
 
 template <int G, int K>
 __device__ __forceinline__ bool wave_setup_tables(const uint8_t *reads, const uint8_t *refs, long long n, int R, int F,
@@ -476,10 +479,16 @@
                 const unsigned lo23 = __builtin_amdgcn_perm(col[3], col[2], 0x05010400u), hi23 = __builtin_amdgcn_perm(col[3], col[2], 0x07030602u);
                 unsigned (&T)[K] = half ? Tb : Ta;
                 T[q0] = __builtin_amdgcn_perm(lo23, lo01, 0x05040100u);
-                T[q0 + 1] = __builtin_amdgcn_perm(lo23, lo01, 0x07060302u);
-                if (q0 + 2 < K) {
-                    T[q0 + 2] = __builtin_amdgcn_perm(hi23, hi01, 0x05040100u);
-                    T[q0 + 3] = __builtin_amdgcn_perm(hi23, hi01, 0x07060302u);
+                if constexpr (K % 2 == 0) {
+                    T[q0 + 1] = __builtin_amdgcn_perm(lo23, lo01, 0x07060302u);
+                    if (q0 + 2 < K) {
+                        T[q0 + 2] = __builtin_amdgcn_perm(hi23, hi01, 0x05040100u);
+                        T[q0 + 3] = __builtin_amdgcn_perm(hi23, hi01, 0x07060302u);
+                    }
+                } else {
+                    if (q0 + 1 < K) T[q0 + 1] = __builtin_amdgcn_perm(lo23, lo01, 0x07060302u);
+                    if (q0 + 2 < K) T[q0 + 2] = __builtin_amdgcn_perm(hi23, hi01, 0x05040100u);
+                    if (q0 + 3 < K) T[q0 + 3] = __builtin_amdgcn_perm(hi23, hi01, 0x07060302u);
                 }
             }
         }
@@ -493,10 +502,14 @@
     bool before_last = false;
     unsigned *stream = reinterpret_cast<unsigned *>(sel);
     const int stride_dw = sel_stride / 4;
+    constexpr bool SEL16 = tilt_tables_only(G, K);
+    unsigned short *stream16 = reinterpret_cast<unsigned short *>(sel);
+    const int stride_h = sel_stride / 2;
     if (live) {
         for (int idx = lane; idx < geo::kGroups * 2 * kPad; idx += kWave) {
             const int g = idx / (2 * kPad), x = idx - g * (2 * kPad);
-            stream[g * stride_dw + (x < kPad ? x : F + x)] = kSelZero4;
+            if constexpr (SEL16) stream16[g * stride_h + (x < kPad ? x : F + x)] = (unsigned short)0x0c0c;
+            else stream[g * stride_dw + (x < kPad ? x : F + x)] = kSelZero4;
         }
         const int ref_skew = (int)((unsigned long long)(refs + pair0 * F) & 15ull);
         typedef unsigned short u16;
@@ -507,6 +520,7 @@
             pb = pb > last ? last : pb;
             const unsigned char *raw_a = raw + ref_skew + pa * F, *raw_b = raw + ref_skew + pb * F;
             unsigned *out_g = stream + g * stride_dw + kPad;
+            unsigned short *out16_g = stream16 + g * stride_h + kPad;
             u16x2 ends_a = u16x2{0, 0}, ends_b = u16x2{0, 0};
             auto note = [](u16x2 &ends, unsigned acgt, int j) __attribute__((always_inline)) {
                 const unsigned none = ~nonzero_bytes(acgt) & 0x80808080u;
@@ -518,19 +532,27 @@
             for (int j = 4 * lane; j < F4; j += 4 * kWave) {
                 const unsigned ca = base_class4(lds_dword_at(raw_a + j)), cb = base_class4(lds_dword_at(raw_b + j));
                 const unsigned sa = select_bytes8(0x0c0c0c03u, 0x0201000cu, ca), sb = select_bytes8(0x0c0c0c07u, 0x0605040cu, cb);
-                uint4 s;
-                s.x = __builtin_amdgcn_perm(sb, sa, 0x0c040c00u) | 0x0c000c00u;
-                s.y = __builtin_amdgcn_perm(sb, sa, 0x0c050c01u) | 0x0c000c00u;
-                s.z = __builtin_amdgcn_perm(sb, sa, 0x0c060c02u) | 0x0c000c00u;
-                s.w = __builtin_amdgcn_perm(sb, sa, 0x0c070c03u) | 0x0c000c00u;
-                *reinterpret_cast<uint4 *>(out_g + j) = s;
+                if constexpr (SEL16) {
+                    uint2 s;
+                    s.x = __builtin_amdgcn_perm(sb, sa, 0x05010400u);
+                    s.y = __builtin_amdgcn_perm(sb, sa, 0x07030602u);
+                    *reinterpret_cast<uint2 *>(out16_g + j) = s;
+                } else {
+                    uint4 s;
+                    s.x = __builtin_amdgcn_perm(sb, sa, 0x0c040c00u) | 0x0c000c00u;
+                    s.y = __builtin_amdgcn_perm(sb, sa, 0x0c050c01u) | 0x0c000c00u;
+                    s.z = __builtin_amdgcn_perm(sb, sa, 0x0c060c02u) | 0x0c000c00u;
+                    s.w = __builtin_amdgcn_perm(sb, sa, 0x0c070c03u) | 0x0c000c00u;
+                    *reinterpret_cast<uint4 *>(out_g + j) = s;
+                }
                 note(ends_a, sa ^ kSelZero4, j);
                 note(ends_b, sb ^ kSelZero4, j);
             }
             for (int j = F4 + lane; j < F; j += kWave) {
                 const int ca = base_class(raw_a[j]), cb = base_class(raw_b[j]);
                 const bool va = ca >= 1 && ca <= 4, vb = cb >= 1 && cb <= 4;
-                out_g[j] = (va ? (unsigned)(ca - 1) : 0x0cu) | (vb ? (unsigned)(cb + 3) : 0x0cu) << 16 | 0x0c000c00u;
+                if constexpr (SEL16) out16_g[j] = (unsigned short)((va ? (unsigned)(ca - 1) : 0x0cu) | (vb ? (unsigned)(cb + 3) : 0x0cu) << 8);
+                else out_g[j] = (va ? (unsigned)(ca - 1) : 0x0cu) | (vb ? (unsigned)(cb + 3) : 0x0cu) << 16 | 0x0c000c00u;
                 ends_a = __builtin_elementwise_max(ends_a, u16x2{va ? (u16)(j + 1) : (u16)0, va ? (u16)0 : (u16)(0xFFFF - j)});
                 ends_b = __builtin_elementwise_max(ends_b, u16x2{vb ? (u16)(j + 1) : (u16)0, vb ? (u16)0 : (u16)(0xFFFF - j)});
             }
@@ -548,7 +570,7 @@
     repair = __builtin_amdgcn_readfirstlane((int)before_last) != 0;
     w.cols_used = __builtin_amdgcn_readfirstlane(cols_used);
     w.prof = raw;
-    w.refc = reinterpret_cast<unsigned char *>(stream + kPad);
+    w.refc = SEL16 ? reinterpret_cast<unsigned char *>(stream16 + kPad) : reinterpret_cast<unsigned char *>(stream + kPad);
     w.first_bad = nullptr;
     w.pair0 = pair0;
     w.last = last;
@@ -642,7 +664,8 @@
     const int tilt_col = TILT ? -(int)(AFFINE ? args.ext_read : args.gap_read) : 0;
     int fold = tilt_row + tilt_col;
     short s_row0 = 0;
-    if constexpr (SOURCES && K <= kTiltMaxK) {
+    constexpr bool TILT_BUILT = SOURCES && tilt_frame_built(G, K), TABLES_ONLY = SOURCES && tilt_tables_only(G, K);
+    if constexpr (TILT_BUILT) {
         if (args.sym_max3_bias > 0 && (args.sym_max3_bias >> 16) != 0) {
             fold = -2 * (int)args.ext_ref;
             s_row0 = (short)((int)args.ext_ref - (int)args.open_ref);
@@ -665,7 +688,14 @@
     const short s_zero = HALF ? __builtin_bit_cast(short, (_Float16)fold) : (short)fold;
     bool tables = false, repair = false;
     unsigned Ta[K], Tb[K];
-    if constexpr (SOURCES && K <= kTiltMaxK) {
+    if constexpr (TABLES_ONLY) {
+        tables = args.sym_max3_bias > 0 && (args.sym_max3_bias >> 16 & 3) == 3;
+        if (!tables) return;
+        if (!wave_setup_tables<G, K>(reads, refs, n_pairs, args.R, F_batch, args.prof_area, args.refc_stride, args.wave_lds,
+                                     s_match, s_mismatch, s_zero, s_row0, block, w, Ta, Tb, repair))
+            return;
+        if (args.form_seen != nullptr && lane == 0) args.form_seen[repair ? 1 : 0] = 1u;
+    } else if constexpr (TILT_BUILT) {
         tables = args.sym_max3_bias > 0 && (args.sym_max3_bias >> 16 & 3) == 3;
         bool live = false;
         if (tables)
@@ -728,7 +758,7 @@
     unsigned pa[K / 2], pb[K / 2];
     s16x2 S0[K], S1[K];
     unsigned ca_next = 0, cb_next = 0;
-    if (PIPE && !tables) {
+    if constexpr (!TABLES_ONLY) if (PIPE && !tables) {
         const unsigned ca = *(lds_cu8 *)(code_addr), cb = *(lds_cu8 *)(code_addr + 1);
         lds_load_lane<K>(lane_base + ca * geo::kPairStride, pa);
         lds_load_lane<K>(lane_base + cb * geo::kPairStride, pb);
@@ -964,8 +994,8 @@
         bool biased = false;
         if constexpr (SOURCES) {
             biased = args.sym_max3_bias > 0;
-            const bool tilted = K <= kTiltMaxK && biased && (args.sym_max3_bias >> 16) != 0;
-            if constexpr (K <= kTiltMaxK) if (tilted) {
+            const bool tilted = TILT_BUILT && biased && (args.sym_max3_bias >> 16) != 0;
+            if constexpr (TILT_BUILT) if (tilted) {
                 const int B = args.sym_max3_bias & 0xFFFF, xi = -(int)args.ext_ref;
                 const int oxi = -(int)args.open_ref - xi;
                 const s16x2 ox_c = pk((short)oxi), kx_c = pk((short)(K * xi));
@@ -986,9 +1016,15 @@
                 up0 = pk((short)(B + xi * u0 - oxi));
                 f_last = HOl[K - 1];
                 constexpr int kLdsProfile = 0, kRowTables = 1, kRowTablesRepair = 2;
+                constexpr bool SEL16 = TABLES_ONLY;
+                typedef __attribute__((address_space(3))) const unsigned short lds_cu16;
                 lds_cu32 *sel_ptr = (lds_cu32 *)(lds_offset(w.refc) + grp * args.refc_stride - 4 * (l - lead));
+                lds_cu16 *sel16_ptr = (lds_cu16 *)(lds_offset(w.refc) + grp * args.refc_stride - 2 * (l - lead));
                 unsigned sel_cur = 0, sel_next = 0;
-                if (tables) {
+                if constexpr (SEL16) {
+                    sel_cur = __builtin_amdgcn_perm(kSelZero4, (unsigned)sel16_ptr[0], kSelWiden);
+                    sel_next = sel16_ptr[1];
+                } else if (tables) {
                     sel_cur = sel_ptr[0];
                     sel_next = sel_ptr[1];
                 }
@@ -1015,9 +1051,15 @@
 #pragma unroll
                             for (int q = 0; q < K; ++q) S[q] = as_pk(as_u32(S[q]) | (q == 0 ? fix_0 : fix_q));
                         }
-                        sel_cur = sel_next;
-                        sel_next = ((volatile lds_cu32 *)sel_ptr)[2];
-                        sel_ptr += 1;
+                        if constexpr (SEL16) {
+                            sel_cur = __builtin_amdgcn_perm(kSelZero4, sel_next, kSelWiden);
+                            sel_next = ((volatile lds_cu16 *)sel16_ptr)[2];
+                            sel16_ptr += 1;
+                        } else {
+                            sel_cur = sel_next;
+                            sel_next = ((volatile lds_cu32 *)sel_ptr)[2];
+                            sel_ptr += 1;
+                        }
                     }
                     s16x2 e_cur;
                     auto pass1 = [&](int q, s16x2 &e) __attribute__((always_inline)) {
@@ -1039,7 +1081,8 @@
                         HOl[q] = ho;
                         if (!(q & 1)) {
                             s16x2 &a = acc[(q + SLOT0) % K];
-                            a = pk_max3_h(a, d[q], dprev[q + 1]);
+                            if (q + 1 < K) a = pk_max3_h(a, d[q], dprev[q + 1]);
+                            else a = pk_max_h(a, d[q]);
                         }
                         e_cur = e_next;
                     }
@@ -1060,18 +1103,18 @@
                         unrolled_steps(std::make_integer_sequence<int, K>{}, [&](auto slot_tag) __attribute__((always_inline)) { tilted_step(slot_tag, form_tag); });
                 };
                 int form = __builtin_amdgcn_readfirstlane(tables ? (repair ? kRowTablesRepair : kRowTables) : kLdsProfile);
-                if (form == kLdsProfile) tilted_sweep(std::integral_constant<int, kLdsProfile>{});
+                if constexpr (!TABLES_ONLY) if (form == kLdsProfile) tilted_sweep(std::integral_constant<int, kLdsProfile>{});
                 asm volatile("" : "+s"(form));
                 if (form == kRowTables) tilted_sweep(std::integral_constant<int, kRowTables>{});
                 asm volatile("" : "+s"(form));
                 if (form == kRowTablesRepair) tilted_sweep(std::integral_constant<int, kRowTablesRepair>{});
                 best = pk(0);
 #pragma unroll
-                for (int q = 0; q < K; q += 2) acc[q] = pk_max_h(acc[q], dprev[q + 1]);
+                for (int q = 0; q + 1 < K; q += 2) acc[q] = pk_max_h(acc[q], dprev[q + 1]);
 #pragma unroll
                 for (int q = 0; q < K; ++q) best = pk_max(best, acc[q] - fl[q]);
             }
-            if (biased && !tilted) {
+            if constexpr (!TABLES_ONLY) if (biased && !tilted) {
                 const s16x2 bias_c = pk((short)args.sym_max3_bias);
                 const s16x2 lead_bias = as_pk(as_u32(bias_c) & ~lmask);
                 auto biased_step = [&](s16x2 (&S)[K]) __attribute__((always_inline)) {
@@ -1124,7 +1167,7 @@
                 best = best - bias_c;
             }
         }
-        if (!biased) {
+        if constexpr (!TABLES_ONLY) if (!biased) {
             for (; t + 1 < steps; t += 2) {
                 step(std::false_type{}, first_t{}, S0, S1);
                 step(std::false_type{}, second_t{}, S1, S0);
@@ -1213,4 +1256,13 @@
     return w;
 }
 
-}
+static_assert(kSideTilePad == row_table_pad(kSideTileG) && kSideTilePairs == 2 * (kWave / kSideTileG), "cell_constants.h restates the side tile's layout");
+inline WaveLds row_table_lds16(int R, int F) {
+    WaveLds w;
+    w.prof_area = side_tile_refs_area(F);
+    w.refc_stride = side_tile_stream_stride(F);
+    w.total = side_tile_wave_lds(R, F);
+    return w;
+}
+
+}
diff --git a/versalignlib_amd/csrc/engine.hip.h b/versalignlib_amd/csrc/engine.hip.h
--- a/versalignlib_amd/csrc/engine.hip.h
+++ b/versalignlib_amd/csrc/engine.hip.h
@@ -44,6 +44,7 @@
 VALIGN_ALL_PARTS(VALIGN_DECLARE_FULL, VALIGN_DECLARE_FAST)
 #undef VALIGN_DECLARE_FULL
 #undef VALIGN_DECLARE_FAST
+VALIGN_SIDE_KERNELS(extern template)
 
 struct Geometry {
     int G, K;
@@ -121,7 +122,10 @@
 static_assert(kNumGeometries == 0 VALIGN_ALL_PARTS(VALIGN_COUNT, VALIGN_COUNT), "kernel_instances.hip.h lists other geometries than this table");
 #undef VALIGN_COUNT
 
+extern const Geometry kSideGeometry;
+
 constexpr int kMaxBlockLds = 160 * 1024;
+static_assert(kSideTileLdsBudget < kMaxBlockLds, "the side tile's LDS budget leaves a margin inside a CU's LDS");
 constexpr int kSlots = 4;
 constexpr int kDefaultBlockLds = 64 * 1024;
 
@@ -138,7 +142,7 @@
     DebugSwitches() {
         const char *env = getenv("VALIGN_HIP_DEBUG");
         if (!env) return;
-        static const char *const known[] = {"no_sym", "no_tag", "no_f16", "no_max3", "no_tilt", "no_row_tables", "no_fused", "no_prof_key", "no_overlap", "no_band_chain",
+        static const char *const known[] = {"no_sym", "no_tag", "no_f16", "no_max3", "no_tilt", "no_row_tables", "no_side_tile", "no_fused", "no_prof_key", "no_overlap", "no_band_chain",
                                             "force_long", "wide_align", "strip_k", "no_single_strip", "no_direct_out", "ragged_min", "chunk_bytes",
                                             "align_chunk_bytes", "direct_bytes", "scratch_cap_mb", "whole_rows", "short_strips", "cigar_rows_mb", "cigar_lanes",
                                             "span_scratch_bytes", "subopt_scratch_bytes", "span_cigar_mb"};
@@ -292,6 +296,7 @@
     RuleInputs rule_inputs() const {
         RuleInputs in = RuleInputs{sc_, R_, F_, sse_policy_, no_sym_, no_tag_, no_f16_, no_prof_key_, no_max3_, no_tilt_};
         in.no_row_tables = no_row_tables_;
+        in.no_side_tile = no_side_tile_;
         return in;
     }
     bool score_int16_ok(int alg) const;
@@ -452,8 +457,15 @@
 
     static LaunchPlan long_plan();
 
-
-    long long whole_rounds(long long pairs) const;
+    LaunchPlan score_plan_for(const LaunchPlan &base, int alg, int R, int F, bool latency, bool refuse = true) const;
+    static LaunchPlan side_plan(int R, int F);
+    const char *side_tile_refusal(int alg, int R, int F, bool latency) const;
+    bool few_pairs(long long n) const { return n > 0 && n <= (long long)latency_plan_.pairs_per_wave * 1024 && band_width_ == 0; }
+    const char *ran_side_tile_form() const;
+    void reset_side_tile_form(hipStream_t stream);
+
+
+    long long whole_rounds(long long pairs, bool sw_scores = false) const;
 
     bool direct_call(long long n, size_t per_pair) const;
 
@@ -500,7 +512,7 @@
 
     void ensure_staging(long long pairs);
 
-    long long host_chunk_pairs(bool shared_scratch, long long n) const;
+    long long host_chunk_pairs(bool shared_scratch, long long n, bool sw_scores = false) const;
     void stage_chunk(int slot, hipStream_t stream, const char *const *reads, const char *const *refs, long long cnt, int threads);
     void wait_slot(int slot, const std::function<void(int)> &drain);
     struct RecordKind {
@@ -642,6 +654,8 @@
     bool no_max3_ = dbg_.on("no_max3");
     bool no_tilt_ = dbg_.on("no_tilt");
     bool no_row_tables_ = dbg_.on("no_row_tables");
+    bool no_side_tile_ = dbg_.on("no_side_tile");
+    bool side_forced_ = false;
     bool no_fused_ = dbg_.on("no_fused");
     bool no_prof_key_ = dbg_.on("no_prof_key");
     bool copy_engines_primed_ = false;
@@ -734,6 +748,7 @@
     DeviceBuffer<BandBlock> d_band_blocks_;
     DeviceBuffer<int> d_band_fill_;
     RaggedCtx rag_[kSlots + 1];
+    DeviceBuffer<unsigned> d_form_seen_;
     DeviceBuffer<uint8_t> d_read_class_;
     DeviceBuffer<uint16_t> d_ref_class_;
 };
diff --git a/versalignlib_amd/csrc/engine_core.hip b/versalignlib_amd/csrc/engine_core.hip
--- a/versalignlib_amd/csrc/engine_core.hip
+++ b/versalignlib_amd/csrc/engine_core.hip
@@ -1,6 +1,17 @@
+#include <numeric>
+
 #include "engine.hip.h"
 
 namespace valign {
+
+static WaveLds side_tile_lds(int R, int F) { return row_table_lds16(R, F); }
+static Geometry side_geometry() {
+    Geometry g{kSideTileG, kSideTileK, false, &side_tile_lds, {}, {}, [](int, int) -> const void * { return nullptr; },
+               [](int, int) -> const void * { return nullptr; }, [](int) -> const void * { return nullptr; }};
+    g.kernel[kAlgSW][kGapAffineSym] = (const void *)&score_kernel<kSideTileG, kSideTileK, kAlgSW, kGapAffineSym>;
+    return g;
+}
+const Geometry kSideGeometry = side_geometry();
 
 Engine::Engine(int device, int R, int F, const Scoring &sc, int force_g, int force_k)
     : device_(device), R_(R), F_(F), sc_(sc) {
@@ -22,6 +33,12 @@
         throw std::runtime_error("device is " + arch_ + "; this library carries gfx950 code only");
     force_g_ = force_g;
     force_k_ = force_k;
+    side_forced_ = tilt_tables_only(force_g, force_k);
+    if (side_forced_) {
+        if (R_ > kSideTileRows)
+            throw std::runtime_error("the forced kernel geometry does not fit read_length=" + std::to_string(R) + ", ref_length=" + std::to_string(F));
+        force_g = force_k = 0;
+    }
     plan_ = choose_plan(R_, F_, force_g, force_k);
     align_resident_ = plan_;
     if (!force_g && !force_k && !plan_.long_mode && plan_.geo && plan_.geo->G * plan_.geo->K > 1536) plan_ = long_plan();
@@ -83,7 +100,11 @@
 }
 
 std::string Engine::describe(int opt, long long n) const {
-    const long long ppb = (long long)plan_.pairs_per_wave * plan_.waves_per_block;
+    LaunchPlan shown = plan_;
+    const int alg_shown = opt & 0xF;
+    if (alg_shown <= kAlgNW && !plan_.long_mode && band_width_ == 0 && !score_wide_cells(alg_shown))
+        shown = score_plan_for(plan_, alg_shown, R_, F_, few_pairs(n), false);
+    const long long ppb = (long long)shown.pairs_per_wave * shown.waves_per_block;
     int band_rows = 0, band_align = 0;
     band_block_shape(band_rows, band_align);
     char buf[4096];
@@ -101,9 +122,9 @@
              "\"ran_subopt\": \"%s\", \"subopt_scratch_bytes\": %lld, \"subopt_ring_cols\": %d, \"ran_extend\": \"%s\", \"extend_wide\": %d, "
              "\"ran_score_geometry\": \"%s\", \"ran_align_geometry\": \"%s\", "
              "\"ran_placed_geometry\": \"%s\", \"ran_subopt_geometry\": \"%s\", \"ran_extend_geometry\": \"%s\"}",
-             arch_.c_str(), device_, opt & 0xF, sc_.affine ? 1 : 0, plan_.geo->G, plan_.geo->K,
-             plan_.geo->G * plan_.geo->K, plan_.pairs_per_wave, plan_.waves_per_block, plan_.lds.total,
-             plan_.lds.total * plan_.waves_per_block, F_ + plan_.geo->G - 1, n > 0 ? (n + ppb - 1) / ppb : 0,
+             arch_.c_str(), device_, opt & 0xF, sc_.affine ? 1 : 0, shown.geo->G, shown.geo->K,
+             shown.geo->G * shown.geo->K, shown.pairs_per_wave, shown.waves_per_block, shown.lds.total,
+             shown.lds.total * shown.waves_per_block, F_ + shown.geo->G - 1, n > 0 ? (n + ppb - 1) / ppb : 0,
              plan_.long_mode ? 1 : 0, band_width_, ragged_, host_stats_.launches,
              host_stats_.cells_padded > 0 ? host_stats_.cells_swept / host_stats_.cells_padded : 1.0,
              score_cell_format(opt & 0xF, n), host_stats_.direct, host_stats_.packed, host_stats_.direct_out,
@@ -121,6 +142,8 @@
     if (ran_score_sym_affine_)
         out.insert(out.size() - 1, std::string(", \"ran_score_sym_affine\": \"") + ran_score_sym_affine_ + "\", \"ran_score_sym_affine_frame\": \"" +
                                        ran_score_sym_affine_frame_ + "\", \"ran_score_sym_affine_scores\": \"" + ran_score_sym_affine_scores_ + "\"");
+    if (ran_score_sym_affine_ && ran_score_geo_ == &kSideGeometry)
+        out.insert(out.size() - 1, std::string(", \"ran_score_sym_affine_form\": \"") + ran_side_tile_form() + "\"");
     return out;
 }
 
@@ -190,6 +213,45 @@
     return best;
 }
 
+LaunchPlan Engine::side_plan(int R, int F) {
+    LaunchPlan p;
+    p.geo = &kSideGeometry;
+    p.lds = kSideGeometry.lds(R, F);
+    p.waves_per_block = kSideTileBlockWaves;
+    p.pairs_per_wave = 2 * (kWave / kSideTileG);
+    return p;
+}
+
+const char *Engine::side_tile_refusal(int alg, int R, int F, bool latency) const {
+    const RuleInputs in = rule_inputs();
+    const int gaps = alg <= kAlgNW ? score_gap_form(in, alg, R, F, kSideTileRows) : -1;
+    return sym_affine_side_tile_refusal(in, alg, gaps, R, F, latency, side_forced_);
+}
+
+const char *Engine::ran_side_tile_form() const {
+    if (!d_form_seen_.get()) return "none";
+    unsigned seen[2] = {0, 0};
+    hip_check(hipSetDevice(device_), "hipSetDevice");
+    hip_check(hipDeviceSynchronize(), "hipDeviceSynchronize");
+    hip_check(hipMemcpy(seen, d_form_seen_.get(), sizeof seen, hipMemcpyDeviceToHost), "hipMemcpy(form words)");
+    return seen[0] && seen[1] ? "both" : (seen[1] ? "row_tables_repair" : (seen[0] ? "row_tables" : "none"));
+}
+
+void Engine::reset_side_tile_form(hipStream_t stream) {
+    if (!d_form_seen_.get()) return;
+    if (stream) hip_check(hipMemsetAsync(d_form_seen_.get(), 0, 2 * sizeof(unsigned), stream), "hipMemsetAsync(form words)");
+    else hip_check(hipMemset(d_form_seen_.get(), 0, 2 * sizeof(unsigned)), "hipMemset(form words)");
+}
+
+LaunchPlan Engine::score_plan_for(const LaunchPlan &base, int alg, int R, int F, bool latency, bool refuse) const {
+    const bool chosen = (force_g_ || force_k_) && !side_forced_;
+    if (chosen) return base;
+    const char *refusal = side_tile_refusal(alg, R, F, latency);
+    if (!refusal[0]) return side_plan(R, F);
+    if (side_forced_ && refuse) throw std::runtime_error(std::string("group_lanes = 8, rows_per_lane = 19: ") + refusal);
+    return base;
+}
+
 LaunchPlan Engine::long_plan() {
     LaunchPlan p;
     p.long_mode = true;
@@ -201,10 +263,16 @@
     return p;
 }
 
-long long Engine::whole_rounds(long long pairs) const {
+long long Engine::whole_rounds(long long pairs, bool sw_scores) const {
     if (plan_.long_mode || !plan_.geo || cu_count_ <= 0) return pairs;
     const long long waves_per_cu = std::min<long long>(32, (kMaxBlockLds / std::max(1, plan_.lds.total * plan_.waves_per_block)) * plan_.waves_per_block);
-    const long long round_pairs = std::max<long long>(1, waves_per_cu) * cu_count_ * plan_.pairs_per_wave;
+    long long round_pairs = std::max<long long>(1, waves_per_cu) * cu_count_ * plan_.pairs_per_wave;
+    if (sw_scores && !((force_g_ || force_k_) && !side_forced_) && !side_tile_refusal(kAlgSW, R_, F_, false)[0]) {
+        const LaunchPlan side = side_plan(R_, F_);
+        const long long side_waves = std::min<long long>(32, (kMaxBlockLds / std::max(1, side.lds.total * side.waves_per_block)) * side.waves_per_block);
+        const long long side_round = std::max<long long>(1, side_waves) * cu_count_ * side.pairs_per_wave;
+        round_pairs = round_pairs / std::gcd(round_pairs, side_round) * side_round;
+    }
     return pairs >= round_pairs ? pairs / round_pairs * round_pairs : pairs;
 }
 
diff --git a/versalignlib_amd/csrc/engine_score.hip b/versalignlib_amd/csrc/engine_score.hip
--- a/versalignlib_amd/csrc/engine_score.hip
+++ b/versalignlib_amd/csrc/engine_score.hip
@@ -13,11 +13,14 @@
         ran_score_cells_ = 0;
         ran_score_geo_ = nullptr;
         ran_score_sym_affine_ = nullptr;
+        reset_side_tile_form(stream);
     }
     if (score_width_ == 16 && !score_int16_ok(alg))
         throw std::runtime_error("shape x scoring can leave the int16 range of the DP cells (read_length " +
                                  std::to_string(R_) + ", ref_length " + std::to_string(F_) + ")");
     const bool wide = score_wide_cells(alg);
+    if (side_forced_ && (plan_.long_mode || wide || band_width_ > 0))
+        throw std::runtime_error("group_lanes = 8, rows_per_lane = 19: the call takes the long-read kernels (a band, int32 cells, or a reference too long for the register sweep)");
     if (plan_.long_mode || wide) {
         score_long_device(alg, n, d_reads, d_refs, d_scores, stream);
         return;
@@ -32,8 +35,8 @@
         hip_check(hipEventRecord(ragged_dev_done_.get(), stream), "hipEventRecord");
         if (swept) return;
     }
-    const bool few = n <= (long long)latency_plan_.pairs_per_wave * 1024 && band_width_ == 0;
-    launch_score(few ? latency_plan_ : plan_, alg, R_, F_, n, d_reads, d_refs, d_scores, stream);
+    const bool few = few_pairs(n);
+    launch_score(score_plan_for(few ? latency_plan_ : plan_, alg, R_, F_, few), alg, R_, F_, n, d_reads, d_refs, d_scores, stream);
 }
 
 void Engine::launch_score(const LaunchPlan &plan, int alg, int R, int F, long long n, const uint8_t *d_reads,
@@ -47,6 +50,7 @@
     a.R = R;
     a.F = F;
     a.n_groups = n_groups;
+    a.form_seen = nullptr;
     const long long pairs_per_block = (long long)plan.pairs_per_wave * plan.waves_per_block;
     long long blocks = (n + pairs_per_block - 1) / pairs_per_block;
     if (n_groups > 0) {
@@ -69,6 +73,7 @@
     put_scoring(a);
     const int gaps = score_gap_form(rule_inputs(), alg, R, F, plan.geo->G * plan.geo->K);
     const void *fn = plan.geo->kernel[alg][gaps];
+    if (!fn) throw std::runtime_error("no score kernel of this gap form on " + ran_geometry(plan.geo));
     ran_score_cells_ |= gap_form_f16(gaps) ? kRanF16 : kRanInt16;
     ran_score_geo_ = plan.geo;
     if (alg == kAlgSW && gaps == kGapAffineSym) {
@@ -76,8 +81,16 @@
         a.sym_max3_bias = max3 ? sym_affine_bias(sc_) : 0;
         const bool tilted = sym_affine_tilt_ok(rule_inputs(), R_, F_, plan.geo->G * plan.geo->K, plan.geo->K);
         if (tilted) a.sym_max3_bias = sym_affine_tilt_bias(sc_) | 1 << 16;
-        const WaveLds tables_lds = row_table_lds(plan.geo->G, R, F);
+        const WaveLds tables_lds = tilt_tables_only(plan.geo->G, plan.geo->K) ? plan.lds : row_table_lds(plan.geo->G, R, F);
         const bool row_tables = tilted && sym_affine_row_tables_ok(rule_inputs(), R_, F_, plan.geo->G * plan.geo->K, plan.geo->K, plan.lds.total, tables_lds.total);
+        if (tilt_tables_only(plan.geo->G, plan.geo->K)) {
+            if (!row_tables) throw std::runtime_error("the 8 x 19 side tile was planned for a launch whose row tables are refused");
+            if (!d_form_seen_.get()) {
+                d_form_seen_.reserve(2 * sizeof(unsigned), "side tile form words");
+                hip_check(hipMemset(d_form_seen_.get(), 0, 2 * sizeof(unsigned)), "hipMemset(form words)");
+            }
+            a.form_seen = d_form_seen_.get();
+        }
         if (row_tables) {
             a.sym_max3_bias |= 1 << 17;
             a.prof_area = tables_lds.prof_area;
@@ -113,11 +126,11 @@
               "hipLaunchKernel(unpack_kernel)");
 }
 
-long long Engine::host_chunk_pairs(bool shared_scratch, long long n) const {
+long long Engine::host_chunk_pairs(bool shared_scratch, long long n, bool sw_scores) const {
     const size_t per_pair = (size_t)R_ + F_;
     const size_t chunk_bytes = shared_scratch && !dbg_.on("chunk_bytes") ? std::max<size_t>(score_chunk_bytes_, 192u << 20) : score_chunk_bytes_;
     long long chunk = per_pair ? (long long)(chunk_bytes / per_pair) : n;
-    chunk = whole_rounds(chunk);
+    chunk = whole_rounds(chunk, sw_scores);
     chunk = std::max<long long>(chunk, 1024);
     return std::min<long long>(chunk, n);
 }
@@ -219,8 +232,10 @@
     const size_t per_pair = (size_t)R_ + F_;
     const bool shared_scratch = (plan_.long_mode || score_wide_cells(alg)) && long_mode(alg, false).brow;
     const bool strips_in_turn = plan_.long_mode && shared_scratch;
-    const long long chunk = host_chunk_pairs(strips_in_turn, n);
+    const bool sw_scores = alg == kAlgSW;
+    const long long chunk = host_chunk_pairs(strips_in_turn, n, sw_scores);
     reset_pipeline();
+    reset_side_tile_form(nullptr);
     ensure_staging(chunk);
     if (threads < 1) threads = 1;
     threads = std::min(threads, 64);
@@ -268,7 +283,7 @@
     int slot = 0;
     long long chunk_no = 0, cnt = 0;
     for (long long begin = 0; begin < n; begin += cnt, slot = (slot + 1) % kSlots, ++chunk_no) {
-        const long long ramp = (n > 2 * chunk) ? (chunk_no == 0 ? whole_rounds(chunk / 4) : (chunk_no == 1 ? whole_rounds(chunk / 2) : chunk)) : chunk;
+        const long long ramp = (n > 2 * chunk) ? (chunk_no == 0 ? whole_rounds(chunk / 4, sw_scores) : (chunk_no == 1 ? whole_rounds(chunk / 2, sw_scores) : chunk)) : chunk;
         cnt = std::min<long long>(std::max<long long>(ramp, 1024), n - begin);
         wait_slot(slot, drain);
         hipStream_t st = streams_[shared_scratch ? 0 : slot].get();
@@ -443,8 +458,8 @@
         size_t end = first;
         int widest = 0;
         while (end < groups.size() && groups[end].R == groups[first].R) widest = std::max(widest, groups[end++].F);
-        launch_score(class_plan(groups[first].R, widest), alg, groups[first].R, widest, 0, x.reads.get(), x.refs.get(), x.scores.get(), stream,
-                     groups.data() + first, (int)(end - first));
+        launch_score(score_plan_for(class_plan(groups[first].R, widest), alg, groups[first].R, widest, false), alg, groups[first].R, widest, 0,
+                     x.reads.get(), x.refs.get(), x.scores.get(), stream, groups.data() + first, (int)(end - first));
         host_stats_.launches += 1;
         first = end;
     }
diff --git a/versalignlib_amd/csrc/kernel_instances.hip.h b/versalignlib_amd/csrc/kernel_instances.hip.h
--- a/versalignlib_amd/csrc/kernel_instances.hip.h
+++ b/versalignlib_amd/csrc/kernel_instances.hip.h
@@ -12,6 +12,8 @@
 #define VALIGN_PART4(X, Y) X(32, 10) Y(16, 12) Y(64, 12)
 #define VALIGN_PART5(X, Y) X(64, 8) X(8, 8) Y(32, 8) Y(32, 12)
 #define VALIGN_KERNEL_PARTS 6
+#define VALIGN_SIDE_PART 1
+#define VALIGN_SIDE_KERNELS(PREFIX) PREFIX __global__ void score_kernel<kSideTileG, kSideTileK, kAlgSW, kGapAffineSym>(const ScoreArgs);
 
 #define VALIGN_ALL_PARTS(X, Y) VALIGN_PART0(X, Y) VALIGN_PART1(X, Y) VALIGN_PART2(X, Y) VALIGN_PART3(X, Y) VALIGN_PART4(X, Y) VALIGN_PART5(X, Y)
 
diff --git a/versalignlib_amd/csrc/kernel_part.hip b/versalignlib_amd/csrc/kernel_part.hip
--- a/versalignlib_amd/csrc/kernel_part.hip
+++ b/versalignlib_amd/csrc/kernel_part.hip
@@ -29,5 +29,8 @@
 #else
 #error "VALIGN_PART out of range"
 #endif
+#if VALIGN_PART == VALIGN_SIDE_PART
+VALIGN_SIDE_KERNELS(template)
+#endif
 
 }
```

Result: faster. 10300 GCUPS (median of 6 runs) (+7.1%).
